# ashawkey/torch-ngp

Hardware: AMD Instinct MI355X
Metric: training samples/s (rays x steps), lego-shaped synthetic, fp16 autocast, full step incl. Adam (higher is better)
Workload: dtype f16

## Files before the change

### include/ngp_hip.h

```cpp
#ifndef NGP_HIP_H
#define NGP_HIP_H

#include <stddef.h>
#include <stdint.h>

#ifdef __cplusplus
extern "C" {
#endif

typedef void* ngp_stream_t;

enum {
    NGP_OK = 0,
    NGP_ERR_INVALID = 1,
    NGP_ERR_LAUNCH = 2,
    NGP_ERR_DEVICE = 3
};

enum { NGP_F32 = 0, NGP_F16 = 1, NGP_F64 = 2 };

#define NGP_MAX_LEVELS 32

const char* ngp_last_error(void);
int ngp_abi_version(void);
// ... 29 lines not shown
int ngp_grid_encode_backward_ordered(const void* grad, const float* inputs, const void* embeddings, const int32_t* offsets,
                                     void* grad_embeddings, uint32_t B, uint32_t D, uint32_t C, uint32_t L, float S, uint32_t H,
                                     const void* dy_dx, void* grad_inputs, uint32_t gridtype, int align_corners, uint32_t interp, int dtype,
                                     float bound, void* workspace, size_t workspace_bytes, ngp_stream_t stream);
int ngp_grid_encode_backward_backward_ordered(const void* grad, const float* inputs, const void* embeddings, const int32_t* offsets,
                                              const void* grad_grad_inputs, void* grad_grad, void* grad_embeddings, void* grad_inputs2,
                                              uint32_t B, uint32_t D, uint32_t C, uint32_t L, float S, uint32_t H, uint32_t gridtype,
                                              int align_corners, uint32_t interp, int dtype, void* workspace, size_t workspace_bytes,
                                              ngp_stream_t stream);
size_t ngp_grid_ordered_workspace_bytes(uint32_t B, uint32_t D, uint32_t C, int dtype);
int ngp_grid_backward_is_reproducible(const int32_t* offsets_host, uint32_t B, uint32_t D, uint32_t C, uint32_t L, float S, uint32_t H,
                                      uint32_t gridtype, int align_corners, int dtype);


int ngp_sh_encode_forward(const void* inputs, void* outputs, uint32_t B, uint32_t D, uint32_t C, void* dy_dx,
                          int dtype, ngp_stream_t stream);
int ngp_sh_encode_backward(const void* grad, const void* inputs, uint32_t B, uint32_t D, uint32_t C,
                           const void* dy_dx, void* grad_inputs, int dtype, ngp_stream_t stream);
int ngp_sh_encode_backward_backward(const void* grad, const void* inputs, const void* dy_dx, const void* u, uint32_t B, uint32_t D,
                                    uint32_t C, void* grad_grad, void* grad_inputs2, int dtype, ngp_stream_t stream);


int ngp_near_far_from_aabb(const float* rays_o, const float* rays_d, const float* aabb, uint32_t N, float min_near,
                           float* nears, float* fars, ngp_stream_t stream);
int ngp_sph_from_ray(const float* rays_o, const float* rays_d, float radius, uint32_t N, float* coords,
                     ngp_stream_t stream);
int ngp_morton3D(const int32_t* coords, uint32_t N, int32_t* indices, ngp_stream_t stream);
int ngp_morton3D_invert(const int32_t* indices, uint32_t N, int32_t* coords, ngp_stream_t stream);
int ngp_packbits(const float* grid, uint32_t N, float density_thresh, uint8_t* bitfield, ngp_stream_t stream);
int ngp_packbits_ex(const float* grid, uint32_t N, float density_thresh, const float* thresh_cap, uint8_t* bitfield,
                    ngp_stream_t stream);

size_t ngp_march_rays_train_workspace_bytes(uint32_t N);
int ngp_march_rays_train(const float* rays_o, const float* rays_d, const uint8_t* grid, float bound, float dt_gamma,
                         uint32_t max_steps, uint32_t N, uint32_t C, uint32_t H, uint32_t M, const float* nears,
                         const float* fars, float* xyzs, float* dirs, float* deltas, int32_t* rays,
                         int32_t* counter, const float* noises, void* workspace, ngp_stream_t stream);

int ngp_composite_rays_train_forward(const float* sigmas, const float* rgbs, const float* deltas,
                                     const int32_t* rays, uint32_t M, uint32_t N, float T_thresh,
                                     float* weights_sum, float* depth, float* image, ngp_stream_t stream);
int ngp_composite_rays_train_backward(const float* grad_weights_sum, const float* grad_image, const float* sigmas,
                                      const float* rgbs, const float* deltas, const int32_t* rays,
                                      const float* weights_sum, const float* image, uint32_t M, uint32_t N,
                                      float T_thresh, float* grad_sigmas, float* grad_rgbs, ngp_stream_t stream);

int ngp_march_rays(uint32_t n_alive, uint32_t n_step, const int32_t* rays_alive, const float* rays_t,
                   const float* rays_o, const float* rays_d, float bound, float dt_gamma, uint32_t max_steps,
                   uint32_t C, uint32_t H, const uint8_t* grid, const float* nears, const float* fars, float* xyzs,
                   float* dirs, float* deltas, const float* noises, ngp_stream_t stream);
int ngp_composite_rays(uint32_t n_alive, uint32_t n_step, float T_thresh, int32_t* rays_alive, float* rays_t,
                       const float* sigmas, const float* rgbs, const float* deltas, float* weights_sum,
                       float* depth, float* image, ngp_stream_t stream);

int ngp_near_far_from_aabb_f64(const double* rays_o, const double* rays_d, const double* aabb, uint32_t N, float min_near,
                               double* nears, double* fars, ngp_stream_t stream);
int ngp_sph_from_ray_f64(const double* rays_o, const double* rays_d, float radius, uint32_t N, double* coords, ngp_stream_t stream);
int ngp_packbits_f64(const double* grid, uint32_t N, float density_thresh, uint8_t* bitfield, ngp_stream_t stream);
int ngp_composite_rays_train_forward_f64(const double* sigmas, const double* rgbs, const double* deltas, const int32_t* rays,
                                         uint32_t M, uint32_t N, float T_thresh, double* weights_sum, double* depth, double* image,
                                         ngp_stream_t stream);
int ngp_composite_rays_train_backward_f64(const double* grad_weights_sum, const double* grad_image, const double* sigmas,
                                          const double* rgbs, const double* deltas, const int32_t* rays, const double* weights_sum,
                                          const double* image, uint32_t M, uint32_t N, float T_thresh, double* grad_sigmas,
                                          double* grad_rgbs, ngp_stream_t stream);
int ngp_composite_rays_f64(uint32_t n_alive, uint32_t n_step, float T_thresh, int32_t* rays_alive, double* rays_t,
                           const double* sigmas, const double* rgbs, const double* deltas, double* weights_sum, double* depth,
                           double* image, ngp_stream_t stream);

size_t ngp_compact_rays_workspace_bytes(uint32_t n_alive);
int ngp_compact_rays(const int32_t* rays_alive, uint32_t n_alive, int32_t* out_alive, int32_t* out_count,
                     void* workspace, ngp_stream_t stream);


int ngp_ffmlp_forward(const void* inputs, const void* weights, uint32_t B, uint32_t input_dim, uint32_t output_dim,
                      uint32_t hidden_dim, uint32_t num_layers, uint32_t activation, uint32_t output_activation,
                      void* forward_buffer, void* outputs, ngp_stream_t stream);
int ngp_ffmlp_inference(const void* inputs, const void* weights, uint32_t B, uint32_t input_dim,
                        uint32_t output_dim, uint32_t hidden_dim, uint32_t num_layers, uint32_t activation,
                        uint32_t output_activation, void* inference_buffer, void* outputs, ngp_stream_t stream);
int ngp_ffmlp_backward(const void* grad, const void* inputs, const void* weights, const void* forward_buffer,
                       uint32_t B, uint32_t input_dim, uint32_t output_dim, uint32_t hidden_dim, uint32_t num_layers,
                       uint32_t activation, uint32_t output_activation, int calc_grad_inputs, void* backward_buffer,
                       void* grad_inputs, void* grad_weights, ngp_stream_t stream);
int ngp_allocate_splitk(size_t size);
int ngp_free_splitk(void);

int ngp_grid_encode_forward_ex(const float* inputs, const void* embeddings, const int32_t* offsets, void* outputs,
                               uint32_t B, uint32_t D, uint32_t C, uint32_t L, float S, uint32_t H, void* dy_dx,
                               uint32_t gridtype, int align_corners, uint32_t interp, int dtype, float bound,
                               ngp_stream_t stream);
int ngp_grid_encode_backward_ex(const void* grad, const float* inputs, const void* embeddings, const int32_t* offsets,
                                void* grad_embeddings, uint32_t B, uint32_t D, uint32_t C, uint32_t L, float S,
                                uint32_t H, const void* dy_dx, void* grad_inputs, uint32_t gridtype, int align_corners,
                                uint32_t interp, int dtype, float bound, ngp_stream_t stream);
int ngp_grid_encode_forward_sched(const float* inputs, const void* embeddings, const int32_t* offsets, void* outputs,
                                  uint32_t B, uint32_t D, uint32_t C, uint32_t L, float S, uint32_t H, void* dy_dx,
                                  uint32_t gridtype, int align_corners, uint32_t interp, int dtype, float bound,
                                  const float* level_cost_host, ngp_stream_t stream);

int ngp_grid_encode_forward_sel(const float* inputs, const void* embeddings, const void* embeddings_alt, const float* parity,
                                const uint32_t* rows_dev, const int32_t* offsets, void* outputs, uint32_t B, uint32_t D, uint32_t C, uint32_t L,
                                float S, uint32_t H, uint32_t gridtype, int align_corners, uint32_t interp, int dtype, float bound,
                                const float* level_cost_host, ngp_stream_t stream);

uint32_t ngp_grid_forward_work_lists(uint32_t L, uint32_t tiles, const float* level_cost_host, uint16_t* level_out, uint32_t* tile0_out,
                                     uint32_t* end_out);

size_t ngp_grid_backward_workspace_bytes(const int32_t* offsets_host, uint32_t B, uint32_t D, uint32_t C, uint32_t L, float S, uint32_t H,
                                         uint32_t gridtype, int align_corners, int dtype);
int ngp_grid_encode_backward_checked(const void* grad, const float* inputs, const void* embeddings, const int32_t* offsets,
                                     void* grad_embeddings, uint32_t B, uint32_t D, uint32_t C, uint32_t L, float S, uint32_t H,
                                     const void* dy_dx, void* grad_inputs, uint32_t gridtype, int align_corners, uint32_t interp,
                                     int dtype, float bound, const int32_t* offsets_host, void* workspace, size_t workspace_bytes,
                                     float* found_inf, ngp_stream_t stream);

typedef struct ngp_table_adam {
    float* param[2]; float* exp_avg[2]; float* exp_avg_sq[2]; void* param_fp16[2];
    const float* state;
    float lr, beta1, beta2, eps;
} ngp_table_adam_t;
uint32_t ngp_grid_table_adam_prefix(const int32_t* offsets_host, uint32_t B, uint32_t D, uint32_t C, uint32_t L, float S, uint32_t H,
                                    uint32_t gridtype, int align_corners, int dtype);
typedef struct ngp_slab_sets {
    const void* slabs_a; uint32_t n_slabs_a, n_params_a; void* grad_weights_a;
    const void* slabs_b; uint32_t n_slabs_b, n_params_b; void* grad_weights_b;
    const float* ray_err; uint32_t n_rays; float* loss;
    uint32_t overwrite_table;
    const ngp_table_adam_t* table_adam;
} ngp_slab_sets_t;
int ngp_grid_encode_backward_checked_slabs(const void* grad, const float* inputs, const void* embeddings, const int32_t* offsets,
                                           void* grad_embeddings, uint32_t B, uint32_t D, uint32_t C, uint32_t L, float S, uint32_t H,
                                           const void* dy_dx, void* grad_inputs, uint32_t gridtype, int align_corners, uint32_t interp,
                                           int dtype, float bound, const int32_t* offsets_host, void* workspace, size_t workspace_bytes,
                                           float* found_inf, const ngp_slab_sets_t* slab_sets, ngp_stream_t stream);
int ngp_grid_encode_backward_ws(const void* grad, const float* inputs, const void* embeddings, const int32_t* offsets,
                                void* grad_embeddings, uint32_t B, uint32_t D, uint32_t C, uint32_t L, float S, uint32_t H,
                                const void* dy_dx, void* grad_inputs, uint32_t gridtype, int align_corners, uint32_t interp,
                                int dtype, float bound, const int32_t* offsets_host, void* workspace, size_t workspace_bytes,
                                ngp_stream_t stream);

size_t ngp_density_grid_update_workspace_bytes(uint32_t n_cells);
int ngp_density_grid_update(const float* sigmas, const int64_t* cells, uint32_t n, float density_scale, float decay, float* density_grid,
                            uint32_t n_cells, float* scratch, float density_thresh, float* mean_out, uint8_t* bitfield, void* workspace,
                            ngp_stream_t stream);

#define NGP_FF_INPUT_PLANAR 1u
#define NGP_FF_DX_PLANAR 2u
#define NGP_FF_LAYERED 4u
#define NGP_FF_SINGLE_WAVE 8u
#define NGP_FF_DEFER_REDUCE 16u
#define NGP_FF_RECOMPUTE 32u
#define NGP_FF_SERIAL_FLUSH 64u
int ngp_ffmlp_forward_ex(const void* inputs, const void* weights, uint32_t B, uint32_t input_dim, uint32_t output_dim,
                         uint32_t hidden_dim, uint32_t num_layers, uint32_t activation, uint32_t output_activation,
                         void* forward_buffer, void* outputs, uint32_t flags, ngp_stream_t stream);
int ngp_ffmlp_inference_ex(const void* inputs, const void* weights, uint32_t B, uint32_t input_dim,
                           uint32_t output_dim, uint32_t hidden_dim, uint32_t num_layers, uint32_t activation,
                           uint32_t output_activation, void* inference_buffer, void* outputs, uint32_t flags,
                           ngp_stream_t stream);
int ngp_ffmlp_backward_ex(const void* grad, const void* inputs, const void* weights, const void* forward_buffer,
                          uint32_t B, uint32_t input_dim, uint32_t output_dim, uint32_t hidden_dim, uint32_t num_layers,
                          uint32_t activation, uint32_t output_activation, int calc_grad_inputs, void* backward_buffer,
                          void* grad_inputs, void* grad_weights, uint32_t flags, ngp_stream_t stream);

size_t ngp_ffmlp_backward_workspace_bytes(uint32_t B, uint32_t input_dim, uint32_t hidden_dim, uint32_t num_layers);
int ngp_ffmlp_backward_ws(const void* grad, const void* inputs, const void* weights, const void* forward_buffer, uint32_t B,
                          uint32_t input_dim, uint32_t output_dim, uint32_t hidden_dim, uint32_t num_layers, uint32_t activation,
                          uint32_t output_activation, int calc_grad_inputs, void* backward_buffer, void* grad_inputs, void* grad_weights,
                          uint32_t flags, void* workspace, size_t workspace_bytes, ngp_stream_t stream);

size_t ngp_ffmlp_backward_backward_workspace_bytes(uint32_t B, uint32_t input_dim, uint32_t hidden_dim, uint32_t num_layers,
                                                   uint32_t activation);
int ngp_ffmlp_backward_backward(const void* grad, const void* inputs, const void* weights, const void* forward_buffer, const void* u,
                                uint32_t B, uint32_t input_dim, uint32_t output_dim, uint32_t hidden_dim, uint32_t num_layers,
                                uint32_t activation, void* grad_grad, void* grad_weights2, void* grad_inputs2, void* workspace,
                                size_t workspace_bytes, ngp_stream_t stream);

int ngp_network_forward(const void* enc, const float* dirs, uint32_t M, uint32_t M_valid, const void* w_sigma, const void* w_color,
                        uint32_t num_layers_sigma, uint32_t num_layers_color, float density_scale, int training,
                        void* forward_buffer_sigma, void* h16, float* sigma, void* color_in, void* forward_buffer_color, float* rgb,
                        uint32_t flags, ngp_stream_t stream);

int ngp_network_forward_rows(const void* enc, const float* dirs, uint32_t M, uint32_t M_valid, const void* w_sigma, const void* w_color,
                             uint32_t num_layers_sigma, uint32_t num_layers_color, float density_scale, int training,
                             void* forward_buffer_sigma, void* h16, float* sigma, void* color_in, void* forward_buffer_color, float* rgb,
                             uint32_t flags, const uint32_t* rows_dev, ngp_stream_t stream);

int ngp_network_backward_color(const void* grad_out16, const void* color_in, const void* w_color, const void* forward_buffer_color, uint32_t M,
                               uint32_t num_layers_color, void* backward_buffer, const float* grad_sigma, const void* h16,
                               float density_scale, void* grad_h16, void* grad_w_color, uint32_t flags, ngp_stream_t stream);
uint32_t ngp_ffmlp_backward_slab_count(uint32_t B, uint32_t input_dim, uint32_t hidden_dim, uint32_t num_layers);
int ngp_ffmlp_reduce_slabs_pair(const void* slabs_a, uint32_t n_slabs_a, uint32_t n_params_a, void* grad_weights_a, const void* slabs_b,
                                uint32_t n_slabs_b, uint32_t n_params_b, void* grad_weights_b, float* found_inf, ngp_stream_t stream);

int ngp_pipeline_mid_forward(const void* h16, const float* dirs, float* sigma, void* color_in, uint32_t M, uint32_t M_valid,
                             float density_scale, ngp_stream_t stream);
int ngp_pipeline_rgb_forward(const void* out16, float* rgb, uint32_t M, ngp_stream_t stream);
int ngp_pipeline_rgb_backward(const float* grad_rgb, const float* rgb, void* grad_out16, uint32_t M, ngp_stream_t stream);
int ngp_pipeline_mid_backward(const float* grad_sigma, const void* h16, const void* grad_color_in, void* grad_h16, uint32_t M,
                              float density_scale, ngp_stream_t stream);

int ngp_pipeline_mse_loss(const float* image, const float* target, uint32_t n, const float* loss_scale, float* loss,
                          float* grad_image, ngp_stream_t stream);

#define NGP_LINEAR_STACK_MAX 8
uint32_t ngp_linear_stack_flat_size(uint32_t depth, uint32_t n_in, uint32_t hidden, uint32_t n_out, int identity);
int ngp_linear_stack_pack(const float* const* weights, uint32_t depth, uint32_t n_in, uint32_t hidden, uint32_t n_out, int identity,
                          void* flat_fp16, ngp_stream_t stream);
int ngp_linear_stack_unpack_grad(const void* grad_flat_fp16, uint32_t depth, uint32_t n_in, uint32_t hidden, uint32_t n_out, int identity,
                                 float* const* grads, ngp_stream_t stream);

int ngp_pad_2d_fp16(const void* src, uint32_t src_rows, uint32_t src_cols, uint32_t src_row_stride, void* dst, uint32_t dst_rows,
                    uint32_t dst_cols, ngp_stream_t stream);

int ngp_rays_from_pixels(const float* poses, uint32_t B, float fx, float fy, float cx, float cy, uint32_t W, const int64_t* inds,
                         uint32_t inds_batch_stride, uint32_t N, float* rays_o, float* rays_d, ngp_stream_t stream);

#define NGP_MARCH_RESET_COUNTER 1u
#define NGP_MARCH_ZERO_TAIL 2u
#define NGP_MARCH_SCAN_LAUNCH 8u
#define NGP_MARCH_NOISE_FROM_SEED 4u
int ngp_march_rays_train_ex(const float* rays_o, const float* rays_d, const uint8_t* grid, float bound, float dt_gamma,
                            uint32_t max_steps, uint32_t N, uint32_t C, uint32_t H, uint32_t M, const float* nears,
                            const float* fars, float* xyzs, float* dirs, float* deltas, int32_t* rays, int32_t* counter,
                            const float* noises, void* workspace, uint32_t flags, ngp_stream_t stream);
int ngp_march_rays_train_aabb(const float* rays_o, const float* rays_d, const uint8_t* grid, float bound, float dt_gamma,
                              uint32_t max_steps, uint32_t N, uint32_t C, uint32_t H, uint32_t M, const float* aabb, float min_near,
                              float* nears, float* fars, float* xyzs, float* dirs, float* deltas, int32_t* rays, int32_t* counter,
                              const float* noises, void* workspace, uint32_t flags, ngp_stream_t stream);

int ngp_march_rays_ex(uint32_t n_alive, uint32_t n_step, const int32_t* rays_alive, const float* rays_t, const float* rays_o,
                      const float* rays_d, float bound, float dt_gamma, uint32_t max_steps, uint32_t C, uint32_t H,
                      const uint8_t* grid, const float* nears, const float* fars, float* xyzs, float* dirs, float* deltas,
                      const float* noises, uint32_t zero_rows, ngp_stream_t stream);

int ngp_march_rays_dev(const int32_t* state, uint32_t alive_bound, uint32_t n_total, uint32_t n_step_cap, const int32_t* rays_alive, const float* rays_t,
                       const float* rays_o, const float* rays_d, float bound, float dt_gamma, uint32_t max_steps, uint32_t C, uint32_t H,
                       const uint8_t* grid, const float* nears, const float* fars, float* xyzs, float* dirs, float* deltas,
                       const float* noises, uint32_t rows, ngp_stream_t stream);
int ngp_march_rays_dev_rows(const int32_t* state, uint32_t alive_bound, uint32_t n_total, uint32_t n_step_cap, const int32_t* rays_alive, const float* rays_t,
                            const float* rays_o, const float* rays_d, float bound, float dt_gamma, uint32_t max_steps, uint32_t C, uint32_t H,
                            const uint8_t* grid, const float* nears, const float* fars, float* xyzs, float* dirs, float* deltas,
                            const float* noises, uint32_t rows, uint32_t* rows_used, ngp_stream_t stream);
int ngp_composite_rays_dev(const int32_t* state, uint32_t alive_bound, uint32_t n_total, uint32_t n_step_cap, float T_thresh, int32_t* rays_alive, float* rays_t,
                           const float* sigmas, const float* rgbs, const float* deltas, float* weights_sum, float* depth, float* image,
                           ngp_stream_t stream);
int ngp_compact_rays_dev(const int32_t* state, uint32_t alive_bound, uint32_t n_total, uint32_t n_step_cap, uint32_t max_steps, const int32_t* rays_alive,
                         int32_t* out_alive, int32_t* out_state, void* workspace, ngp_stream_t stream);

int ngp_composite_rays_features(uint32_t n_alive, uint32_t n_step, float T_thresh, const int32_t* rays_alive, const float* sigmas,
                                const void* feats, const float* deltas, const float* weights_sum, uint32_t C, int feat_dtype,
                                float* out, ngp_stream_t stream);
int ngp_composite_rays_features_dev(const int32_t* state, uint32_t alive_bound, uint32_t n_total, uint32_t n_step_cap, float T_thresh,
                                    const int32_t* rays_alive, const float* sigmas, const void* feats, const float* deltas,
                                    const float* weights_sum, uint32_t C, int feat_dtype, float* out, ngp_stream_t stream);

typedef struct ngp_render_loop {
    int32_t* state;
    int32_t* alive[2];
    float* rays_t; const float* rays_o; const float* rays_d; const float* nears; const float* fars; const uint8_t* grid; const float* noises;
    float* xyzs; float* dirs; float* deltas; void* enc; float* sigmas; float* rgbs;
    const void* embeddings; const int32_t* offsets; const float* level_cost_host; const void* w_sigma; const void* w_color;
    float* weights_sum; float* depth; float* image; void* compact_workspace;
    uint32_t* rows_used;
    uint32_t lanes, rows, n_total, n_step_cap, max_steps, cascade, grid_size;
    uint32_t L, H, gridtype, interp, num_layers_sigma, num_layers_color;
    int32_t align_corners;
    float bound, dt_gamma, T_thresh, S, density_scale;
} ngp_render_loop_t;
int ngp_render_iterations_dev(const ngp_render_loop_t* args, uint32_t n_iter, uint32_t first_cur, ngp_stream_t stream);

size_t ngp_coarse_occupancy_bytes(uint32_t C, uint32_t H);
int ngp_coarse_occupancy(const uint8_t* grid, uint32_t C, uint32_t H, uint8_t* coarse, ngp_stream_t stream);
int ngp_cull_rays(const float* rays_o, const float* rays_d, const float* nears, const float* fars, uint32_t N, float bound, uint32_t C,
                  uint32_t H, const uint8_t* coarse, int32_t* rays_alive, ngp_stream_t stream);

int ngp_composite_rays_train_forward_ex(const float* sigmas, const float* rgbs, const float* deltas, const int32_t* rays,
                                        uint32_t M, uint32_t N, float T_thresh, float* weights_sum, float* depth, float* image,
                                        int bg_mode, float bg_scalar, const float* bg, const float* nears, const float* fars,
                                        float* image_out, float* depth_out, ngp_stream_t stream);
int ngp_composite_rays_train_backward_ex(const float* grad_weights_sum, const float* grad_image, const float* sigmas,
                                         const float* rgbs, const float* deltas, const int32_t* rays,
                                         const float* weights_sum, const float* image, uint32_t M, uint32_t N,
                                         float T_thresh, float* grad_sigmas, float* grad_rgbs, int bg_mode, float bg_scalar,
                                         const float* bg, const uint32_t* rows_used, ngp_stream_t stream);

int ngp_composite_rays_train_geo_forward(const float* sigmas, const float* rgbs, const float* deltas, const int32_t* rays, uint32_t M,
                                         uint32_t N, float T_thresh, float* weights_sum, float* depth, float* image,
                                         float* distortion, ngp_stream_t stream);
int ngp_composite_rays_train_geo_backward(const float* grad_weights_sum, const float* grad_depth, const float* grad_image,
                                          const float* grad_distortion, const float* sigmas, const float* rgbs, const float* deltas,
                                          const int32_t* rays, const float* weights_sum, const float* depth, const float* image,
                                          const float* distortion, uint32_t M, uint32_t N, float T_thresh, float* grad_sigmas,
                                          float* grad_rgbs, ngp_stream_t stream);
int ngp_composite_rays_train_geo_forward_f64(const double* sigmas, const double* rgbs, const double* deltas, const int32_t* rays,
                                             uint32_t M, uint32_t N, float T_thresh, double* weights_sum, double* depth, double* image,
                                             double* distortion, ngp_stream_t stream);
int ngp_composite_rays_train_geo_backward_f64(const double* grad_weights_sum, const double* grad_depth, const double* grad_image,
                                              const double* grad_distortion, const double* sigmas, const double* rgbs,
                                              const double* deltas, const int32_t* rays, const double* weights_sum, const double* depth,
                                              const double* image, const double* distortion, uint32_t M, uint32_t N, float T_thresh,
                                              double* grad_sigmas, double* grad_rgbs, ngp_stream_t stream);

int ngp_composite_rays_train_features_forward(const float* sigmas, const void* feats, const float* deltas, const int32_t* rays, uint32_t M,
                                              uint32_t N, uint32_t C, float T_thresh, int feat_dtype, float* out, ngp_stream_t stream);
// ... 93 lines not shown
```

### torch-ngp_amd/_ngp_capi.py

```python
import ctypes
import os

import torch

_HERE = os.path.dirname(os.path.abspath(__file__))
LIB_PATH = os.environ.get('NGP_HIP_LIBRARY') or os.path.join(_HERE, 'libngp_hip.so')

NGP_F32, NGP_F16, NGP_F64 = 0, 1, 2
NGP_FF_INPUT_PLANAR, NGP_FF_DX_PLANAR, NGP_FF_LAYERED, NGP_FF_SINGLE_WAVE, NGP_FF_DEFER_REDUCE, NGP_FF_RECOMPUTE = 1, 2, 4, 8, 16, 32
NGP_FF_SERIAL_FLUSH = 64
NGP_MARCH_RESET_COUNTER, NGP_MARCH_ZERO_TAIL, NGP_MARCH_NOISE_FROM_SEED, NGP_MARCH_SCAN_LAUNCH = 1, 2, 4, 8
NGP_OPT_PHASE_CHECK, NGP_OPT_PHASE_UPDATE, NGP_OPT_PHASE_COMMIT, NGP_OPT_PHASE_FLIP = 1, 2, 4, 8
ABI_VERSION = 11

if not os.path.exists(LIB_PATH):
    raise ImportError(
        f"{LIB_PATH} is missing: build the HIP extension first (python __graft_entry__.py, or "
        f"make -C {os.path.join(_HERE, 'csrc')}).  There is no CPU fallback for these operators.")

lib = ctypes.CDLL(LIB_PATH)

_vp, _u32, _f32, _i32, _sz = ctypes.c_void_p, ctypes.c_uint32, ctypes.c_float, ctypes.c_int, ctypes.c_size_t

_SIGNATURES = {
    'ngp_grid_encode_forward': [_vp, _vp, _vp, _vp, _u32, _u32, _u32, _u32, _f32, _u32, _vp, _u32, _i32, _u32, _i32, _vp],
    'ngp_grid_encode_backward': [_vp, _vp, _vp, _vp, _vp, _u32, _u32, _u32, _u32, _f32, _u32, _vp, _vp, _u32, _i32, _u32, _i32, _vp],
    'ngp_grad_total_variation': [_vp, _vp, _vp, _vp, _f32, _u32, _u32, _u32, _u32, _f32, _u32, _u32, _i32, _i32, _vp],
    'ngp_grid_corner_indices': [_vp, _vp, _vp, _u32, _u32, _u32, _f32, _u32, _u32, _i32, _vp],
    'ngp_grid_level_table': [_u32, _f32, _u32, _vp, _vp],
    'ngp_grid_encode_backward_backward': [_vp, _vp, _vp, _vp, _vp, _vp, _vp, _vp, _u32, _u32, _u32, _u32, _f32, _u32, _u32, _i32, _u32, _i32, _vp,
                                          _sz, _vp],
    'ngp_grid_encode_backward_ordered': [_vp, _vp, _vp, _vp, _vp, _u32, _u32, _u32, _u32, _f32, _u32, _vp, _vp, _u32, _i32, _u32, _i32, _f32, _vp,
                                         _sz, _vp],
    'ngp_grid_encode_backward_backward_ordered': [_vp, _vp, _vp, _vp, _vp, _vp, _vp, _vp, _u32, _u32, _u32, _u32, _f32, _u32, _u32, _i32, _u32, _i32,
                                                  _vp, _sz, _vp],
    'ngp_grid_backward_is_reproducible': [_vp, _u32, _u32, _u32, _u32, _f32, _u32, _u32, _i32, _i32],
    'ngp_sh_encode_forward': [_vp, _vp, _u32, _u32, _u32, _vp, _i32, _vp],
    'ngp_sh_encode_backward': [_vp, _vp, _u32, _u32, _u32, _vp, _vp, _i32, _vp],
    'ngp_freq_encode_forward': [_vp, _u32, _u32, _u32, _u32, _vp, _vp],
    'ngp_freq_encode_backward': [_vp, _vp, _u32, _u32, _u32, _u32, _vp, _vp],
    'ngp_freq_encode_forward_f64': [_vp, _u32, _u32, _u32, _u32, _vp, _vp],
    'ngp_freq_encode_backward_f64': [_vp, _vp, _u32, _u32, _u32, _u32, _vp, _vp],
    'ngp_freq_encode_backward_backward': [_vp, _vp, _vp, _u32, _u32, _u32, _u32, _vp, _vp, _i32, _vp],
    'ngp_sh_encode_backward_backward': [_vp, _vp, _vp, _vp, _u32, _u32, _u32, _vp, _vp, _i32, _vp],
    'ngp_near_far_from_aabb': [_vp, _vp, _vp, _u32, _f32, _vp, _vp, _vp],
    'ngp_sph_from_ray': [_vp, _vp, _f32, _u32, _vp, _vp],
    'ngp_morton3D': [_vp, _u32, _vp, _vp],
    'ngp_morton3D_invert': [_vp, _u32, _vp, _vp],
    'ngp_packbits': [_vp, _u32, _f32, _vp, _vp],
    'ngp_packbits_ex': [_vp, _u32, _f32, _vp, _vp, _vp],
    'ngp_march_rays_train': [_vp, _vp, _vp, _f32, _f32, _u32, _u32, _u32, _u32, _u32, _vp, _vp, _vp, _vp, _vp, _vp, _vp, _vp, _vp, _vp],
    'ngp_composite_rays_train_forward': [_vp, _vp, _vp, _vp, _u32, _u32, _f32, _vp, _vp, _vp, _vp],
    'ngp_composite_rays_train_backward': [_vp, _vp, _vp, _vp, _vp, _vp, _vp, _vp, _u32, _u32, _f32, _vp, _vp, _vp],
    'ngp_march_rays': [_u32, _u32, _vp, _vp, _vp, _vp, _f32, _f32, _u32, _u32, _u32, _vp, _vp, _vp, _vp, _vp, _vp, _vp, _vp],
    'ngp_march_rays_ex': [_u32, _u32, _vp, _vp, _vp, _vp, _f32, _f32, _u32, _u32, _u32, _vp, _vp, _vp, _vp, _vp, _vp, _vp, _u32, _vp],
    'ngp_composite_rays': [_u32, _u32, _f32, _vp, _vp, _vp, _vp, _vp, _vp, _vp, _vp, _vp],
    'ngp_near_far_from_aabb_f64': [_vp, _vp, _vp, _u32, _f32, _vp, _vp, _vp],
    'ngp_sph_from_ray_f64': [_vp, _vp, _f32, _u32, _vp, _vp],
    'ngp_packbits_f64': [_vp, _u32, _f32, _vp, _vp],
    'ngp_composite_rays_train_forward_f64': [_vp, _vp, _vp, _vp, _u32, _u32, _f32, _vp, _vp, _vp, _vp],
    'ngp_composite_rays_train_backward_f64': [_vp, _vp, _vp, _vp, _vp, _vp, _vp, _vp, _u32, _u32, _f32, _vp, _vp, _vp],
    'ngp_composite_rays_f64': [_u32, _u32, _f32, _vp, _vp, _vp, _vp, _vp, _vp, _vp, _vp, _vp],
    'ngp_compact_rays': [_vp, _u32, _vp, _vp, _vp, _vp],
    'ngp_coarse_occupancy': [_vp, _u32, _u32, _vp, _vp],
    'ngp_cull_rays': [_vp, _vp, _vp, _vp, _u32, _f32, _u32, _u32, _vp, _vp, _vp],
    'ngp_march_rays_dev': [_vp, _u32, _u32, _u32, _vp, _vp, _vp, _vp, _f32, _f32, _u32, _u32, _u32, _vp, _vp, _vp, _vp, _vp, _vp, _vp, _u32, _vp],
    'ngp_composite_rays_dev': [_vp, _u32, _u32, _u32, _f32, _vp, _vp, _vp, _vp, _vp, _vp, _vp, _vp, _vp],
    'ngp_compact_rays_dev': [_vp, _u32, _u32, _u32, _u32, _vp, _vp, _vp, _vp, _vp],
    'ngp_render_iterations_dev': [_vp, _u32, _u32, _vp],
    'ngp_ffmlp_forward': [_vp, _vp, _u32, _u32, _u32, _u32, _u32, _u32, _u32, _vp, _vp, _vp],
    'ngp_ffmlp_inference': [_vp, _vp, _u32, _u32, _u32, _u32, _u32, _u32, _u32, _vp, _vp, _vp],
    'ngp_ffmlp_backward': [_vp, _vp, _vp, _vp, _u32, _u32, _u32, _u32, _u32, _u32, _u32, _i32, _vp, _vp, _vp, _vp],
    'ngp_grid_encode_forward_ex': [_vp, _vp, _vp, _vp, _u32, _u32, _u32, _u32, _f32, _u32, _vp, _u32, _i32, _u32, _i32, _f32, _vp],
    'ngp_grid_encode_forward_sched': [_vp, _vp, _vp, _vp, _u32, _u32, _u32, _u32, _f32, _u32, _vp, _u32, _i32, _u32, _i32, _f32, _vp, _vp],
    'ngp_grid_encode_forward_sel': [_vp, _vp, _vp, _vp, _vp, _vp, _vp, _u32, _u32, _u32, _u32, _f32, _u32, _u32, _i32, _u32, _i32, _f32, _vp, _vp],
    'ngp_grid_encode_backward_ex': [_vp, _vp, _vp, _vp, _vp, _u32, _u32, _u32, _u32, _f32, _u32, _vp, _vp, _u32, _i32, _u32, _i32, _f32, _vp],
    'ngp_grid_encode_backward_ws': [_vp, _vp, _vp, _vp, _vp, _u32, _u32, _u32, _u32, _f32, _u32, _vp, _vp, _u32, _i32, _u32, _i32, _f32, _vp, _vp,
                                    _sz, _vp],
    'ngp_grid_encode_backward_checked': [_vp, _vp, _vp, _vp, _vp, _u32, _u32, _u32, _u32, _f32, _u32, _vp, _vp, _u32, _i32, _u32, _i32, _f32, _vp,
                                         _vp, _sz, _vp, _vp],
    'ngp_grid_encode_backward_checked_slabs': [_vp, _vp, _vp, _vp, _vp, _u32, _u32, _u32, _u32, _f32, _u32, _vp, _vp, _u32, _i32, _u32, _i32, _f32,
                                               _vp, _vp, _sz, _vp, _vp, _vp],
    'ngp_density_grid_update': [_vp, _vp, _u32, _f32, _f32, _vp, _u32, _vp, _f32, _vp, _vp, _vp, _vp],
    'ngp_ffmlp_forward_ex': [_vp, _vp, _u32, _u32, _u32, _u32, _u32, _u32, _u32, _vp, _vp, _u32, _vp],
    'ngp_ffmlp_inference_ex': [_vp, _vp, _u32, _u32, _u32, _u32, _u32, _u32, _u32, _vp, _vp, _u32, _vp],
    'ngp_ffmlp_backward_ex': [_vp, _vp, _vp, _vp, _u32, _u32, _u32, _u32, _u32, _u32, _u32, _i32, _vp, _vp, _vp, _u32, _vp],
    'ngp_ffmlp_backward_ws': [_vp, _vp, _vp, _vp, _u32, _u32, _u32, _u32, _u32, _u32, _u32, _i32, _vp, _vp, _vp, _u32, _vp, _sz, _vp],
    'ngp_ffmlp_backward_backward': [_vp, _vp, _vp, _vp, _vp, _u32, _u32, _u32, _u32, _u32, _u32, _vp, _vp, _vp, _vp, _sz, _vp],
    'ngp_network_forward': [_vp, _vp, _u32, _u32, _vp, _vp, _u32, _u32, _f32, _i32, _vp, _vp, _vp, _vp, _vp, _vp, _u32, _vp],
    'ngp_network_forward_rows': [_vp, _vp, _u32, _u32, _vp, _vp, _u32, _u32, _f32, _i32, _vp, _vp, _vp, _vp, _vp, _vp, _u32, _vp, _vp],
    'ngp_march_rays_dev_rows': [_vp, _u32, _u32, _u32, _vp, _vp, _vp, _vp, _f32, _f32, _u32, _u32, _u32, _vp, _vp, _vp, _vp, _vp, _vp, _vp, _u32, _vp, _vp],
    'ngp_pipeline_mid_forward': [_vp, _vp, _vp, _vp, _u32, _u32, _f32, _vp],
    'ngp_pipeline_rgb_forward': [_vp, _vp, _u32, _vp],
    'ngp_pipeline_rgb_backward': [_vp, _vp, _vp, _u32, _vp],
    'ngp_pipeline_mid_backward': [_vp, _vp, _vp, _vp, _u32, _f32, _vp],
    'ngp_pipeline_mse_loss': [_vp, _vp, _u32, _vp, _vp, _vp, _vp],
    'ngp_rays_from_pixels': [_vp, _u32, _f32, _f32, _f32, _f32, _u32, _vp, _u32, _u32, _vp, _vp, _vp],
    'ngp_march_rays_train_ex': [_vp, _vp, _vp, _f32, _f32, _u32, _u32, _u32, _u32, _u32, _vp, _vp, _vp, _vp, _vp, _vp, _vp, _vp, _vp, _u32, _vp],
    'ngp_march_rays_train_aabb': [_vp, _vp, _vp, _f32, _f32, _u32, _u32, _u32, _u32, _u32, _vp, _f32, _vp, _vp, _vp, _vp, _vp, _vp, _vp, _vp, _vp, _u32,
                                  _vp],
    'ngp_composite_rays_train_forward_ex': [_vp, _vp, _vp, _vp, _u32, _u32, _f32, _vp, _vp, _vp, _i32, _f32, _vp, _vp, _vp, _vp, _vp, _vp],
    'ngp_composite_rays_train_backward_ex': [_vp, _vp, _vp, _vp, _vp, _vp, _vp, _vp, _u32, _u32, _f32, _vp, _vp, _i32, _f32, _vp, _vp, _vp],
    'ngp_composite_rays_train_geo_forward': [_vp, _vp, _vp, _vp, _u32, _u32, _f32, _vp, _vp, _vp, _vp, _vp],
    'ngp_composite_rays_train_geo_backward': [_vp, _vp, _vp, _vp, _vp, _vp, _vp, _vp, _vp, _vp, _vp, _vp, _u32, _u32, _f32, _vp, _vp, _vp],
    'ngp_composite_rays_train_geo_forward_f64': [_vp, _vp, _vp, _vp, _u32, _u32, _f32, _vp, _vp, _vp, _vp, _vp],
    'ngp_composite_rays_train_geo_backward_f64': [_vp, _vp, _vp, _vp, _vp, _vp, _vp, _vp, _vp, _vp, _vp, _vp, _u32, _u32, _f32, _vp, _vp, _vp],
    'ngp_composite_rays_train_features_forward': [_vp, _vp, _vp, _vp, _u32, _u32, _u32, _f32, _i32, _vp, _vp],
    'ngp_composite_rays_train_features_backward': [_vp, _vp, _vp, _vp, _vp, _vp, _u32, _u32, _u32, _f32, _i32, _vp, _vp, _vp],
    'ngp_composite_rays_train_features_forward_f64': [_vp, _vp, _vp, _vp, _u32, _u32, _u32, _f32, _vp, _vp],
    'ngp_composite_rays_train_features_backward_f64': [_vp, _vp, _vp, _vp, _vp, _vp, _u32, _u32, _u32, _f32, _vp, _vp, _vp],
    'ngp_composite_rays_features': [_u32, _u32, _f32, _vp, _vp, _vp, _vp, _vp, _u32, _i32, _vp, _vp],
    'ngp_composite_rays_features_dev': [_vp, _u32, _u32, _u32, _f32, _vp, _vp, _vp, _vp, _vp, _u32, _i32, _vp, _vp],
    'ngp_composite_train_loss_backward': [_vp, _vp, _vp, _vp, _u32, _u32, _f32, _i32, _f32, _vp, _vp, _vp, _vp, _vp, _vp, _vp, _vp, _vp, _vp, _vp,
                                          _vp, _vp, _sz, _vp],
    'ngp_composite_train_geo_loss_backward': [_vp, _vp, _vp, _vp, _u32, _u32, _f32, _i32, _f32, _vp, _vp, _vp, _vp, _f32, _f32, _vp, _vp, _vp, _vp,
                                              _vp, _vp, _vp, _vp, _vp, _vp, _vp, _vp, _vp, _sz, _vp],
    'ngp_network_backward_color': [_vp, _vp, _vp, _vp, _u32, _u32, _vp, _vp, _vp, _f32, _vp, _vp, _u32, _vp],
    'ngp_ffmlp_reduce_slabs_pair': [_vp, _u32, _u32, _vp, _vp, _u32, _u32, _vp, _vp, _vp],
    'ngp_optim_adam_step': [_i32, _vp, _vp, _vp, _vp, _vp, _vp, _vp, _vp, _f32, _f32, _f32, _f32, _f32, _f32, _f32, _vp, _vp],
    'ngp_optim_adam_step_ex': [_i32, _vp, _vp, _vp, _vp, _vp, _vp, _vp, _vp, _f32, _f32, _f32, _f32, _f32, _f32, _f32, _vp, _vp, _f32, _u32, _vp],
    'ngp_optim_adam_small_commit': [_i32, _vp, _vp, _vp, _vp, _vp, _vp, _vp, _vp, _f32, _f32, _f32, _f32, _f32, _f32, _f32, _vp, _i32, _vp, _vp,
                                    ctypes.c_uint64, _vp],
    'ngp_optim_ema_update': [_i32, _vp, _vp, _vp, _f32, _vp],
    'ngp_optim_poison_shards': [_vp, _u32, ctypes.c_uint64, _vp, _vp],
    'ngp_optim_shard_verdict': [_vp, _vp, _vp, _u32, ctypes.c_uint64, _vp],
    'ngp_linear_stack_pack': [_vp, _u32, _u32, _u32, _u32, _i32, _vp, _vp],
    'ngp_linear_stack_unpack_grad': [_vp, _u32, _u32, _u32, _u32, _i32, _vp, _vp],
    'ngp_pad_2d_fp16': [_vp, _u32, _u32, _u32, _vp, _u32, _u32, _vp],
    'ngp_allocate_splitk': [_sz],
    'ngp_free_splitk': [],
    'ngp_cmdlist_create': [_vp],
    'ngp_cmdlist_begin': [_vp],
    'ngp_cmdlist_mark': [_vp, _u32, _i32],
    'ngp_cmdlist_end': [_vp],
    'ngp_cmdlist_count': [_vp, _vp],
    'ngp_cmdlist_entry_name': [_vp, _u32, _vp, _u32],
    'ngp_cmdlist_replay': [_vp, _vp],
    'ngp_cmdlist_wait_mark': [_vp, _u32, _vp],
    'ngp_cmdlist_destroy': [_vp],
    'ngp_ray_sample_ts': [_vp, _vp, _vp, _vp, _u32, _u32, _f32, _vp, _vp],
    'ngp_ray_sample_ts_f64': [_vp, _vp, _vp, _vp, _u32, _u32, _f32, _vp, _vp],
    'ngp_ray_points_forward': [_vp, _vp, _vp, _vp, _u32, _u32, _f32, _vp, _vp, _vp],
    'ngp_ray_points_forward_f64': [_vp, _vp, _vp, _vp, _u32, _u32, _f32, _vp, _vp, _vp],
    'ngp_ray_points_backward': [_vp, _vp, _vp, _vp, _vp, _vp, _vp, _u32, _u32, _f32, _vp, _vp, _vp],
    'ngp_ray_points_backward_f64': [_vp, _vp, _vp, _vp, _vp, _vp, _u32, _u32, _f32, _vp, _vp, _vp],
    'ngp_grid_input_gradient': [_vp, _vp, _vp, _vp, _u32, _u32, _u32, _u32, _f32, _u32, _u32, _i32, _u32, _i32, _f32, _vp, _vp],
    'ngp_rays_from_pixels_backward': [_vp, _vp, _u32, _f32, _f32, _f32, _f32, _u32, _vp, _u32, _u32, _vp, _vp],
}
for _name, _args in _SIGNATURES.items():
    _fn = getattr(lib, _name)
    _fn.argtypes = _args
    _fn.restype = ctypes.c_int
lib.ngp_last_error.restype = ctypes.c_char_p
lib.ngp_target_arch.restype = ctypes.c_char_p
lib.ngp_abi_version.restype = ctypes.c_int
lib.ngp_ffmlp_backward_slab_count.argtypes = [_u32, _u32, _u32, _u32]
lib.ngp_ffmlp_backward_slab_count.restype = _u32
lib.ngp_march_rays_train_workspace_bytes.argtypes = [_u32]
lib.ngp_march_rays_train_workspace_bytes.restype = _sz
lib.ngp_compact_rays_workspace_bytes.argtypes = [_u32]
lib.ngp_ffmlp_backward_workspace_bytes.argtypes = [_u32, _u32, _u32, _u32]
lib.ngp_ffmlp_backward_workspace_bytes.restype = _sz
lib.ngp_ffmlp_backward_backward_workspace_bytes.argtypes = [_u32, _u32, _u32, _u32, _u32]
# ... 156 lines not shown
```

### torch-ngp_amd/csrc/ffmlp.hip

```cpp
#include "common.h"
#include "sh_poly.inc"

namespace ngp {

constexpr int FF_WAVES = 4;
constexpr int FF_THREADS = FF_WAVES * 64;
constexpr int FF_TILE = 32;

enum Act : uint32_t { ACT_RELU = 0, ACT_EXP = 1, ACT_SINE = 2, ACT_SIGMOID = 3, ACT_SQUAREPLUS = 4, ACT_SOFTPLUS = 5, ACT_NONE = 6 };
constexpr float K_ACT = 10.0f;

__device__ __forceinline__ float act_forward(uint32_t a, float x) {
    switch (a) {
        case ACT_RELU: return x > 0.0f ? x : 0.0f;
        case ACT_EXP: return __expf(x);
        case ACT_SINE: return __sinf(x);
        case ACT_SIGMOID: return 1.0f / (1.0f + __expf(-x));
        case ACT_SQUAREPLUS: { const float s = x * K_ACT; return 0.5f * (s + sqrtf(s * s + 4.0f)) / K_ACT; }
        case ACT_SOFTPLUS: return __logf(__expf(x * K_ACT) + 1.0f) / K_ACT;
        default: return x;
    }
}
__device__ __forceinline__ float act_backward_factor(uint32_t a, float y) {
    switch (a) {
// ... 138 lines not shown
            const uint32_t e = e0 + b * blockDim.x;
            const half_t *pl = nullptr, *ph = nullptr;
            if (e < total) forward_fragment_source<WIDTH>(e + shift, w, in_dim, num_layers, pl, ph);
            real[b] = pl != nullptr;
            lo[b] = *reinterpret_cast<const half4_t*>(pl ? pl : w);
            hi[b] = *reinterpret_cast<const half4_t*>(ph ? ph : w);
        }
#pragma unroll
        for (int b = 0; b < IMG_BATCH; b++) {
            const uint32_t e = e0 + b * blockDim.x;
            if (e < total) {
                const half4_t z = {(half_t)0.0f, (half_t)0.0f, (half_t)0.0f, (half_t)0.0f};
                const half4_t l4 = real[b] ? lo[b] : z, h4 = real[b] ? hi[b] : z;
                img[e] = half8_t{l4.x, l4.y, l4.z, l4.w, h4.x, h4.y, h4.z, h4.w};
            }
        }
    }
}

template <int WIDTH>
__device__ __forceinline__ void pack_hidden(const float16_t (&acc)[Shape<WIDTH>::NIB], half8_t (&frag)[Shape<WIDTH>::NKB]) {
#pragma unroll
    for (int kb = 0; kb < Shape<WIDTH>::NKB; kb++) {
#pragma unroll
        for (int j = 0; j < 8; j++) frag[kb][j] = (half_t)acc[kb >> 1][(kb & 1) * 8 + j];
    }
}

__device__ __forceinline__ uint32_t relu_pack2(float a, float b) {
    typedef float f32x2 __attribute__((ext_vector_type(2)));
    typedef short i16x2 __attribute__((ext_vector_type(2)));
    const half2_t hv = __builtin_convertvector(f32x2{a, b}, half2_t);
    return __builtin_bit_cast(uint32_t, __builtin_elementwise_max(__builtin_bit_cast(i16x2, hv), i16x2{0, 0}));
}
template <int WIDTH>
__device__ __forceinline__ void pack_hidden_relu(const float16_t (&acc)[Shape<WIDTH>::NIB], half8_t (&frag)[Shape<WIDTH>::NKB]) {
    typedef uint32_t u32x4 __attribute__((ext_vector_type(4)));
#pragma unroll
    for (int kb = 0; kb < Shape<WIDTH>::NKB; kb++) {
        u32x4 w;
#pragma unroll
        for (int q = 0; q < 4; q++) w[q] = relu_pack2(acc[kb >> 1][(kb & 1) * 8 + 2 * q], acc[kb >> 1][(kb & 1) * 8 + 2 * q + 1]);
        frag[kb] = __builtin_bit_cast(half8_t, w);
    }
}


__device__ __forceinline__ half8_t load_features8(const half_t* __restrict__ inputs, bool planar, size_t rows, size_t s, uint32_t in_dim,
                                                  uint32_t f0) {
    if (!planar) return *reinterpret_cast<const half8_t*>(inputs + s * in_dim + f0);
    half8_t v;
#pragma unroll
    for (int q = 0; q < 4; q++) {
        const half2_t t = *reinterpret_cast<const half2_t*>(inputs + ((size_t)(f0 / 2 + q) * rows + s) * 2);
        v[2 * q] = t.x;
        v[2 * q + 1] = t.y;
    }
    return v;
}

template <typename V>
__device__ __forceinline__ void stream_store(V* dst, V v) {
    __builtin_nontemporal_store(v, dst);
}

template <int WIDTH, bool TRAIN, bool PLAIN >
__device__ __forceinline__ void ffmlp_forward_body(const half_t* __restrict__ inputs, const half_t* __restrict__ weights,
                                                   half_t* __restrict__ forward_buffer, half_t* __restrict__ outputs, uint32_t n_tiles,
                                                   uint32_t in_dim, uint32_t num_layers, uint32_t act, uint32_t out_act, bool in_planar) {
    constexpr int NIB = Shape<WIDTH>::NIB, NKB = Shape<WIDTH>::NKB;
    extern __shared__ __attribute__((aligned(16))) unsigned char smem[];
    half8_t* img = reinterpret_cast<half8_t*>(smem);
    build_forward_image<WIDTH>(img, weights, in_dim, num_layers);
    const size_t rows = (size_t)n_tiles * FF_TILE;
    __syncthreads();

    const int lane = threadIdx.x & 63, wid = threadIdx.x >> 6;
    const int n = lane & 31, h = lane >> 5;
    const uint32_t in_kb = in_dim / 16;
    const half8_t* img_l0 = img + lane;
    const half8_t* img_hid = img_l0 + (size_t)NIB * in_kb * 64;
    const half8_t* img_out = img_hid + (size_t)(num_layers - 1) * NIB * NKB * 64;
    const size_t layer_stride = (size_t)n_tiles * NKB * 64;

    for (uint32_t tile = blockIdx.x * FF_WAVES + wid; tile < n_tiles; tile += gridDim.x * FF_WAVES) {
        const size_t srow = (size_t)tile * FF_TILE + n;
        float16_t acc[NIB];
#pragma unroll
        for (int ib = 0; ib < NIB; ib++) acc[ib] = zero16();
        for (uint32_t kb = 0; kb < in_kb; kb++) {
            const half8_t x = load_features8(inputs, in_planar, rows, srow, in_dim, 16 * kb + 8 * h);
#pragma unroll
            for (int ib = 0; ib < NIB; ib++) acc[ib] = mfma(img_l0[(ib * in_kb + kb) * 64], x, acc[ib]);
        }
        half8_t hid[NKB];
        for (uint32_t l = 0;; l++) {
            if (PLAIN || act == ACT_RELU) {
                pack_hidden_relu<WIDTH>(acc, hid);
            } else {
                if (act != ACT_NONE) {
#pragma unroll
                    for (int ib = 0; ib < NIB; ib++)
#pragma unroll
                        for (int r = 0; r < 16; r++) acc[ib][r] = act_forward(act, acc[ib][r]);
                }
                pack_hidden<WIDTH>(acc, hid);
            }
            if (TRAIN) {
                half8_t* dst = reinterpret_cast<half8_t*>(forward_buffer) + l * layer_stride + (size_t)tile * NKB * 64 + lane;
#pragma unroll
                for (int kb = 0; kb < NKB; kb++) stream_store(dst + kb * 64, hid[kb]);
            }
            if (l + 1 == num_layers) break;
            const half8_t* wl = img_hid + (size_t)l * NIB * NKB * 64;
#pragma unroll
            for (int ib = 0; ib < NIB; ib++) {
                acc[ib] = zero16();
#pragma unroll
                for (int kb = 0; kb < NKB; kb++) acc[ib] = mfma(wl[(ib * NKB + kb) * 64], hid[kb], acc[ib]);
            }
        }
        float16_t o = zero16();
#pragma unroll
        for (int kb = 0; kb < NKB; kb++) o = mfma(img_out[kb * 64], hid[kb], o);
        half4_t lo, hi;
#pragma unroll
        for (int c = 0; c < 4; c++) {
            lo[c] = (half_t)(PLAIN ? o[c] : act_forward(out_act, o[c]));
            hi[c] = (half_t)(PLAIN ? o[4 + c] : act_forward(out_act, o[4 + c]));
        }
        half_t* orow = outputs + ((size_t)tile * FF_TILE + n) * 16 + 4 * h;
        *reinterpret_cast<half4_t*>(orow) = lo;
        *reinterpret_cast<half4_t*>(orow + 8) = hi;
    }
}

template <int WIDTH, bool TRAIN, bool PLAIN>
__global__ __launch_bounds__(FF_THREADS) __attribute__((amdgpu_waves_per_eu(4, 4))) void k_ffmlp_forward(
    const half_t* __restrict__ inputs, const half_t* __restrict__ weights, half_t* __restrict__ forward_buffer, half_t* __restrict__ outputs,
    uint32_t n_tiles, uint32_t in_dim, uint32_t num_layers, uint32_t act, uint32_t out_act, bool in_planar) {
    ffmlp_forward_body<WIDTH, TRAIN, PLAIN>(inputs, weights, forward_buffer, outputs, n_tiles, in_dim, num_layers, act, out_act, in_planar);
}
template <int WIDTH, bool TRAIN, bool PLAIN>
__global__ __launch_bounds__(FF_THREADS) __attribute__((amdgpu_waves_per_eu(2, 2))) void k_ffmlp_forward_wide(
    const half_t* __restrict__ inputs, const half_t* __restrict__ weights, half_t* __restrict__ forward_buffer, half_t* __restrict__ outputs,
    uint32_t n_tiles, uint32_t in_dim, uint32_t num_layers, uint32_t act, uint32_t out_act, bool in_planar) {
    ffmlp_forward_body<WIDTH, TRAIN, PLAIN>(inputs, weights, forward_buffer, outputs, n_tiles, in_dim, num_layers, act, out_act, in_planar);
}


template <bool TRAIN, int NT>
__device__ __forceinline__ void relu_network_tail(float16_t (&acc)[NT][2], float16_t (&o)[NT], const half8_t* __restrict__ hid_img,
                                                  const half8_t* __restrict__ out_img, uint32_t nl, half_t* __restrict__ fb, size_t layer_stride,
                                                  const uint32_t (&tile)[NT], const bool (&live)[NT], int lane) {
    constexpr int WIDTH = 64, NIB = 2, NKB = 4;
    half8_t hid[NT][NKB];
    for (uint32_t l = 0;; l++) {
#pragma unroll
        for (int t = 0; t < NT; t++) {
            pack_hidden_relu<WIDTH>(acc[t], hid[t]);
            if (TRAIN && fb && live[t]) {
                half8_t* dst = reinterpret_cast<half8_t*>(fb) + l * layer_stride + (size_t)tile[t] * NKB * 64 + lane;
#pragma unroll
                for (int kb = 0; kb < NKB; kb++) stream_store(dst + kb * 64, hid[t][kb]);
            }
        }
        if (l + 1 == nl) break;
        const half8_t* wl = hid_img + (size_t)l * NIB * NKB * 64;
#pragma unroll
        for (int ib = 0; ib < NIB; ib++) {
#pragma unroll
            for (int t = 0; t < NT; t++) acc[t][ib] = zero16();
#pragma unroll
            for (int kb = 0; kb < NKB; kb++) {
                const half8_t a = wl[(ib * NKB + kb) * 64];
#pragma unroll
                for (int t = 0; t < NT; t++) acc[t][ib] = mfma(a, hid[t][kb], acc[t][ib]);
            }
        }
    }
#pragma unroll
    for (int t = 0; t < NT; t++) o[t] = zero16();
#pragma unroll
    for (int kb = 0; kb < NKB; kb++) {
        const half8_t a = out_img[kb * 64];
#pragma unroll
        for (int t = 0; t < NT; t++) o[t] = mfma(a, hid[t][kb], o[t]);
    }
}

template <bool TRAIN, int WAVES , int NT >
__global__ __launch_bounds__(WAVES * 64) __attribute__((amdgpu_waves_per_eu(NT == 1 ? 4 : 2, NT == 1 ? 4 : 3))) void k_network_forward(
    const half_t* __restrict__ enc, bool enc_planar, const float* __restrict__ dirs, uint32_t M_valid, const half_t* __restrict__ w_sigma,
    const half_t* __restrict__ w_color, half_t* __restrict__ fb_s, half_t* __restrict__ h16, float* __restrict__ sigma,
    half_t* __restrict__ color_in, half_t* __restrict__ fb_c, float* __restrict__ rgb, uint32_t n_tiles_cap, uint32_t nl_s, uint32_t nl_c,
    float density_scale, const uint32_t* __restrict__ rows_dev) {
    constexpr int WIDTH = 64, NIB = 2, NKB = 4;
    constexpr uint32_t in_kb = 2;
    const uint32_t n_tiles = rows_dev ? min(n_tiles_cap, (rows_dev[0] + (uint32_t)FF_TILE - 1u) / (uint32_t)FF_TILE) : n_tiles_cap;
    extern __shared__ __attribute__((aligned(16))) unsigned char smem[];
    half8_t* img_s = reinterpret_cast<half8_t*>(smem);
    const uint32_t frags_s = NIB * in_kb + (nl_s - 1) * NIB * NKB + NKB;
    half8_t* img_c = img_s + (size_t)frags_s * 64;
    const size_t rows = (size_t)n_tiles_cap * FF_TILE;
    const int lane = threadIdx.x & 63, wid = threadIdx.x >> 6;
    const int n = lane & 31, h = lane >> 5;
    const uint32_t n_groups = (n_tiles + NT - 1) / NT;
    half8_t x_next[NT][in_kb];
    float dir_next[NT][3];
#pragma unroll
    for (int t = 0; t < NT; t++) dir_next[t][0] = dir_next[t][1] = dir_next[t][2] = 0.0f;
    auto request = [&](uint32_t group) {
        if (group < n_groups) {
#pragma unroll
            for (int t = 0; t < NT; t++) {
                const uint32_t tl = group * NT + t < n_tiles ? group * NT + t : n_tiles - 1;
                const size_t srow = (size_t)tl * FF_TILE + n;
#pragma unroll
                for (uint32_t kb = 0; kb < in_kb; kb++) x_next[t][kb] = load_features8(enc, enc_planar, rows, srow, 32, 16 * kb + 8 * h);
                dir_next[t][0] = dir_next[t][1] = dir_next[t][2] = 0.0f;
                if (srow < M_valid) { dir_next[t][0] = dirs[srow * 3]; dir_next[t][1] = dirs[srow * 3 + 1]; dir_next[t][2] = dirs[srow * 3 + 2]; }
            }
        }
    };
    request(blockIdx.x * WAVES + wid);
    build_forward_image<WIDTH>(img_s, w_sigma, 32, nl_s);
    build_forward_image<WIDTH>(img_c, w_color, 32, nl_c);
    __syncthreads();

    const size_t layer_stride = (size_t)n_tiles_cap * NKB * 64;
    const half8_t* s_l0 = img_s + lane;
    const half8_t* s_hid = s_l0 + (size_t)NIB * in_kb * 64;
    const half8_t* s_out = s_hid + (size_t)(nl_s - 1) * NIB * NKB * 64;
    const half8_t* c_l0 = img_c + lane;
    const half8_t* c_hid = c_l0 + (size_t)NIB * in_kb * 64;
    const half8_t* c_out = c_hid + (size_t)(nl_c - 1) * NIB * NKB * 64;

    for (uint32_t group = blockIdx.x * WAVES + wid; group < n_groups; group += gridDim.x * WAVES) {
        uint32_t tile[NT];
        bool live[NT];
        size_t srow[NT];
        half8_t x_cur[NT][in_kb];
        float dir_x[NT], dir_y[NT], dir_z[NT];
#pragma unroll
        for (int t = 0; t < NT; t++) {
            live[t] = NT == 1 || group * NT + t < n_tiles;
            tile[t] = live[t] ? group * NT + t : n_tiles - 1;
            srow[t] = (size_t)tile[t] * FF_TILE + n;
#pragma unroll
            for (uint32_t kb = 0; kb < in_kb; kb++) x_cur[t][kb] = x_next[t][kb];
            dir_x[t] = dir_next[t][0]; dir_y[t] = dir_next[t][1]; dir_z[t] = dir_next[t][2];
        }
        request(group + gridDim.x * WAVES);
        float16_t acc[NT][NIB], o[NT];
#pragma unroll
        for (int t = 0; t < NT; t++)
#pragma unroll
            for (int ib = 0; ib < NIB; ib++) acc[t][ib] = zero16();
#pragma unroll
        for (uint32_t kb = 0; kb < in_kb; kb++)
#pragma unroll
            for (int ib = 0; ib < NIB; ib++) {
                const half8_t a = s_l0[(ib * in_kb + kb) * 64];
#pragma unroll
                for (int t = 0; t < NT; t++) acc[t][ib] = mfma(a, x_cur[t][kb], acc[t][ib]);
            }
        relu_network_tail<TRAIN, NT>(acc, o, s_hid, s_out, nl_s, fb_s, layer_stride, tile, live, lane);
        half8_t cin[NT][2];
#pragma unroll
        for (int t = 0; t < NT; t++) {
            half4_t lo, hi;
#pragma unroll
            for (int c = 0; c < 4; c++) { lo[c] = (half_t)o[t][c]; hi[c] = (half_t)o[t][4 + c]; }
            if (TRAIN && live[t]) {
                half_t* hrow = h16 + srow[t] * 16 + 4 * h;
                *reinterpret_cast<half4_t*>(hrow) = lo;
                *reinterpret_cast<half4_t*>(hrow + 8) = hi;
            }
            if (h == 0 && live[t]) sigma[srow[t]] = density_scale * expf((float)lo[0]);
            const float x = dir_x[t], y = dir_y[t], z = dir_z[t];
            float sh_0, sh_1, sh_2, sh_3, sh_4, sh_5, sh_6, sh_7, sh_8, sh_9, sh_10, sh_11, sh_12, sh_13, sh_14, sh_15;
#define SH_OUT(i, v) { sh_##i = (v); asm volatile("" : "+v"(sh_##i)); }
            SH_BAND_0_VALUES;
            SH_BAND_1_VALUES;
            SH_BAND_2_VALUES;
            SH_BAND_3_VALUES;
#undef SH_OUT
            typedef float f32x2 __attribute__((ext_vector_type(2)));
#define SH_PAIR(q, a0, a1, b0, b1) { const half2_t pr = __builtin_convertvector(f32x2{h ? b0 : a0, h ? b1 : a1}, half2_t); cin[t][0][2 * (q)] = pr.x; cin[t][0][2 * (q) + 1] = pr.y; }
            SH_PAIR(0, sh_0, sh_1, sh_8, sh_9);
            SH_PAIR(1, sh_2, sh_3, sh_10, sh_11);
            SH_PAIR(2, sh_4, sh_5, sh_12, sh_13);
            SH_PAIR(3, sh_6, sh_7, sh_14, sh_15);
#undef SH_PAIR
            const uint32_t m0 = __builtin_bit_cast(uint32_t, half2_t{lo[0], lo[1]}), m1 = __builtin_bit_cast(uint32_t, half2_t{lo[2], lo[3]});
            const uint32_t m2 = __builtin_bit_cast(uint32_t, half2_t{hi[0], hi[1]}), m3 = __builtin_bit_cast(uint32_t, half2_t{hi[2], hi[3]});
            const half2_t p0 = __builtin_bit_cast(half2_t, (uint32_t)__shfl_xor((int)m0, 32, 64)), p1 = __builtin_bit_cast(half2_t, (uint32_t)__shfl_xor((int)m1, 32, 64));
            const half2_t p2 = __builtin_bit_cast(half2_t, (uint32_t)__shfl_xor((int)m2, 32, 64)), p3 = __builtin_bit_cast(half2_t, (uint32_t)__shfl_xor((int)m3, 32, 64));
            if (h == 0) {
                cin[t][1][0] = lo[1]; cin[t][1][1] = lo[2]; cin[t][1][2] = lo[3];
                cin[t][1][3] = p0.x; cin[t][1][4] = p0.y; cin[t][1][5] = p1.x; cin[t][1][6] = p1.y;
                cin[t][1][7] = hi[0];
            } else {
                cin[t][1][0] = p2.y; cin[t][1][1] = p3.x; cin[t][1][2] = p3.y;
                cin[t][1][3] = hi[0]; cin[t][1][4] = hi[1]; cin[t][1][5] = hi[2]; cin[t][1][6] = hi[3];
                cin[t][1][7] = (half_t)0.0f;
            }
            if (TRAIN && live[t]) {
                half_t* crow = color_in + srow[t] * 32 + 8 * h;
                stream_store(reinterpret_cast<half8_t*>(crow), cin[t][0]);
                stream_store(reinterpret_cast<half8_t*>(crow + 16), cin[t][1]);
            }
        }
#pragma unroll
        for (int t = 0; t < NT; t++)
#pragma unroll
            for (int ib = 0; ib < NIB; ib++) acc[t][ib] = zero16();
#pragma unroll
        for (uint32_t kb = 0; kb < in_kb; kb++)
#pragma unroll
            for (int ib = 0; ib < NIB; ib++) {
                const half8_t a = c_l0[(ib * in_kb + kb) * 64];
#pragma unroll
                for (int t = 0; t < NT; t++) acc[t][ib] = mfma(a, cin[t][kb], acc[t][ib]);
            }
        relu_network_tail<TRAIN, NT>(acc, o, c_hid, c_out, nl_c, fb_c, layer_stride, tile, live, lane);
#pragma unroll
        for (int t = 0; t < NT; t++) {
            if (h == 0 && live[t]) {
                float* prgb = rgb + srow[t] * 3;
#pragma unroll
                for (int c = 0; c < 3; c++) {
                    const float v = (float)(half_t)o[t][c];
                    prgb[c] = (float)to_half_rne(1.0f / (1.0f + expf(-v)));
                }
            }
        }
    }
}

template <int WIDTH>
__host__ __device__ __forceinline__ uint32_t bwd_frag_count(uint32_t in_dim, uint32_t num_layers, bool with_dx) {
    constexpr int NIB = Shape<WIDTH>::NIB, NKB = Shape<WIDTH>::NKB;
    return NIB + (num_layers - 1) * NIB * NKB + (with_dx ? ((in_dim + 31) / 32) * NKB : 0);
}

template <int WIDTH>
__device__ __forceinline__ void backward_fragment_source(uint32_t e, const half_t* __restrict__ w, uint32_t in_dim, uint32_t num_layers,
                                                         const half_t*& src, uint32_t& stride, bool& slot_order) {
    constexpr int NIB = Shape<WIDTH>::NIB, NKB = Shape<WIDTH>::NKB;
    const half_t* w_hid = w + (size_t)WIDTH * in_dim;
    const half_t* w_out = w_hid + (size_t)(num_layers - 1) * WIDTH * WIDTH;
    const uint32_t frag = e >> 6, lane = e & 63;
    const int i = lane & 31, h = lane >> 5;
    uint32_t f = frag;
    if (f < NIB) {
        src = 32 * f + i < (uint32_t)WIDTH ? w_out + (size_t)(8 * h) * WIDTH + (32 * f + i) : nullptr;
        stride = WIDTH;
        slot_order = false;
    } else if ((f -= NIB) < (num_layers - 1) * NIB * NKB) {
        const uint32_t li = f / (NIB * NKB), rem = f % (NIB * NKB);
        const uint32_t ib = rem / NKB, kb = rem % NKB;
        const half_t* wl = w_hid + (size_t)(num_layers - 2 - li) * WIDTH * WIDTH;
        src = 32 * ib + i < (uint32_t)WIDTH ? wl + (size_t)slot_feature(kb, h, 0) * WIDTH + (32 * ib + i) : nullptr;
        stride = WIDTH;
        slot_order = true;
    } else {
        f -= (num_layers - 1) * NIB * NKB;
        const uint32_t ib = f / NKB, kb = f % NKB;
        const uint32_t col = 32 * ib + i;
        src = col < in_dim ? w + (size_t)slot_feature(kb, h, 0) * in_dim + col : nullptr;
        stride = in_dim;
        slot_order = true;
    }
}

template <int WIDTH>
__device__ void build_backward_image(half8_t* img, const half_t* __restrict__ w, uint32_t in_dim, uint32_t num_layers, bool with_dx,
                                     uint32_t first_frag = 0, uint32_t n_frags = 0xFFFFFFFFu) {
    constexpr int BATCH = 3;
    const uint32_t total = (n_frags == 0xFFFFFFFFu ? bwd_frag_count<WIDTH>(in_dim, num_layers, with_dx) : n_frags) * 64;
    const uint32_t shift = first_frag * 64;
    for (uint32_t e0 = threadIdx.x; e0 < total; e0 += BATCH * blockDim.x) {
        half_t v[BATCH][8];
        bool real[BATCH];
#pragma unroll
        for (int b = 0; b < BATCH; b++) {
            const uint32_t e = e0 + b * blockDim.x;
            const half_t* src = nullptr;
            uint32_t stride = 0;
            bool slot_order = false;
            if (e < total) backward_fragment_source<WIDTH>(e + shift, w, in_dim, num_layers, src, stride, slot_order);
            real[b] = src != nullptr;
            const half_t* p = src ? src : w;
            const uint32_t st = src ? stride : 0u;
#pragma unroll
            for (int j = 0; j < 8; j++) {
                const uint32_t row = slot_order ? (uint32_t)((j & 3) + 8 * (j >> 2)) : (uint32_t)j;
                v[b][j] = p[(size_t)row * st];
            }
        }
#pragma unroll
        for (int b = 0; b < BATCH; b++) {
            const uint32_t e = e0 + b * blockDim.x;
            if (e < total) {
                half8_t o;
#pragma unroll
                for (int j = 0; j < 8; j++) o[j] = real[b] ? v[b][j] : (half_t)0.0f;
                img[e] = o;
            }
        }
    }
}

struct Selectors {
    half8_t hid[2];
    half8_t nat[2];
    half8_t out;
};

__device__ __forceinline__ Selectors make_selectors(int n, int h) {
    Selectors s;
#pragma unroll
    for (int e = 0; e < 2; e++)
#pragma unroll
        for (int j = 0; j < 8; j++) {
            const bool hid = ((n >> 4) == e) && (((n >> 2) & 1) == h) && (j == ((n >> 3) & 1) * 4 + (n & 3));
            const bool nat = ((n >> 4) == e) && (((n >> 3) & 1) == h) && (j == (n & 7));
            s.hid[e][j] = hid ? (half_t)1.0f : (half_t)0.0f;
            s.nat[e][j] = nat ? (half_t)1.0f : (half_t)0.0f;
        }
#pragma unroll
    for (int j = 0; j < 8; j++) s.out[j] = ((n < 16) && ((n >> 3) == h) && (j == (n & 7))) ? (half_t)1.0f : (half_t)0.0f;
    return s;
}

__device__ __forceinline__ void pack_transposed(const float16_t& t, half8_t (&frag)[2]) {
#pragma unroll
    for (int g = 0; g < 2; g++)
#pragma unroll
        for (int j = 0; j < 8; j++) frag[g][j] = (half_t)t[8 * g + j];
}

template <int WIDTH>
__device__ __forceinline__ void transpose_hidden(const half8_t (&v)[Shape<WIDTH>::NKB], const Selectors& sel,
                                                 half8_t (&out)[Shape<WIDTH>::NIB][2]) {
#pragma unroll
    for (int ib = 0; ib < Shape<WIDTH>::NIB; ib++) {
        float16_t t = mfma(v[2 * ib], sel.hid[0], zero16());
        if constexpr (Shape<WIDTH>::NKB > 1) t = mfma(v[2 * ib + 1], sel.hid[1], t);
        pack_transposed(t, out[ib]);
    }
}

__device__ __noinline__ float act_backward_factor_slow(uint32_t a, float y) { return act_backward_factor(a, y); }

template <int WIDTH, bool RELU>
__device__ __forceinline__ void activation_transfer(uint32_t act, const float16_t (&acc)[Shape<WIDTH>::NIB],
                                                    const half8_t (&post)[Shape<WIDTH>::NKB], half8_t (&dz)[Shape<WIDTH>::NKB]) {
    if (RELU) {
        typedef short short2_t __attribute__((ext_vector_type(2)));
#pragma unroll
        for (int kb = 0; kb < Shape<WIDTH>::NKB; kb++) {
            uint32_t out[4];
#pragma unroll
            for (int q = 0; q < 4; q++) {
                const half2_t h = {(half_t)acc[kb >> 1][(kb & 1) * 8 + 2 * q], (half_t)acc[kb >> 1][(kb & 1) * 8 + 2 * q + 1]};
                const half2_t y = {post[kb][2 * q], post[kb][2 * q + 1]};
                const short2_t live = ((short2_t){0, 0} - __builtin_bit_cast(short2_t, y)) >> (short2_t){15, 15};
                out[q] = __builtin_bit_cast(uint32_t, h) & __builtin_bit_cast(uint32_t, live);
            }
            uint32_t packed[4] = {out[0], out[1], out[2], out[3]};
            __builtin_memcpy(&dz[kb], packed, sizeof(packed));
        }
    } else {
#pragma unroll
        for (int kb = 0; kb < Shape<WIDTH>::NKB; kb++)
#pragma unroll
            for (int j = 0; j < 8; j++)
// ... 216 lines not shown
#pragma unroll
    for (int li = 0; li < NHM; li++) {
        const uint32_t base = lay.hidden(lay.num_layers - 1 - li);
#pragma unroll
        for (int ib = 0; ib < NIB; ib++)
#pragma unroll
            for (int jb = 0; jb < NIB; jb++) sink.put(gw_hid[li][ib][jb], base, WIDTH, ib, jb, WIDTH, WIDTH);
    }
#pragma unroll
    for (int jb = 0; jb < NIB; jb++) sink.put(gw_out[jb], lay.out(), WIDTH, 0, jb, 16, WIDTH);
}

template <int WIDTH, int IN_JB , int NHM , bool RELU >
__global__ __launch_bounds__(FF_THREADS) void k_ffmlp_backward(const half_t* __restrict__ grad, const half_t* __restrict__ inputs,
                                                               const half_t* __restrict__ weights, const half_t* __restrict__ forward_buffer,
                                                               uint32_t n_tiles, uint32_t in_dim, uint32_t num_layers, uint32_t act,
                                                               bool with_dx, half_t* __restrict__ grad_inputs, float* __restrict__ slabs,
                                                               half_t* __restrict__ grad_weights_direct, bool in_planar, bool dx_planar, uint32_t pf_depth,
                                                               uint32_t lds_bytes, bool serial_flush) {
    constexpr int NIB = Shape<WIDTH>::NIB, NKB = Shape<WIDTH>::NKB;
    extern __shared__ __attribute__((aligned(16))) unsigned char smem[];
    half8_t* img = reinterpret_cast<half8_t*>(smem);
    const uint32_t nfrag = bwd_frag_count<WIDTH>(in_dim, num_layers, with_dx);
    build_backward_image<WIDTH>(img, weights, in_dim, num_layers, with_dx);
    const int lane = threadIdx.x & 63, wid = threadIdx.x >> 6;
    const int n = lane & 31, h = lane >> 5;
    (void)nfrag;
    const Selectors sel = make_selectors(n, h);
    __syncthreads();

    const uint32_t in_kb = in_dim / 16;
    const half8_t* img_out = img + lane;
    const half8_t* img_hid = img_out + (size_t)NIB * 64;
    const half8_t* img_in = img_hid + (size_t)(num_layers - 1) * NIB * NKB * 64;
    const size_t layer_stride = (size_t)n_tiles * NKB * 64;
    const half8_t* fb = reinterpret_cast<const half8_t*>(forward_buffer);
    const size_t rows = (size_t)n_tiles * FF_TILE;

    float16_t gw_out[NIB];
    float16_t gw_in[NIB][IN_JB];
#pragma unroll
    for (int jb = 0; jb < NIB; jb++) gw_out[jb] = zero16();
#pragma unroll
    for (int ib = 0; ib < NIB; ib++)
#pragma unroll
        for (int jb = 0; jb < IN_JB; jb++) gw_in[ib][jb] = zero16();
    float16_t gw_hid[NHM][NIB][NIB];
#pragma unroll
    for (int l = 0; l < NHM; l++)
#pragma unroll
        for (int ib = 0; ib < NIB; ib++)
#pragma unroll
            for (int jb = 0; jb < NIB; jb++) gw_hid[l][ib][jb] = zero16();

    const uint32_t tile_frags = 1 + num_layers * NKB + in_dim / 16;
    unsigned char* pf_base = smem + (size_t)nfrag * 1024 + (size_t)wid * pf_depth * tile_frags * 1024;
    const uint32_t tile_step = gridDim.x * FF_WAVES;
    uint32_t cur = 0;
    {
        const uint32_t first = blockIdx.x * FF_WAVES + wid;
        if (first < n_tiles) prefetch_tile<WIDTH>(pf_base, first, grad, fb, inputs, num_layers, layer_stride, rows, in_dim, in_planar, lane, n, h);
    }
    for (uint32_t tile = blockIdx.x * FF_WAVES + wid; tile < n_tiles; tile += tile_step) {
        asm volatile("s_waitcnt vmcnt(0)" ::: "memory");
        const unsigned char* tb = pf_base + (size_t)cur * tile_frags * 1024;
        if (pf_depth > 1) {
            cur ^= 1u;
            if (tile + tile_step < n_tiles)
                prefetch_tile<WIDTH>(pf_base + (size_t)cur * tile_frags * 1024, tile + tile_step, grad, fb, inputs, num_layers, layer_stride,
                                     rows, in_dim, in_planar, lane, n, h);
        }
        const half8_t* tfrag = reinterpret_cast<const half8_t*>(tb) + lane;
        const half8_t dy = tfrag[0];
        half8_t a_prev[NKB];
#pragma unroll
        for (int kb = 0; kb < NKB; kb++) a_prev[kb] = tfrag[(1 + (num_layers - 1) * NKB + kb) * 64];
        half8_t aT[NIB][2], zT[NIB][2];
        transpose_hidden<WIDTH>(a_prev, sel, aT);
        {
            half8_t yT[2];
            pack_transposed(mfma(dy, sel.out, zero16()), yT);
#pragma unroll
            for (int g = 0; g < 2; g++)
#pragma unroll
                for (int jb = 0; jb < NIB; jb++) gw_out[jb] = mfma(yT[g], aT[jb][g], gw_out[jb]);
        }
        float16_t acc[NIB];
        dgrad_out<WIDTH>(img_out, dy, acc);

        half8_t dz[NKB];
#pragma unroll
        for (int li = 0; li < NHM; li++) {
            activation_transfer<WIDTH, RELU>(act, acc, a_prev, dz);
            const uint32_t lay = num_layers - 1 - li;
#pragma unroll
            for (int kb = 0; kb < NKB; kb++) a_prev[kb] = tfrag[(1 + (lay - 1) * NKB + kb) * 64];
            transpose_hidden<WIDTH>(dz, sel, zT);
            transpose_hidden<WIDTH>(a_prev, sel, aT);
            wgrad_blocks(zT, aT, gw_hid[li]);
            dgrad_hidden<WIDTH>(img_hid + (size_t)li * NIB * NKB * 64, dz, acc);
        }
        activation_transfer<WIDTH, RELU>(act, acc, a_prev, dz);
        transpose_hidden<WIDTH>(dz, sel, zT);
        {
#pragma unroll
            for (int jb = 0; jb < IN_JB; jb++) {
                float16_t t = zero16();
#pragma unroll
                for (int e = 0; e < 2; e++) {
                    const uint32_t kb = 2 * jb + e;
                    if (kb < in_kb) t = mfma(tile_x(tb + (size_t)(1 + num_layers * NKB) * 1024, kb, in_planar, lane), sel.nat[e], t);
                }
                half8_t xT[2];
                pack_transposed(t, xT);
#pragma unroll
                for (int g = 0; g < 2; g++)
#pragma unroll
                    for (int ib = 0; ib < NIB; ib++) gw_in[ib][jb] = mfma(zT[ib][g], xT[g], gw_in[ib][jb]);
            }
        }
        if (with_dx) store_dx<WIDTH, IN_JB>(img_in, dz, grad_inputs, tile, n, h, in_dim, rows, dx_planar);
        if (pf_depth == 1 && tile + tile_step < n_tiles) {
            asm volatile("s_waitcnt lgkmcnt(0)" ::: "memory");
            prefetch_tile<WIDTH>(pf_base, tile + tile_step, grad, fb, inputs, num_layers, layer_stride, rows, in_dim, in_planar, lane, n, h);
        }
    }

    float* red = reinterpret_cast<float*>(smem);
    const SlabLayout lay{WIDTH, in_dim, num_layers};
    const uint32_t n_params = lay.n_params();
    auto each = [&](const auto& sink) { slab_put_all<WIDTH, IN_JB, NHM>(sink, lay, gw_in, gw_hid, gw_out); };
    if (slab_staged_single<WIDTH, IN_JB, NHM> && !serial_flush) {
        static_assert(!slab_staged_single<WIDTH, IN_JB, NHM> || slab_fits_whole<WIDTH, IN_JB, NHM>, "the single-wave staged sum is one pass");
        slab_sum_pass<FF_THREADS>(red, lds_bytes, SlabPart{0, n_params}, wid, slabs + (size_t)blockIdx.x * n_params, grad_weights_direct, n, h, each);
        return;
    }
    slab_serial_begin<FF_THREADS>(red, n_params);
    const SlabSerial serial{red, n, h};
    for (int turn = 0; turn < FF_WAVES; turn++) {
        if (wid == turn) each(serial);
        __syncthreads();
    }
    slab_serial_store<FF_THREADS>(red, n_params, slabs, grad_weights_direct);
}

constexpr int FP_PAIRS = 4;
constexpr int FP_THREADS = 2 * FP_PAIRS * 64;

struct MidEpilogue {
    const float* grad_sigma;
    const half_t* h16;
    half_t* grad_h16;
    float density_scale;
};

template <int WIDTH, int NHM, typename Sink>
__device__ __forceinline__ void recompute_hidden(const half8_t* __restrict__ fimg_lane, uint32_t in_kb, const unsigned char* xb, bool in_planar,
                                                 int lane, Sink&& sink) {
    constexpr int NIB = Shape<WIDTH>::NIB, NKB = Shape<WIDTH>::NKB;
    float16_t acc[NIB];
#pragma unroll
    for (int ib = 0; ib < NIB; ib++) acc[ib] = zero16();
    for (uint32_t kb = 0; kb < in_kb; kb++) {
        const half8_t x = tile_x(xb, kb, in_planar, lane);
#pragma unroll
        for (int ib = 0; ib < NIB; ib++) acc[ib] = mfma(fimg_lane[(ib * in_kb + kb) * 64], x, acc[ib]);
    }
    const half8_t* fhid = fimg_lane + (size_t)NIB * in_kb * 64;
    half8_t hid[NKB];
#pragma unroll
    for (int l = 0; l <= NHM; l++) {
        pack_hidden_relu<WIDTH>(acc, hid);
        sink(l, hid);
        if (l == NHM) break;
        const half8_t* wl = fhid + (size_t)l * NIB * NKB * 64;
#pragma unroll
        for (int ib = 0; ib < NIB; ib++) {
            acc[ib] = zero16();
#pragma unroll
            for (int kb = 0; kb < NKB; kb++) acc[ib] = mfma(wl[(ib * NKB + kb) * 64], hid[kb], acc[ib]);
        }
    }
}

template <int N>
__device__ __forceinline__ void wait_vmcnt() {
    asm volatile("s_waitcnt vmcnt(%0)" ::"n"(N) : "memory");
}

template <int WIDTH, int IN_JB, int NHM , bool RELU, bool RECOMP = false>
__global__ __launch_bounds__(FP_THREADS) __attribute__((amdgpu_waves_per_eu(2, 2)))
void k_ffmlp_backward_paired(const half_t* __restrict__ grad, const half_t* __restrict__ inputs, const half_t* __restrict__ weights,
                             const half_t* __restrict__ forward_buffer, uint32_t n_tiles, uint32_t in_dim, uint32_t num_layers, uint32_t act,
                             bool with_dx, half_t* __restrict__ grad_inputs, float* __restrict__ slabs,
                             half_t* __restrict__ grad_weights_direct, bool in_planar, bool dx_planar, uint32_t pf_depth, MidEpilogue mid,
                             uint32_t lds_bytes, bool serial_flush) {
    static_assert(NHM == 1 || NHM == 2, "the paired backward covers 2- and 3-layer networks");
    constexpr int NIB = Shape<WIDTH>::NIB, NKB = Shape<WIDTH>::NKB;
    extern __shared__ __attribute__((aligned(16))) unsigned char smem[];
    half8_t* img = reinterpret_cast<half8_t*>(smem);
    const uint32_t nfrag = bwd_frag_count<WIDTH>(in_dim, num_layers, with_dx);
    const uint32_t in_kb = in_dim / 16;
    const uint32_t ffrag = RECOMP ? NIB * in_kb + (num_layers - 1) * NIB * NKB : 0u;
    const int lane = threadIdx.x & 63, wid = threadIdx.x >> 6;
    const int n = lane & 31, h = lane >> 5;
    const int pair = wid & (FP_PAIRS - 1), role = wid / FP_PAIRS;
    const size_t layer_stride = (size_t)n_tiles * NKB * 64;
    const half8_t* fb = reinterpret_cast<const half8_t*>(forward_buffer);
    const size_t rows = (size_t)n_tiles * FF_TILE;
    const uint32_t act_layers = RECOMP ? 0u : num_layers;
    const uint32_t tile_frags = 1 + act_layers * NKB + in_kb;
    unsigned char* pf_base = smem + (size_t)(nfrag + ffrag) * 1024 + (size_t)pair * pf_depth * tile_frags * 1024;
    half8_t* scratch = reinterpret_cast<half8_t*>(smem + (size_t)(nfrag + ffrag) * 1024 + (size_t)FP_PAIRS * pf_depth * tile_frags * 1024 +
                                                  (size_t)pair * NHM * NKB * 1024) + lane;
    const uint32_t base_step = gridDim.x * FP_PAIRS;
    uint32_t cur = 0;
    const uint32_t tile_loads = tile_dma_count<WIDTH>(act_layers, in_dim, in_planar);
    auto prefetch = [&](uint32_t buffer, uint32_t tile) {
        const uint32_t issued = prefetch_tile<WIDTH>(pf_base + (size_t)buffer * tile_frags * 1024, tile, grad, fb, inputs, act_layers, layer_stride,
                                                     rows, in_dim, in_planar, lane, n, h);
        NGP_BOUNDS(issued == tile_loads);
        (void)issued;
    };
    if (role == 0) {
        for (uint32_t d = 0; d + 1 < (pf_depth > 1 ? pf_depth : 2u); d++)
            if (blockIdx.x * FP_PAIRS + d * base_step + pair < n_tiles) prefetch(d, blockIdx.x * FP_PAIRS + d * base_step + pair);
    }
    build_backward_image<WIDTH>(img, weights, in_dim, num_layers, with_dx);
    if (RECOMP) build_forward_image<WIDTH>(img + (size_t)nfrag * 64, weights, in_dim, num_layers, 0, ffrag);
    const Selectors sel = make_selectors(n, h);
    __syncthreads();

    const half8_t* img_out = img + lane;
    const half8_t* img_hid = img_out + (size_t)NIB * 64;
    const half8_t* img_in = img_hid + (size_t)(num_layers - 1) * NIB * NKB * 64;
    const half8_t* fimg = img + (size_t)nfrag * 64 + lane;
    static_assert(tile_dma_count<64>(0, 32, false) == 3u && tile_dma_count<64>(0, 32, true) == 9u && tile_dma_count<64>(2, 32, false) == 11u &&
                  tile_dma_count<64>(2, 32, true) == 17u, "the enumerated vmcnt immediates below are the DMA counts of the three-deep shapes");
    const bool deep = pf_depth == 3 && (tile_loads == 3u || tile_loads == 9u || tile_loads == 11u || tile_loads == 17u);
    auto next_tile_buffer = [&](uint32_t base) -> const unsigned char* {
        if (role == 0) {
            if (deep && base + base_step + pair < n_tiles) {
                switch (tile_loads) {
                    case 3u: wait_vmcnt<3>(); break;
                    case 9u: wait_vmcnt<9>(); break;
                    case 11u: wait_vmcnt<11>(); break;
                    default: wait_vmcnt<17>(); break;
                }
            } else {
                wait_vmcnt<0>();
            }
        }
        __syncthreads();
        const unsigned char* tb = pf_base + (size_t)cur * tile_frags * 1024;
        if (pf_depth > 1) {
            const uint32_t ahead = pf_depth - 1;
            const uint32_t fill = cur == 0 ? pf_depth - 1 : cur - 1;
            cur = cur + 1 == pf_depth ? 0u : cur + 1;
            if (role == 0 && base + ahead * base_step + pair < n_tiles) prefetch(fill, base + ahead * base_step + pair);
        }
        return tb;
    };
    auto end_of_round = [&](uint32_t base) {
        if (pf_depth == 1) {
            __syncthreads();
            if (role == 0 && base + base_step + pair < n_tiles) prefetch(0, base + base_step + pair);
        }
    };
    float* red = reinterpret_cast<float*>(smem);
    const SlabLayout lay{WIDTH, in_dim, num_layers};
    const uint32_t n_params = lay.n_params();
    const uint32_t base_out = lay.out();
    const uint32_t base_top = lay.hidden(num_layers - 1);
    const uint32_t base_low = lay.hidden(1);
    const SlabSerial serial{red, n, h};
    constexpr bool whole = slab_fits_whole<WIDTH, IN_JB, NHM>;
    const SlabPart part_a = whole ? SlabPart{0u, n_params} : SlabPart{base_low, n_params - base_low}, part_b = SlabPart{0u, base_low};
    auto pass = [&](SlabPart p, auto&& stage_fn) {
        slab_sum_pass<FP_THREADS>(red, lds_bytes, p, pair, slabs + (size_t)blockIdx.x * n_params, grad_weights_direct, n, h, stage_fn);
    };

    if (role == 0) {
        float16_t gw_out[NIB], gw_top[NIB][NIB];
#pragma unroll
        for (int jb = 0; jb < NIB; jb++) gw_out[jb] = zero16();
#pragma unroll
        for (int ib = 0; ib < NIB; ib++)
#pragma unroll
            for (int jb = 0; jb < NIB; jb++) gw_top[ib][jb] = zero16();
        for (uint32_t base = blockIdx.x * FP_PAIRS; base < n_tiles; base += base_step) {
            const unsigned char* tb = next_tile_buffer(base);
            if (base + pair < n_tiles) {
                const half8_t* tfrag = reinterpret_cast<const half8_t*>(tb) + lane;
                const half8_t dy = tfrag[0];
                half8_t a_top[NKB], a_below[NKB];
                if constexpr (RECOMP) {
                    recompute_hidden<WIDTH, NHM>(fimg, in_kb, tb + 1024, in_planar, lane, [&](int l, const half8_t (&hid)[NKB]) {
                        if (l == NHM) {
#pragma unroll
                            for (int kb = 0; kb < NKB; kb++) a_top[kb] = hid[kb];
                        } else if (l == NHM - 1) {
#pragma unroll
                            for (int kb = 0; kb < NKB; kb++) a_below[kb] = hid[kb];
                        }
                    });
                } else {
#pragma unroll
                    for (int kb = 0; kb < NKB; kb++) a_top[kb] = tfrag[(1 + NHM * NKB + kb) * 64];
#pragma unroll
                    for (int kb = 0; kb < NKB; kb++) a_below[kb] = tfrag[(1 + (NHM - 1) * NKB + kb) * 64];
                }
                half8_t aT[NIB][2], zT[NIB][2];
                transpose_hidden<WIDTH>(a_top, sel, aT);
                {
                    half8_t yT[2];
                    pack_transposed(mfma(dy, sel.out, zero16()), yT);
#pragma unroll
                    for (int g = 0; g < 2; g++)
#pragma unroll
                        for (int jb = 0; jb < NIB; jb++) gw_out[jb] = mfma(yT[g], aT[jb][g], gw_out[jb]);
                }
                float16_t acc[NIB];
                dgrad_out<WIDTH>(img_out, dy, acc);
                half8_t dz[NKB];
                activation_transfer<WIDTH, RELU>(act, acc, a_top, dz);
                transpose_hidden<WIDTH>(dz, sel, zT);
                transpose_hidden<WIDTH>(a_below, sel, aT);
                wgrad_blocks(zT, aT, gw_top);
            }
            end_of_round(base);
        }
        auto each = [&](const auto& sink) {
#pragma unroll
            for (int ib = 0; ib < NIB; ib++)
#pragma unroll
                for (int jb = 0; jb < NIB; jb++) sink.put(gw_top[ib][jb], base_top, WIDTH, ib, jb, WIDTH, WIDTH);
#pragma unroll
            for (int jb = 0; jb < NIB; jb++) sink.put(gw_out[jb], base_out, WIDTH, 0, jb, 16, WIDTH);
        };
        if (slab_staged_paired<WIDTH, IN_JB, NHM> && !serial_flush) {
            pass(part_a, each);
            if constexpr (!whole) pass(part_b, [](const SlabCopy&) {});
            return;
        }
        slab_serial_begin<FP_THREADS>(red, n_params);
        for (int turn = 0; turn < FP_PAIRS; turn++) {
            if (pair == turn) each(serial);
            __syncthreads();
        }
    } else {
        float16_t gw_in[NIB][IN_JB], gw_low[NHM == 2 ? NIB : 1][NHM == 2 ? NIB : 1];
#pragma unroll
        for (int ib = 0; ib < NIB; ib++)
#pragma unroll
            for (int jb = 0; jb < IN_JB; jb++) gw_in[ib][jb] = zero16();
        if constexpr (NHM == 2) {
#pragma unroll
            for (int ib = 0; ib < NIB; ib++)
#pragma unroll
                for (int jb = 0; jb < NIB; jb++) gw_low[ib][jb] = zero16();
        }
        for (uint32_t base = blockIdx.x * FP_PAIRS; base < n_tiles; base += base_step) {
            const unsigned char* tb = next_tile_buffer(base);
            const uint32_t tile = base + pair;
            if (tile < n_tiles) {
                const half8_t* tfrag = reinterpret_cast<const half8_t*>(tb) + lane;
                const half8_t dy = tfrag[0];
                half8_t a_prev[NKB];
                const half8_t* afrag = RECOMP ? scratch : tfrag + 64;
                if constexpr (RECOMP) {
                    recompute_hidden<WIDTH, NHM>(fimg, in_kb, tb + 1024, in_planar, lane, [&](int l, const half8_t (&hid)[NKB]) {
                        if (l == NHM) {
#pragma unroll
                            for (int kb = 0; kb < NKB; kb++) a_prev[kb] = hid[kb];
                        } else {
#pragma unroll
                            for (int kb = 0; kb < NKB; kb++) scratch[(l * NKB + kb) * 64] = hid[kb];
                        }
                    });
                    asm volatile("" ::: "memory");
                } else {
#pragma unroll
                    for (int kb = 0; kb < NKB; kb++) a_prev[kb] = afrag[(NHM * NKB + kb) * 64];
                }
                float16_t acc[NIB];
                dgrad_out<WIDTH>(img_out, dy, acc);
                half8_t dz[NKB];
                half8_t aT[NIB][2], zT[NIB][2];
                activation_transfer<WIDTH, RELU>(act, acc, a_prev, dz);
#pragma unroll
                for (int kb = 0; kb < NKB; kb++) a_prev[kb] = afrag[((NHM - 1) * NKB + kb) * 64];
                dgrad_hidden<WIDTH>(img_hid, dz, acc);
                if constexpr (NHM == 2) {
                    activation_transfer<WIDTH, RELU>(act, acc, a_prev, dz);
#pragma unroll
                    for (int kb = 0; kb < NKB; kb++) a_prev[kb] = afrag[kb * 64];
                    transpose_hidden<WIDTH>(dz, sel, zT);
                    transpose_hidden<WIDTH>(a_prev, sel, aT);
                    wgrad_blocks(zT, aT, gw_low);
                    const half8_t* wl = img_hid + (size_t)NIB * NKB * 64;
#pragma unroll
                    for (int ib = 0; ib < NIB; ib++) {
                        acc[ib] = zero16();
#pragma unroll
                        for (int kb = 0; kb < NKB; kb++) acc[ib] = mfma(wl[(ib * NKB + kb) * 64], dz[kb], acc[ib]);
                    }
                }
                activation_transfer<WIDTH, RELU>(act, acc, a_prev, dz);
                transpose_hidden<WIDTH>(dz, sel, zT);
#pragma unroll
                for (int jb = 0; jb < IN_JB; jb++) {
                    float16_t t = zero16();
#pragma unroll
                    for (int e = 0; e < 2; e++) {
                        const uint32_t kb = 2 * jb + e;
                        if (kb < in_kb) t = mfma(tile_x(tb + (size_t)(1 + act_layers * NKB) * 1024, kb, in_planar, lane), sel.nat[e], t);
                    }
                    half8_t xT[2];
                    pack_transposed(t, xT);
#pragma unroll
                    for (int g = 0; g < 2; g++)
#pragma unroll
                        for (int ib = 0; ib < NIB; ib++) gw_in[ib][jb] = mfma(zT[ib][g], xT[g], gw_in[ib][jb]);
                }
                if (with_dx && mid.grad_sigma) {
                    if constexpr (IN_JB == 1) {
                        float16_t dx = zero16();
#pragma unroll
                        for (int kb = 0; kb < NKB; kb++) dx = mfma(img_in[kb * 64], dz[kb], dx);
                        const size_t srow = (size_t)tile * FF_TILE + n;
                        half_t v2[4], v3[4];
#pragma unroll
                        for (int j = 0; j < 4; j++) { v2[j] = (half_t)dx[8 + j]; v3[j] = (half_t)dx[12 + j]; }
                        const float sib2 = __shfl_xor((float)v2[3], 32, 64), sib3 = __shfl_xor((float)v3[3], 32, 64);
                        half4_t a, b;
                        if (h == 0) {
                            const float x0 = (float)mid.h16[srow * 16];
                            const float gs = (mid.density_scale * mid.grad_sigma[srow]) * (x0 != x0 ? x0 : expf(fminf(15.0f, fmaxf(-15.0f, x0))));
                            a = half4_t{to_half_rne(gs), v2[0], v2[1], v2[2]};
                            b = half4_t{(half_t)sib2, v3[0], v3[1], v3[2]};
                        } else {
                            a = half4_t{(half_t)sib2, v2[0], v2[1], v2[2]};
                            b = half4_t{(half_t)sib3, v3[0], v3[1], v3[2]};
                        }
                        half_t* grow = mid.grad_h16 + srow * 16 + 4 * h;
                        *reinterpret_cast<half4_t*>(grow) = a;
                        *reinterpret_cast<half4_t*>(grow + 8) = b;
                    }
                } else if (with_dx) {
                    store_dx<WIDTH, IN_JB>(img_in, dz, grad_inputs, tile, n, h, in_dim, rows, dx_planar);
                }
            }
            end_of_round(base);
        }
        auto each_in = [&](const auto& sink) {
#pragma unroll
            for (int ib = 0; ib < NIB; ib++)
#pragma unroll
                for (int jb = 0; jb < IN_JB; jb++) sink.put(gw_in[ib][jb], lay.in(), in_dim, ib, jb, WIDTH, in_dim);
        };
        auto each_low = [&](const auto& sink) {
            if constexpr (NHM == 2) {
#pragma unroll
                for (int ib = 0; ib < NIB; ib++)
#pragma unroll
                    for (int jb = 0; jb < NIB; jb++) sink.put(gw_low[ib][jb], base_low, WIDTH, ib, jb, WIDTH, WIDTH);
            }
        };
        if (slab_staged_paired<WIDTH, IN_JB, NHM> && !serial_flush) {
            pass(part_a, [&](const SlabCopy& c) {
                if constexpr (whole) each_in(c);
                each_low(c);
            });
            if constexpr (!whole) pass(part_b, each_in);
            return;
        }
        slab_serial_begin<FP_THREADS>(red, n_params);
        for (int turn = 0; turn < FP_PAIRS; turn++) {
            if (pair == turn) {
                each_in(serial);
                each_low(serial);
            }
            __syncthreads();
        }
    }
    slab_serial_store<FP_THREADS>(red, n_params, slabs, grad_weights_direct);
}


template <int WIDTH>
__device__ __forceinline__ void fwd_matmul_range(uint32_t m, uint32_t in_dim, uint32_t num_layers, uint32_t& first, uint32_t& count) {
    constexpr uint32_t NIB = Shape<WIDTH>::NIB, NKB = Shape<WIDTH>::NKB;
    const uint32_t in_kb = in_dim / 16;
    if (m == 0) { first = 0; count = NIB * in_kb; }
    else if (m < num_layers) { first = NIB * in_kb + (m - 1) * NIB * NKB; count = NIB * NKB; }
    else { first = NIB * in_kb + (num_layers - 1) * NIB * NKB; count = NKB; }
}

template <int WIDTH, bool TRAIN>
__global__ __launch_bounds__(FF_THREADS) void k_ffmlp_forward_layered(const half_t* __restrict__ inputs, const half_t* __restrict__ weights,
                                                                      half_t* __restrict__ buffer, half_t* __restrict__ outputs, uint32_t n_tiles,
                                                                      uint32_t in_dim, uint32_t num_layers, uint32_t act, uint32_t out_act,
                                                                      bool in_planar) {
    constexpr int NIB = Shape<WIDTH>::NIB, NKB = Shape<WIDTH>::NKB;
    extern __shared__ __attribute__((aligned(16))) unsigned char smem[];
    half8_t* img = reinterpret_cast<half8_t*>(smem);
    const int lane = threadIdx.x & 63, wid = threadIdx.x >> 6;
    const int n = lane & 31, h = lane >> 5;
    const uint32_t in_kb = in_dim / 16;
    const size_t rows = (size_t)n_tiles * FF_TILE;
    const size_t layer_stride = (size_t)n_tiles * NKB * 64;
    half8_t* buf = reinterpret_cast<half8_t*>(buffer);
    const half8_t* a = img + lane;
    for (uint32_t m = 0; m <= num_layers; m++) {
        uint32_t first, count;
        fwd_matmul_range<WIDTH>(m, in_dim, num_layers, first, count);
        __syncthreads();
        build_forward_image<WIDTH>(img, weights, in_dim, num_layers, first, count);
        __syncthreads();
        for (uint32_t tile = blockIdx.x * FF_WAVES + wid; tile < n_tiles; tile += gridDim.x * FF_WAVES) {
                const half8_t* src = buf + (TRAIN ? (size_t)(m ? m - 1 : 0) * layer_stride : 0) + (size_t)tile * NKB * 64 + lane;
            if (m == num_layers) {
                float16_t o = zero16();
#pragma unroll
                for (int kb = 0; kb < NKB; kb++) o = mfma(a[kb * 64], src[kb * 64], o);
                half4_t lo, hi;
#pragma unroll
                for (int c = 0; c < 4; c++) {
                    lo[c] = (half_t)act_forward(out_act, o[c]);
                    hi[c] = (half_t)act_forward(out_act, o[4 + c]);
                }
                half_t* orow = outputs + ((size_t)tile * FF_TILE + n) * 16 + 4 * h;
                *reinterpret_cast<half4_t*>(orow) = lo;
                *reinterpret_cast<half4_t*>(orow + 8) = hi;
                continue;
            }
            float16_t acc[NIB];
#pragma unroll
            for (int ib = 0; ib < NIB; ib++) acc[ib] = zero16();
            if (m == 0) {
                const size_t srow = (size_t)tile * FF_TILE + n;
                for (uint32_t kb = 0; kb < in_kb; kb++) {
                    const half8_t x = load_features8(inputs, in_planar, rows, srow, in_dim, 16 * kb + 8 * h);
#pragma unroll
                    for (int ib = 0; ib < NIB; ib++) acc[ib] = mfma(a[(ib * in_kb + kb) * 64], x, acc[ib]);
                }
            } else {
#pragma unroll
                for (int kb = 0; kb < NKB; kb++) {
                    const half8_t hk = src[kb * 64];
#pragma unroll
                    for (int ib = 0; ib < NIB; ib++) acc[ib] = mfma(a[(ib * NKB + kb) * 64], hk, acc[ib]);
                }
            }
            half8_t* dst = buf + (TRAIN ? (size_t)m * layer_stride : 0) + (size_t)tile * NKB * 64 + lane;
#pragma unroll
            for (int kb = 0; kb < NKB; kb++) {
                half8_t f;
#pragma unroll
                for (int j = 0; j < 8; j++) f[j] = (half_t)act_forward(act, acc[kb >> 1][(kb & 1) * 8 + j]);
                dst[kb * 64] = f;
            }
        }
        __threadfence();
    }
}

template <int WIDTH, bool RELU>
__global__ __launch_bounds__(FF_THREADS) void k_ffmlp_dgrad_layered(const half_t* __restrict__ grad, const half_t* __restrict__ weights,
                                                                    const half_t* __restrict__ forward_buffer, half_t* __restrict__ backward_buffer,
                                                                    uint32_t n_tiles, uint32_t in_dim, uint32_t num_layers, uint32_t act, bool with_dx,
                                                                    half_t* __restrict__ grad_inputs, bool dx_planar) {
    constexpr int NIB = Shape<WIDTH>::NIB, NKB = Shape<WIDTH>::NKB;
    extern __shared__ __attribute__((aligned(16))) unsigned char smem[];
    half8_t* img = reinterpret_cast<half8_t*>(smem);
    const int lane = threadIdx.x & 63, wid = threadIdx.x >> 6;
    const int n = lane & 31, h = lane >> 5;
    const size_t rows = (size_t)n_tiles * FF_TILE;
    const size_t layer_stride = (size_t)n_tiles * NKB * 64;
    const half8_t* fb = reinterpret_cast<const half8_t*>(forward_buffer);
    half8_t* bb = reinterpret_cast<half8_t*>(backward_buffer);
    const half8_t* a = img + lane;
    const uint32_t in_jb = (in_dim + 31) / 32;
    const uint32_t passes = num_layers + (with_dx ? 1u : 0u);
    for (uint32_t p = 0; p < passes; p++) {
        uint32_t first, count;
        if (p == 0) { first = 0; count = NIB; }
        else if (p < num_layers) { first = NIB + (p - 1) * NIB * NKB; count = NIB * NKB; }
        else { first = NIB + (num_layers - 1) * NIB * NKB; count = in_jb * NKB; }
        __syncthreads();
// ... 189 lines not shown
    NGP_REQUIRE(num_layers >= 2, NGP_ERR_INVALID, "%s: num_layers should be larger than 2 (3 matmuls), but got %u", fn, num_layers);
    NGP_REQUIRE(B % 128 == 0, NGP_ERR_INVALID, "%s: batch size must be 128 * m, but got %u", fn, B);
    return NGP_OK;
}

static int raise_lds(const void* kern, size_t lds, const char* what) {
    if (lds > 64 * 1024) {
        hipError_t e = hipFuncSetAttribute(kern, hipFuncAttributeMaxDynamicSharedMemorySize, (int)lds);
        NGP_REQUIRE(e == hipSuccess, NGP_ERR_LAUNCH, "%s: cannot raise the dynamic LDS limit: %s", what, hipGetErrorString(e));
    }
    return NGP_OK;
}

static int reduce_slabs(const void* slabs, uint32_t n_slabs, uint32_t n_params, void* grad_weights, hipStream_t st, const char* what) {
    SlabSets sets = {};
    const uint32_t blocks = slab_set(sets, 0, slabs, n_slabs, n_params, grad_weights, false);
    NGP_LAUNCH(k_ffmlp_reduce_slabs_pair, dim3(blocks), dim3(RS_PARAMS * RS_GROUPS), 0, st, sets, (float*)nullptr);
    return check_launch(what);
}

template <int WIDTH>
static size_t forward_image_bytes(uint32_t in_dim, uint32_t num_layers) {
    return (size_t)fwd_frag_count<WIDTH>(in_dim, num_layers) * 1024;
}

template <int WIDTH, bool TRAIN>
static int launch_forward_layered(const void* inputs, const void* weights, uint32_t B, uint32_t in_dim, uint32_t num_layers, uint32_t act,
                                  uint32_t out_act, void* buffer, void* outputs, uint32_t flags, hipStream_t st) {
    constexpr int NIB = Shape<WIDTH>::NIB, NKB = Shape<WIDTH>::NKB;
    const uint32_t n_tiles = B / FF_TILE;
    uint32_t frags = NIB * (in_dim / 16);
    if (frags < (uint32_t)(NIB * NKB)) frags = NIB * NKB;
    const size_t lds = (size_t)frags * 1024;
    NGP_REQUIRE(lds <= 152 * 1024, NGP_ERR_INVALID, "ffmlp: one %u x %u layer (%zu B) exceeds the LDS of a CU", (unsigned)WIDTH, in_dim, lds);
    NGP_REQUIRE(buffer, NGP_ERR_INVALID, "ffmlp: this network shape needs the %s the reference passes", TRAIN ? "forward_buffer" : "inference_buffer [B, hidden]");
    auto kern = k_ffmlp_forward_layered<WIDTH, TRAIN>;
    int rc = raise_lds(reinterpret_cast<const void*>(kern), lds, "ffmlp");
    if (rc) return rc;
    const uint32_t per_cu = (uint32_t)((160 * 1024) / (lds + 1024));
    uint32_t blocks = (uint32_t)device_info().cus * (per_cu < 1 ? 1 : (per_cu > 2 ? 2 : per_cu));
    const uint32_t need = cdiv(n_tiles, FF_WAVES);
    if (blocks > need) blocks = need;
    NGP_LAUNCH(kern, dim3(blocks), dim3(FF_THREADS), lds, st, (const half_t*)inputs, (const half_t*)weights, (half_t*)buffer,
                       (half_t*)outputs, n_tiles, in_dim, num_layers, act, out_act, (flags & NGP_FF_INPUT_PLANAR) != 0);
    return check_launch(TRAIN ? "ffmlp_forward(layered)" : "ffmlp_inference(layered)");
}

template <int WIDTH, bool TRAIN>
static int launch_forward(const void* inputs, const void* weights, uint32_t B, uint32_t in_dim, uint32_t num_layers, uint32_t act,
                          uint32_t out_act, void* fwd, void* outputs, uint32_t flags, hipStream_t st) {
    const uint32_t n_tiles = B / FF_TILE;
    const size_t lds = forward_image_bytes<WIDTH>(in_dim, num_layers);
    if (WIDTH > 128 || lds > 152 * 1024 || (flags & NGP_FF_LAYERED))
        return launch_forward_layered<WIDTH, TRAIN>(inputs, weights, B, in_dim, num_layers, act, out_act, fwd, outputs, flags, st);
    if constexpr (WIDTH > 128) {
        return NGP_ERR_INVALID;
    } else {
    const bool plain = act == ACT_RELU && out_act == ACT_NONE;
    using forward_kernel_t = void (*)(const half_t*, const half_t*, half_t*, half_t*, uint32_t, uint32_t, uint32_t, uint32_t, uint32_t, bool);
    forward_kernel_t kern;
    if constexpr (WIDTH > 64) kern = plain ? k_ffmlp_forward_wide<WIDTH, TRAIN, true> : k_ffmlp_forward_wide<WIDTH, TRAIN, false>;
    else kern = plain ? k_ffmlp_forward<WIDTH, TRAIN, true> : k_ffmlp_forward<WIDTH, TRAIN, false>;
    int rc = raise_lds(reinterpret_cast<const void*>(kern), lds, "ffmlp");
    if (rc) return rc;
    const uint32_t per_cu = (uint32_t)((160 * 1024) / (lds + 1024));
    uint32_t blocks = (uint32_t)device_info().cus * (per_cu < 1 ? 1 : (per_cu > 4 ? 4 : per_cu));
    const uint32_t need = cdiv(n_tiles, FF_WAVES);
    if (blocks > need) blocks = need;
    const hipError_t e = NGP_LAUNCH_STATUS(kern, dim3(blocks), dim3(FF_THREADS), lds, st, (const half_t*)inputs, (const half_t*)weights, (half_t*)fwd,
                                           (half_t*)outputs, n_tiles, in_dim, num_layers, act, out_act, (flags & NGP_FF_INPUT_PLANAR) != 0);
    NGP_REQUIRE(e == hipSuccess, NGP_ERR_LAUNCH, "ffmlp: kernel launch failed: %s", hipGetErrorString(e));
    return check_launch(TRAIN ? "ffmlp_forward" : "ffmlp_inference");
    }
}

constexpr uint32_t WG_MAX_CHUNKS = 64;

template <int WIDTH>
static int launch_backward_layered(const void* grad, const void* inputs, const void* weights, const void* fwd, uint32_t B, uint32_t in_dim,
                                   uint32_t num_layers, uint32_t act, bool with_dx, void* backward_buffer, void* grad_inputs,
                                   void* grad_weights, uint32_t flags, void* workspace, size_t workspace_bytes, hipStream_t st) {
    constexpr int NIB = Shape<WIDTH>::NIB, NKB = Shape<WIDTH>::NKB;
    const bool in_planar = (flags & NGP_FF_INPUT_PLANAR) != 0, dx_planar = (flags & NGP_FF_DX_PLANAR) != 0;
    const uint32_t n_tiles = B / FF_TILE;
    const uint32_t in_jb = (in_dim + 31) / 32;
    uint32_t frags = NIB * NKB;
    if (with_dx && frags < in_jb * NKB) frags = in_jb * NKB;
    const size_t lds = (size_t)frags * 1024;
    NGP_REQUIRE(lds <= 152 * 1024, NGP_ERR_INVALID, "ffmlp_backward: one %u x %u layer (%zu B) exceeds the LDS of a CU", (unsigned)WIDTH, in_dim, lds);
    const void* dk = act == ACT_RELU ? reinterpret_cast<const void*>(k_ffmlp_dgrad_layered<WIDTH, true>)
                                     : reinterpret_cast<const void*>(k_ffmlp_dgrad_layered<WIDTH, false>);
    int rc = raise_lds(dk, lds, "ffmlp_backward");
    if (rc) return rc;
    const uint32_t per_cu = (uint32_t)((160 * 1024) / (lds + 1024));
    uint32_t blocks = (uint32_t)device_info().cus * (per_cu < 1 ? 1 : (per_cu > 2 ? 2 : per_cu));
    const uint32_t need = cdiv(n_tiles, FF_WAVES);
    if (blocks > need) blocks = need;
    if (act == ACT_RELU)
        NGP_LAUNCH((k_ffmlp_dgrad_layered<WIDTH, true>), dim3(blocks), dim3(FF_THREADS), lds, st, (const half_t*)grad, (const half_t*)weights,
                           (const half_t*)fwd, (half_t*)backward_buffer, n_tiles, in_dim, num_layers, act, with_dx, (half_t*)grad_inputs, dx_planar);
    else
        NGP_LAUNCH((k_ffmlp_dgrad_layered<WIDTH, false>), dim3(blocks), dim3(FF_THREADS), lds, st, (const half_t*)grad, (const half_t*)weights,
                           (const half_t*)fwd, (half_t*)backward_buffer, n_tiles, in_dim, num_layers, act, with_dx, (half_t*)grad_inputs, dx_planar);
    rc = check_launch("ffmlp_backward(dgrad)");
    if (rc) return rc;
    const uint32_t n_params = ff_param_count(in_dim, WIDTH, num_layers);
    const uint32_t jobs = wgrad_jobs_of(NIB, in_jb) + (num_layers - 1) * wgrad_jobs_of(NIB, NIB) + wgrad_jobs_of(1, NIB);
    uint32_t chunks = 1;
    if (workspace) {
        chunks = (uint32_t)(workspace_bytes / ((size_t)n_params * 4));
        const uint32_t want = cdiv((uint32_t)device_info().cus * 4u, jobs);
        if (chunks > want) chunks = want;
        if (chunks > WG_MAX_CHUNKS) chunks = WG_MAX_CHUNKS;
        const uint32_t by_tiles = cdiv(n_tiles, 2 * FF_WAVES);
        if (chunks > by_tiles) chunks = by_tiles;
        if (chunks < 1) chunks = 1;
    }
    const uint32_t tiles_per_chunk = cdiv(n_tiles, chunks);
    chunks = cdiv(n_tiles, tiles_per_chunk);
    const bool direct = chunks == 1;
    NGP_LAUNCH(k_ffmlp_wgrad<WIDTH>, dim3(chunks, jobs), dim3(FF_THREADS), 0, st, (const half_t*)grad, (const half_t*)inputs, (const half_t*)fwd,
                       (const half_t*)backward_buffer, n_tiles, in_dim, num_layers, in_planar, tiles_per_chunk, direct ? (float*)nullptr : (float*)workspace,
                       direct ? (half_t*)grad_weights : (half_t*)nullptr);
    rc = check_launch("ffmlp_backward(wgrad)");
    if (rc || direct) return rc;
    return reduce_slabs(workspace, chunks, n_params, grad_weights, st, "ffmlp_backward(reduce)");
}

static bool ff_register_resident(uint32_t in_dim, uint32_t hidden, uint32_t num_layers) {
    return (hidden == 32 || hidden == 64) && num_layers <= 4 && in_dim <= 64;
}
static bool ff_leaves_slabs(uint32_t in_dim, uint32_t hidden, uint32_t num_layers) {
    return ff_register_resident(in_dim, hidden, num_layers) && num_layers >= 2 && num_layers <= 3;
}

template <int WIDTH>
static uint32_t backward_slab_count(uint32_t B, uint32_t in_dim, uint32_t num_layers) {
    const uint32_t n_params = SlabLayout{WIDTH, in_dim, num_layers}.n_params();
    const size_t buf_bytes = (size_t)num_layers * B * WIDTH * sizeof(half_t);
    uint32_t blocks = (uint32_t)device_info().cus;
    const uint32_t need = cdiv(B / FF_TILE, FF_WAVES);
    if (blocks > need) blocks = need;
    const size_t fit = buf_bytes / ((size_t)n_params * 4);
    if (blocks > fit) blocks = (uint32_t)fit;
    return blocks;
}

struct BackwardLds {
    size_t image, tile;
    uint32_t pf_depth;
    size_t stage, total;
};
template <int WIDTH, int IN_JB, int NHM>
static BackwardLds backward_lds_plan(uint32_t in_dim, uint32_t num_layers, bool with_dx, uint32_t flags, bool recompute) {
    constexpr int NKB = Shape<WIDTH>::NKB;
    static_assert(FF_WAVES == FP_PAIRS, "one tile stream per wave or per pair: the same number of tile buffers");
    const SlabLayout lay{WIDTH, in_dim, num_layers};
    BackwardLds p;
    const uint32_t nfrag = bwd_frag_count<WIDTH>(in_dim, num_layers, with_dx);
    size_t scratch = 0;
    if (recompute) {
        p.image = (size_t)(nfrag + fwd_frag_count<WIDTH>(in_dim, num_layers) - NKB) * 1024;
        p.tile = (size_t)(1 + in_dim / 16) * 1024;
        p.pf_depth = 3;
        scratch = (size_t)FP_PAIRS * NHM * NKB * 1024;
    } else {
        p.image = (size_t)nfrag * 1024;
        p.tile = (size_t)(1 + num_layers * NKB + in_dim / 16) * 1024;
        p.pf_depth = p.image + 2 * FF_WAVES * p.tile > 160 * 1024 ? 1 : 2;
    }
    const bool paired = (NHM == 1 || NHM == 2) && !(flags & NGP_FF_SINGLE_WAVE);
    const bool staged = !(flags & NGP_FF_SERIAL_FLUSH) && (paired ? slab_staged_paired<WIDTH, IN_JB, NHM> : slab_staged_single<WIDTH, IN_JB, NHM>);
    p.stage = staged ? slab_stage_bytes(slab_fits_whole<WIDTH, IN_JB, NHM>, lay) : 0;
    p.total = p.image + (size_t)p.pf_depth * FF_WAVES * p.tile + scratch;
    if (p.total < (size_t)lay.n_params() * 4) p.total = (size_t)lay.n_params() * 4;
    if (p.total < p.stage) p.total = p.stage;
    return p;
}

template <typename Launch>
static int launch_and_reduce(const void* kern, size_t lds, uint32_t blocks, bool defer, void* backward_buffer, void* grad_weights, uint32_t n_params,
                             hipStream_t st, Launch&& launch) {
    int rc = raise_lds(kern, lds, "ffmlp_backward");
    if (rc) return rc;
    const bool direct = blocks <= 1;
    launch(dim3(direct ? 1 : blocks), direct ? (float*)nullptr : (float*)backward_buffer, direct ? (half_t*)grad_weights : (half_t*)nullptr);
    rc = check_launch("ffmlp_backward");
    if (rc || direct || defer) return rc;
    return reduce_slabs(backward_buffer, blocks, n_params, grad_weights, st, "ffmlp_backward(reduce)");
}

template <int WIDTH, int IN_JB, int NHM, bool RELU>
static int launch_backward_t(const void* grad, const void* inputs, const void* weights, const void* fwd, uint32_t B, uint32_t in_dim,
                           uint32_t num_layers, uint32_t act, bool with_dx, void* backward_buffer, void* grad_inputs,
                           void* grad_weights, uint32_t flags, hipStream_t st, const MidEpilogue* mid_in) {
    const bool in_planar = (flags & NGP_FF_INPUT_PLANAR) != 0, dx_planar = (flags & NGP_FF_DX_PLANAR) != 0;
    const bool defer = (flags & NGP_FF_DEFER_REDUCE) != 0, serial = (flags & NGP_FF_SERIAL_FLUSH) != 0;
    const MidEpilogue mid = mid_in ? *mid_in : MidEpilogue{nullptr, nullptr, nullptr, 0.0f};
    const uint32_t n_tiles = B / FF_TILE;
    const uint32_t n_params = SlabLayout{WIDTH, in_dim, num_layers}.n_params();
    const BackwardLds lds = backward_lds_plan<WIDTH, IN_JB, NHM>(in_dim, num_layers, with_dx, flags, false);
    NGP_REQUIRE(lds.total <= 160 * 1024, NGP_ERR_INVALID, "ffmlp_backward: LDS need (%zu B) exceeds 160 KiB", lds.total);
    const uint32_t blocks = backward_slab_count<WIDTH>(B, in_dim, num_layers);
    const half_t *g = (const half_t*)grad, *x = (const half_t*)inputs, *w = (const half_t*)weights;
    if (flags & NGP_FF_RECOMPUTE) {
        if constexpr (WIDTH == 64 && IN_JB == 1 && RELU && (NHM == 1 || NHM == 2)) {
            NGP_REQUIRE(in_dim == 32 && !(flags & NGP_FF_SINGLE_WAVE), NGP_ERR_INVALID, "ffmlp_backward: NGP_FF_RECOMPUTE needs input_dim 32 and the paired kernel");
            const BackwardLds lds_r = backward_lds_plan<WIDTH, IN_JB, NHM>(in_dim, num_layers, with_dx, flags, true);
            NGP_REQUIRE(lds_r.total <= 160 * 1024, NGP_ERR_INVALID, "ffmlp_backward: LDS need (%zu B) exceeds 160 KiB", lds_r.total);
            auto pk = k_ffmlp_backward_paired<WIDTH, IN_JB, NHM, RELU, true>;
            return launch_and_reduce(reinterpret_cast<const void*>(pk), lds_r.total, blocks, defer, backward_buffer, grad_weights, n_params, st,
                                     [&](dim3 grid, float* slabs, half_t* direct) {
                NGP_LAUNCH(pk, grid, dim3(FP_THREADS), lds_r.total, st, g, x, w, (const half_t*)nullptr, n_tiles, in_dim, num_layers, act, with_dx,
                                   (half_t*)grad_inputs, slabs, direct, in_planar, dx_planar, lds_r.pf_depth, mid, (uint32_t)lds_r.total, serial);
            });
        } else {
            NGP_REQUIRE(false, NGP_ERR_INVALID, "ffmlp_backward: NGP_FF_RECOMPUTE serves 64-wide ReLU networks with 32 inputs and 2 or 3 layers");
        }
    }
    if constexpr (NHM == 1 || NHM == 2) {
        if (!(flags & NGP_FF_SINGLE_WAVE)) {
            auto pk = k_ffmlp_backward_paired<WIDTH, IN_JB, NHM, RELU>;
            return launch_and_reduce(reinterpret_cast<const void*>(pk), lds.total, blocks, defer, backward_buffer, grad_weights, n_params, st,
                                     [&](dim3 grid, float* slabs, half_t* direct) {
                NGP_LAUNCH(pk, grid, dim3(FP_THREADS), lds.total, st, g, x, w, (const half_t*)fwd, n_tiles, in_dim, num_layers, act, with_dx,
                                   (half_t*)grad_inputs, slabs, direct, in_planar, dx_planar, lds.pf_depth, mid, (uint32_t)lds.total, serial);
            });
        }
    }
    NGP_REQUIRE(!mid.grad_sigma && !defer, NGP_ERR_INVALID, "ffmlp_backward: this extension needs the paired kernel (2 or 3 layers)");
    auto kern = k_ffmlp_backward<WIDTH, IN_JB, NHM, RELU>;
    return launch_and_reduce(reinterpret_cast<const void*>(kern), lds.total, blocks, false, backward_buffer, grad_weights, n_params, st,
                             [&](dim3 grid, float* slabs, half_t* direct) {
        NGP_LAUNCH(kern, grid, dim3(FF_THREADS), lds.total, st, g, x, w, (const half_t*)fwd, n_tiles, in_dim, num_layers, act, with_dx,
                           (half_t*)grad_inputs, slabs, direct, in_planar, dx_planar, lds.pf_depth, (uint32_t)lds.total, serial);
    });
}

template <int WIDTH, int IN_JB, int NHM>
static int launch_backward(const void* grad, const void* inputs, const void* weights, const void* fwd, uint32_t B, uint32_t in_dim,
                           uint32_t num_layers, uint32_t act, bool with_dx, void* backward_buffer, void* grad_inputs,
                           void* grad_weights, uint32_t flags, hipStream_t st, const MidEpilogue* mid = nullptr) {
    if (act == ACT_RELU)
        return launch_backward_t<WIDTH, IN_JB, NHM, true>(grad, inputs, weights, fwd, B, in_dim, num_layers, act, with_dx, backward_buffer,
                                                          grad_inputs, grad_weights, flags, st, mid);
    return launch_backward_t<WIDTH, IN_JB, NHM, false>(grad, inputs, weights, fwd, B, in_dim, num_layers, act, with_dx, backward_buffer,
                                                       grad_inputs, grad_weights, flags, st, mid);
}

}

using namespace ngp;

#define FF_WIDTHS(CALL)                  \
    switch (hidden_dim) {                \
        case 16: return CALL(16);        \
        case 32: return CALL(32);        \
        case 64: return CALL(64);        \
        case 128: return CALL(128);      \
        default: return CALL(256);       \
    }

extern "C" int ngp_ffmlp_forward_ex(const void* inputs, const void* weights, uint32_t B, uint32_t input_dim, uint32_t output_dim,
                                    uint32_t hidden_dim, uint32_t num_layers, uint32_t activation, uint32_t output_activation,
                                    void* forward_buffer, void* outputs, uint32_t flags, ngp_stream_t stream) {
    int rc = check_ff_args("ffmlp_forward", B, input_dim, output_dim, hidden_dim, num_layers);
    if (rc) return rc;
    if (B == 0) return NGP_OK;
    NGP_REQUIRE(inputs && weights && forward_buffer && outputs, NGP_ERR_INVALID, "ffmlp_forward: NULL tensor");
    hipStream_t st = as_stream(stream);
#define FF_FWD(W) launch_forward<W, true>(inputs, weights, B, input_dim, num_layers, activation, output_activation, forward_buffer, outputs, flags, st)
    FF_WIDTHS(FF_FWD)
#undef FF_FWD
}

extern "C" int ngp_ffmlp_inference_ex(const void* inputs, const void* weights, uint32_t B, uint32_t input_dim, uint32_t output_dim,
                                      uint32_t hidden_dim, uint32_t num_layers, uint32_t activation, uint32_t output_activation,
                                      void* inference_buffer, void* outputs, uint32_t flags, ngp_stream_t stream) {
    int rc = check_ff_args("ffmlp_inference", B, input_dim, output_dim, hidden_dim, num_layers);
    if (rc) return rc;
    if (B == 0) return NGP_OK;
    NGP_REQUIRE(inputs && weights && outputs, NGP_ERR_INVALID, "ffmlp_inference: NULL tensor");
    hipStream_t st = as_stream(stream);
#define FF_INF(W) launch_forward<W, false>(inputs, weights, B, input_dim, num_layers, activation, output_activation, inference_buffer, outputs, flags, st)
    FF_WIDTHS(FF_INF)
#undef FF_INF
}

extern "C" size_t ngp_ffmlp_backward_workspace_bytes(uint32_t B, uint32_t input_dim, uint32_t hidden_dim, uint32_t num_layers) {
    if (ff_register_resident(input_dim, hidden_dim, num_layers) || B == 0) return 0;
    return (size_t)WG_MAX_CHUNKS * SlabLayout{hidden_dim, input_dim, num_layers}.n_params() * sizeof(float);
}

extern "C" int ngp_ffmlp_backward_ws(const void* grad, const void* inputs, const void* weights, const void* forward_buffer, uint32_t B,
                                     uint32_t input_dim, uint32_t output_dim, uint32_t hidden_dim, uint32_t num_layers, uint32_t activation,
                                     uint32_t output_activation, int calc_grad_inputs, void* backward_buffer, void* grad_inputs,
                                     void* grad_weights, uint32_t flags, void* workspace, size_t workspace_bytes, ngp_stream_t stream) {
    (void)output_activation;
    int rc = check_ff_args("ffmlp_backward", B, input_dim, output_dim, hidden_dim, num_layers);
    if (rc) return rc;
    if (B == 0) {
        if (grad_weights && !(flags & NGP_FF_DEFER_REDUCE)) {
            const size_t n_w = (size_t)hidden_dim * ((size_t)input_dim + (size_t)hidden_dim * (num_layers - 1) + (size_t)output_dim);
            hipError_t e = ::ngp::memset_async(grad_weights, 0, n_w * sizeof(half_t), as_stream(stream));
            NGP_REQUIRE(e == hipSuccess, NGP_ERR_LAUNCH, "ffmlp_backward: hipMemsetAsync failed: %s", hipGetErrorString(e));
        }
        return NGP_OK;
    }
    NGP_REQUIRE(grad && inputs && weights && (forward_buffer || (flags & NGP_FF_RECOMPUTE)) && backward_buffer && grad_weights, NGP_ERR_INVALID,
                "ffmlp_backward: NULL tensor");
    NGP_REQUIRE(!calc_grad_inputs || grad_inputs, NGP_ERR_INVALID, "ffmlp_backward: grad_inputs is NULL but calc_grad_inputs is set");
    hipStream_t st = as_stream(stream);
    const bool dx = calc_grad_inputs != 0;
    const bool fast = ff_register_resident(input_dim, hidden_dim, num_layers) && !(flags & NGP_FF_LAYERED);
    NGP_REQUIRE(fast || !(flags & NGP_FF_RECOMPUTE), NGP_ERR_INVALID, "ffmlp_backward: NGP_FF_RECOMPUTE serves 64-wide ReLU networks with 32 inputs and 2 or 3 layers");
    NGP_REQUIRE(fast || !(flags & NGP_FF_DEFER_REDUCE), NGP_ERR_INVALID, "ffmlp_backward: NGP_FF_DEFER_REDUCE needs a 2- or 3-layer network of width 32 / 64");
    if (!fast) {
#define FF_LAY(W) launch_backward_layered<W>(grad, inputs, weights, forward_buffer, B, input_dim, num_layers, activation, dx, backward_buffer, grad_inputs, grad_weights, flags, workspace, workspace_bytes, st)
        FF_WIDTHS(FF_LAY)
#undef FF_LAY
    }
    const uint32_t in_jb = (input_dim + 31) / 32;
#define FF_BWD(W, J, N) \
    return launch_backward<W, J, N>(grad, inputs, weights, forward_buffer, B, input_dim, num_layers, activation, dx, backward_buffer, grad_inputs, grad_weights, flags, st)
#define FF_BWD_N(W, J)                      \
    switch (num_layers - 1) {               \
        case 1: FF_BWD(W, J, 1);            \
        case 2: FF_BWD(W, J, 2);            \
        default: FF_BWD(W, J, 3);           \
    }
    if (hidden_dim == 64) {
        if (in_jb == 1) { FF_BWD_N(64, 1) }
        FF_BWD_N(64, 2)
    }
    if (in_jb == 1) { FF_BWD_N(32, 1) }
    FF_BWD_N(32, 2)
#undef FF_BWD_N
#undef FF_BWD
}

extern "C" int ngp_ffmlp_backward_ex(const void* grad, const void* inputs, const void* weights, const void* forward_buffer, uint32_t B,
                                     uint32_t input_dim, uint32_t output_dim, uint32_t hidden_dim, uint32_t num_layers, uint32_t activation,
                                     uint32_t output_activation, int calc_grad_inputs, void* backward_buffer, void* grad_inputs,
                                     void* grad_weights, uint32_t flags, ngp_stream_t stream) {
    return ngp_ffmlp_backward_ws(grad, inputs, weights, forward_buffer, B, input_dim, output_dim, hidden_dim, num_layers, activation,
                                 output_activation, calc_grad_inputs, backward_buffer, grad_inputs, grad_weights, flags, nullptr, 0, stream);
}


extern "C" uint32_t ngp_ffmlp_backward_slab_count(uint32_t B, uint32_t input_dim, uint32_t hidden_dim, uint32_t num_layers) {
    if (!ff_leaves_slabs(input_dim, hidden_dim, num_layers) || B == 0) return 0;
    const uint32_t blocks = hidden_dim == 64 ? backward_slab_count<64>(B, input_dim, num_layers) : backward_slab_count<32>(B, input_dim, num_layers);
    return blocks <= 1 ? 0u : blocks;
}

extern "C" int ngp_ffmlp_reduce_slabs_pair(const void* slabs_a, uint32_t n_slabs_a, uint32_t n_params_a, void* grad_weights_a,
                                           const void* slabs_b, uint32_t n_slabs_b, uint32_t n_params_b, void* grad_weights_b,
                                           float* found_inf, ngp_stream_t stream) {
    SlabSets sets = {};
    const uint32_t blocks_a = slab_set(sets, 0, slabs_a, n_slabs_a, n_params_a, grad_weights_a, found_inf != nullptr);
    const uint32_t blocks_b = slab_set(sets, 1, slabs_b, n_slabs_b, n_params_b, grad_weights_b, found_inf != nullptr);
    if (blocks_a + blocks_b == 0) return NGP_OK;
    NGP_REQUIRE((!blocks_a || ((slabs_a || !n_slabs_a) && grad_weights_a)) && (!blocks_b || ((slabs_b || !n_slabs_b) && grad_weights_b)),
                NGP_ERR_INVALID, "ffmlp_reduce_slabs_pair: NULL tensor");
    NGP_LAUNCH(k_ffmlp_reduce_slabs_pair, dim3(blocks_a + blocks_b), dim3(RS_PARAMS * RS_GROUPS), 0, as_stream(stream), sets, found_inf);
    return check_launch("ffmlp_reduce_slabs_pair");
}

extern "C" int ngp_network_backward_color(const void* grad_out16, const void* color_in, const void* w_color, const void* forward_buffer_color,
                                          uint32_t M, uint32_t num_layers_color, void* backward_buffer, const float* grad_sigma,
                                          const void* h16, float density_scale, void* grad_h16, void* grad_w_color, uint32_t flags,
                                          ngp_stream_t stream) {
    NGP_REQUIRE(num_layers_color == 2 || num_layers_color == 3, NGP_ERR_INVALID,
                "network_backward_color: 2 or 3 layers (got %u); use ngp_ffmlp_backward_ex + ngp_pipeline_mid_backward", num_layers_color);
    NGP_REQUIRE(!(flags & ~(NGP_FF_DEFER_REDUCE | NGP_FF_RECOMPUTE | NGP_FF_SERIAL_FLUSH)), NGP_ERR_INVALID,
                "network_backward_color: only NGP_FF_DEFER_REDUCE, NGP_FF_RECOMPUTE and NGP_FF_SERIAL_FLUSH are accepted");
    int rc = check_ff_args("network_backward_color", M, 32, 16, 64, num_layers_color);
    if (rc) return rc;
    if (M == 0) return NGP_OK;
    NGP_REQUIRE(grad_out16 && color_in && w_color && (forward_buffer_color || (flags & NGP_FF_RECOMPUTE)) && backward_buffer && grad_sigma && h16 &&
                    grad_h16 && grad_w_color,
                NGP_ERR_INVALID, "network_backward_color: NULL tensor");
    const MidEpilogue mid{grad_sigma, (const half_t*)h16, (half_t*)grad_h16, density_scale};
    if (num_layers_color == 2)
        return launch_backward<64, 1, 1>(grad_out16, color_in, w_color, forward_buffer_color, M, 32, 2, ACT_RELU, true, backward_buffer, nullptr,
                                         grad_w_color, flags, as_stream(stream), &mid);
    return launch_backward<64, 1, 2>(grad_out16, color_in, w_color, forward_buffer_color, M, 32, 3, ACT_RELU, true, backward_buffer, nullptr,
                                     grad_w_color, flags, as_stream(stream), &mid);
}

extern "C" int ngp_network_forward(const void* enc, const float* dirs, uint32_t M, uint32_t M_valid, const void* w_sigma, const void* w_color,
                                   uint32_t num_layers_sigma, uint32_t num_layers_color, float density_scale, int training,
                                   void* forward_buffer_sigma, void* h16, float* sigma, void* color_in, void* forward_buffer_color,
                                   float* rgb, uint32_t flags, ngp_stream_t stream) {
    return ngp_network_forward_rows(enc, dirs, M, M_valid, w_sigma, w_color, num_layers_sigma, num_layers_color, density_scale, training,
                                    forward_buffer_sigma, h16, sigma, color_in, forward_buffer_color, rgb, flags, nullptr, stream);
}

extern "C" int ngp_network_forward_rows(const void* enc, const float* dirs, uint32_t M, uint32_t M_valid, const void* w_sigma, const void* w_color,
                                        uint32_t num_layers_sigma, uint32_t num_layers_color, float density_scale, int training,
                                        void* forward_buffer_sigma, void* h16, float* sigma, void* color_in, void* forward_buffer_color,
                                        float* rgb, uint32_t flags, const uint32_t* rows_dev, ngp_stream_t stream) {
    NGP_REQUIRE(M % 128 == 0, NGP_ERR_INVALID, "network_forward: sample count must be 128 * m, but got %u", M);
    NGP_REQUIRE(num_layers_sigma >= 2 && num_layers_color >= 2, NGP_ERR_INVALID, "network_forward: num_layers should be larger than 2");
    if (M == 0) return NGP_OK;
    NGP_REQUIRE(enc && dirs && w_sigma && w_color && sigma && rgb, NGP_ERR_INVALID, "network_forward: NULL tensor");
    NGP_REQUIRE(!training || (h16 && color_in && (forward_buffer_sigma != nullptr) == (forward_buffer_color != nullptr)), NGP_ERR_INVALID,
                "network_forward: the training variant needs h16 and color_in, and both forward buffers or (NGP_FF_RECOMPUTE backward) neither");
    const size_t lds = forward_image_bytes<64>(32, num_layers_sigma) + forward_image_bytes<64>(32, num_layers_color);
    NGP_REQUIRE(lds <= 152 * 1024, NGP_ERR_INVALID, "network_forward: weights (%zu B) exceed the LDS of a CU", lds);
#ifndef NGP_NETFWD_TRAIN_WAVES
#define NGP_NETFWD_TRAIN_WAVES 4
#endif
#ifndef NGP_NETFWD_INFER_WAVES
#define NGP_NETFWD_INFER_WAVES 4
#endif
#ifndef NGP_NETFWD_TRAIN_TILES
#define NGP_NETFWD_TRAIN_TILES 1
#endif
#ifndef NGP_NETFWD_INFER_TILES
#define NGP_NETFWD_INFER_TILES 1
#endif
    constexpr int TW = NGP_NETFWD_TRAIN_WAVES, IW = NGP_NETFWD_INFER_WAVES, TT = NGP_NETFWD_TRAIN_TILES, IT = NGP_NETFWD_INFER_TILES;
    const void* kern = training ? reinterpret_cast<const void*>(k_network_forward<true, TW, TT>) : reinterpret_cast<const void*>(k_network_forward<false, IW, IT>);
    int rc = raise_lds(kern, lds, "network_forward");
    if (rc) return rc;
    const uint32_t n_tiles = M / FF_TILE;
    const uint32_t waves = training ? TW : IW, nt = training ? TT : IT;
    const uint32_t by_lds = (uint32_t)((160 * 1024) / (lds + 1024)), by_waves = (nt == 1 ? 16u : 12u) / waves;
#ifndef NGP_NETFWD_PER_CU
#define NGP_NETFWD_PER_CU 4u
#endif
    uint32_t per_cu = by_lds < by_waves ? by_lds : by_waves;
    per_cu = per_cu < 1 ? 1 : (per_cu > NGP_NETFWD_PER_CU ? NGP_NETFWD_PER_CU : per_cu);
    uint32_t blocks = (uint32_t)device_info().cus * per_cu;
    const uint32_t need = cdiv(cdiv(n_tiles, nt), waves);
    if (blocks > need) blocks = need;
    hipStream_t st = as_stream(stream);
    const bool planar = (flags & NGP_FF_INPUT_PLANAR) != 0;
    if (training)
        NGP_LAUNCH((k_network_forward<true, TW, TT>), dim3(blocks), dim3(TW * 64), lds, st, (const half_t*)enc, planar, dirs, M_valid, (const half_t*)w_sigma,
                           (const half_t*)w_color, (half_t*)forward_buffer_sigma, (half_t*)h16, sigma, (half_t*)color_in, (half_t*)forward_buffer_color, rgb,
                           n_tiles, num_layers_sigma, num_layers_color, density_scale, rows_dev);
    else
        NGP_LAUNCH((k_network_forward<false, IW, IT>), dim3(blocks), dim3(IW * 64), lds, st, (const half_t*)enc, planar, dirs, M_valid, (const half_t*)w_sigma,
                           (const half_t*)w_color, (half_t*)nullptr, (half_t*)nullptr, sigma, (half_t*)nullptr, (half_t*)nullptr, rgb, n_tiles,
                           num_layers_sigma, num_layers_color, density_scale, rows_dev);
    return check_launch("network_forward");
}

extern "C" int ngp_ffmlp_forward(const void* inputs, const void* weights, uint32_t B, uint32_t input_dim, uint32_t output_dim,
                                 uint32_t hidden_dim, uint32_t num_layers, uint32_t activation, uint32_t output_activation,
                                 void* forward_buffer, void* outputs, ngp_stream_t stream) {
    return ngp_ffmlp_forward_ex(inputs, weights, B, input_dim, output_dim, hidden_dim, num_layers, activation, output_activation,
                                forward_buffer, outputs, 0u, stream);
}
extern "C" int ngp_ffmlp_inference(const void* inputs, const void* weights, uint32_t B, uint32_t input_dim, uint32_t output_dim,
                                   uint32_t hidden_dim, uint32_t num_layers, uint32_t activation, uint32_t output_activation,
                                   void* inference_buffer, void* outputs, ngp_stream_t stream) {
    return ngp_ffmlp_inference_ex(inputs, weights, B, input_dim, output_dim, hidden_dim, num_layers, activation, output_activation,
                                  inference_buffer, outputs, 0u, stream);
}
extern "C" int ngp_ffmlp_backward(const void* grad, const void* inputs, const void* weights, const void* forward_buffer, uint32_t B,
                                  uint32_t input_dim, uint32_t output_dim, uint32_t hidden_dim, uint32_t num_layers, uint32_t activation,
                                  uint32_t output_activation, int calc_grad_inputs, void* backward_buffer, void* grad_inputs,
                                  void* grad_weights, ngp_stream_t stream) {
    return ngp_ffmlp_backward_ex(grad, inputs, weights, forward_buffer, B, input_dim, output_dim, hidden_dim, num_layers, activation,
                                 output_activation, calc_grad_inputs, backward_buffer, grad_inputs, grad_weights, 0u, stream);
}

static size_t g_splitk_request = 0;
extern "C" int ngp_allocate_splitk(size_t size) {
    g_splitk_request = size;
    return NGP_OK;
}
extern "C" int ngp_free_splitk(void) {
    g_splitk_request = 0;
    return NGP_OK;
}

#include "ffmlp_second.inc"
```

### torch-ngp_amd/fused.py

```python
import ctypes
import os
from collections import namedtuple

import numpy as np
import torch
from torch.autograd import Function

import _ngp_capi as capi
from optim import announce_overwrite, clean_deposits, resync_stale_shadows

_PLANAR_IN = capi.NGP_FF_INPUT_PLANAR
_PLANAR_DX = capi.NGP_FF_DX_PLANAR

NetCfg = namedtuple('NetCfg', 'bound L S H gridtype align interp nl_sigma nl_color training')
RenderCfg = namedtuple('RenderCfg', 'cascade grid_size min_near capacity perturb dt_gamma max_steps T_thresh density_scale bg_scalar')
Marched = namedtuple('Marched', 'xyzs dirs deltas rays nears fars ws')
Saved = namedtuple('Saved', 'xyzs offsets enc ws16 wc16 fb_s fb_c h16 color_in rgb sigma deltas rays weights_sum image_raw bg march_ws')
Bufs = namedtuple('Bufs', 'emb16 ws16 wc16 g_emb g_ws g_wc')


class GeoLoss(namedtuple('GeoLoss', 'lambda_distortion lambda_depth target_depth depth_weight', defaults=(0.0, 0.0, None, None))):
    __slots__ = ()

    def __new__(cls, lambda_distortion=0.0, lambda_depth=0.0, target_depth=None, depth_weight=None):
        lams = []
        for name, v in (('lambda_distortion', lambda_distortion), ('lambda_depth', lambda_depth)):
            if isinstance(v, bool) or not isinstance(v, (int, float)):
                raise TypeError(f'GeoLoss: {name} must be a host float, got {type(v).__name__}')
            v = float(v)
            if not (0.0 <= v < float('inf')):
                raise ValueError(f'GeoLoss: {name} must be finite and >= 0, got {v}')
            lams.append(v)
        if lams[1] > 0 and target_depth is None:
            raise ValueError('GeoLoss: lambda_depth > 0 needs target_depth')
        for name, t in (('target_depth', target_depth), ('depth_weight', depth_weight)):
            if t is not None and not (torch.is_tensor(t) and t.dtype == torch.float32 and t.dim() == 1 and t.is_contiguous()):
                raise ValueError(f'GeoLoss: {name} must be a contiguous [N] float32 tensor')
        return super().__new__(cls, lams[0], lams[1], target_depth, depth_weight)


def _grid_forward(x, emb16, offsets, enc, M, L, S, H, gridtype, align, interp, bound, costs, st):
    sel = getattr(emb16, '_ngp_sel', None)
    if sel is not None:
        capi.check(capi.lib.ngp_grid_encode_forward_sel(x.data_ptr(), emb16.data_ptr(), sel[0].data_ptr(), sel[1].data_ptr(), None, offsets.data_ptr(),
                                                         enc.data_ptr(), M, 3, 2, L, S, H, gridtype, align, interp, capi.NGP_F16, float(bound), costs, st))
    else:
        capi.check(capi.lib.ngp_grid_encode_forward_sched(x.data_ptr(), emb16.data_ptr(), offsets.data_ptr(), enc.data_ptr(), M, 3, 2, L, S, H,
                                                           None, gridtype, align, interp, capi.NGP_F16, float(bound), costs, st))


class _fused_ngp(Function):
    @staticmethod
    def forward(ctx, x, d, embeddings, w_sigma, w_color, offsets, cfg, bufs, density_scale=1.0):
        M = x.shape[0]
        dev = x.device
        st = capi.stream()
        x = x.contiguous()
        d = d.contiguous()
        half = dict(device=dev, dtype=torch.half)

        enc = torch.empty(cfg.L, M, 2, **half)
        costs = capi.ray_level_costs(cfg.L, cfg.S, cfg.H, 3.0 ** 0.5 / (1024.0 * max(float(cfg.bound), 1e-6))) if USE_BALANCED_FORWARD else None
        _grid_forward(x, bufs.emb16, offsets, enc, M, cfg.L, cfg.S, cfg.H, cfg.gridtype, cfg.align, cfg.interp, cfg.bound, costs, st)
        h16 = torch.empty(M, 16, **half)
        color_in = torch.empty(M, 32, **half)
        out16 = torch.empty(M, 16, **half)
        sigma = torch.empty(M, device=dev, dtype=torch.float32)
        rgb = torch.empty(M, 3, device=dev, dtype=torch.float32)
        d_valid = d.shape[0]
        if cfg.training:
            fb_s = torch.empty(cfg.nl_sigma, M, 64, **half)
            fb_c = torch.empty(cfg.nl_color, M, 64, **half)
        else:
            fb_s = fb_c = None
        assert not cfg.training or density_scale == 1.0, 'the backward of _fused_ngp knows no density scale (the fused training render folds it itself)'
        _network_forward(enc, d, d_valid, bufs.ws16, bufs.wc16, cfg.nl_sigma, cfg.nl_color, float(density_scale), cfg.training, fb_s, h16, sigma,
                         color_in, fb_c, out16, rgb, M, st)
        if cfg.training:
            ctx.save_for_backward(x, offsets, enc, bufs.ws16, bufs.wc16, fb_s, fb_c, h16, color_in, rgb)
            ctx.cfg = cfg
            ctx.n_emb = embeddings.shape[0]
            ctx.bufs = bufs
        return sigma, rgb

    @staticmethod
    def backward(ctx, grad_sigma, grad_rgb):
        x, offsets, enc, ws16, wc16, fb_s, fb_c, h16, color_in, rgb = ctx.saved_tensors
        cfg = ctx.cfg
        nl_sigma, nl_color = cfg.nl_sigma, cfg.nl_color
        M = x.shape[0]
        dev = x.device
        st = capi.stream()
        half = dict(device=dev, dtype=torch.half)
        grad_sigma = torch.zeros(M, device=dev) if grad_sigma is None else grad_sigma.contiguous().float()
        grad_rgb = torch.zeros(M, 3, device=dev) if grad_rgb is None else grad_rgb.contiguous().float()

        g_out16 = torch.empty(M, 16, **half)
        capi.check(capi.lib.ngp_pipeline_rgb_backward(grad_rgb.data_ptr(), rgb.data_ptr(), g_out16.data_ptr(), M, st))
        g_color_in = torch.empty(M, 32, **half)
        g_emb, g_ws, g_wc, deposited = _grad_targets(ctx.bufs, ctx.n_emb, dev)
        scratch_c = torch.empty(nl_color, M, 64, **half)
        capi.check(capi.lib.ngp_ffmlp_backward_ex(g_out16.data_ptr(), color_in.data_ptr(), wc16.data_ptr(), fb_c.data_ptr(), M, 32, 16, 64,
                                                   nl_color, 0, 6, 1, scratch_c.data_ptr(), g_color_in.data_ptr(), g_wc.data_ptr(), 0, st))
        g_h16 = g_out16
        capi.check(capi.lib.ngp_pipeline_mid_backward(grad_sigma.data_ptr(), h16.data_ptr(), g_color_in.data_ptr(), g_h16.data_ptr(), M, 1.0, st))
        g_enc = torch.empty(cfg.L, M, 2, **half)
        scratch_s = scratch_c[:nl_sigma]
        capi.check(capi.lib.ngp_ffmlp_backward_ex(g_h16.data_ptr(), enc.data_ptr(), ws16.data_ptr(), fb_s.data_ptr(), M, 32, 16, 64, nl_sigma,
                                                   0, 6, 1, scratch_s.data_ptr(), g_enc.data_ptr(), g_ws.data_ptr(), _PLANAR_IN | _PLANAR_DX, st))
        _grid_backward(g_enc, x, offsets, g_emb, M, cfg.L, cfg.S, cfg.H, cfg.gridtype, cfg.align, cfg.interp, cfg.bound, st)
        if deposited:
            return None, None, None, None, None, None, None, None, None
        return None, None, g_emb, g_ws, g_wc, None, None, None, None


USE_FUSED_NETWORK = True


def _network_forward(enc, dirs, d_valid, ws16, wc16, nl_sigma, nl_color, density_scale, training, fb_s, h16, sigma, color_in, fb_c, out16, rgb, M, st):
    if USE_FUSED_NETWORK:
        capi.check(capi.lib.ngp_network_forward(enc.data_ptr(), dirs.data_ptr(), M, d_valid, ws16.data_ptr(), wc16.data_ptr(), nl_sigma, nl_color,
                                                 float(density_scale), 1 if training else 0, capi.ptr(fb_s), capi.ptr(h16) if training else None,
                                                 sigma.data_ptr(), capi.ptr(color_in) if training else None, capi.ptr(fb_c), rgb.data_ptr(), _PLANAR_IN, st))
        return
    if training:
        capi.check(capi.lib.ngp_ffmlp_forward_ex(enc.data_ptr(), ws16.data_ptr(), M, 32, 16, 64, nl_sigma, 0, 6, fb_s.data_ptr(), h16.data_ptr(),
                                                  _PLANAR_IN, st))
    else:
        capi.check(capi.lib.ngp_ffmlp_inference_ex(enc.data_ptr(), ws16.data_ptr(), M, 32, 16, 64, nl_sigma, 0, 6, None, h16.data_ptr(), _PLANAR_IN, st))
    capi.check(capi.lib.ngp_pipeline_mid_forward(h16.data_ptr(), dirs.data_ptr(), sigma.data_ptr(), color_in.data_ptr(), M, d_valid, float(density_scale), st))
    if training:
        capi.check(capi.lib.ngp_ffmlp_forward_ex(color_in.data_ptr(), wc16.data_ptr(), M, 32, 16, 64, nl_color, 0, 6, fb_c.data_ptr(), out16.data_ptr(), 0, st))
    else:
        capi.check(capi.lib.ngp_ffmlp_inference_ex(color_in.data_ptr(), wc16.data_ptr(), M, 32, 16, 64, nl_color, 0, 6, None, out16.data_ptr(), 0, st))
    capi.check(capi.lib.ngp_pipeline_rgb_forward(out16.data_ptr(), rgb.data_ptr(), M, st))


def _grid_backward(g_enc, x, offsets, g_emb, M, L, S, H, gridtype, align, interp, bound, st, found_inf=None, slabs=None, overwrite=False,
                   table_adam=None):
    arr, ws, nbytes = capi.grid_backward_workspace(offsets, M, 3, 2, L, S, H, gridtype, align, capi.NGP_F16)
    if overwrite:
        slabs = slabs if slabs is not None else capi.SlabSets()
        slabs.overwrite_table = 1
    if table_adam is not None:
        if not overwrite:
            raise RuntimeError('fused: table_adam needs overwrite_table')
        slabs.table_adam = ctypes.cast(ctypes.pointer(table_adam), ctypes.c_void_p)
    if found_inf is not None and arr is None:
        raise RuntimeError('fused: the in-kernel non-finite sweep needs the host copy of the encoder offsets (call iteration_checks_gradients '
                           'outside stream capture first)')
    capi.check(capi.lib.ngp_grid_encode_backward_checked_slabs(g_enc.data_ptr(), x.data_ptr(), None, offsets.data_ptr(), capi.ptr(g_emb), M, 3, 2, L, S,
                                                                 H, None, None, gridtype, align, interp, capi.NGP_F16, float(bound),
                                                                 None if arr is None else ctypes.cast(arr, ctypes.c_void_p), capi.ptr(ws), nbytes,
                                                                 capi.ptr(found_inf), None if slabs is None else ctypes.cast(ctypes.pointer(slabs), ctypes.c_void_p),
                                                                 st))


def _half_weights(params, cast=True):
    sh = [getattr(p, '_ngp_fp16_pin', None) for p in params]
    if any(t is None for t in sh):
        resync_stale_shadows(params)
        sh = [t if t is not None else getattr(p, '_ngp_fp16', None) for t, p in zip(sh, params)]
    if cast:
        sh = [t if t is not None else p.detach().to(torch.half) for t, p in zip(sh, params)]
    return sh


def _operands(params, deposit, overwrite_table=False):
    sh = [getattr(p, '_ngp_fp16', None) for p in params]
    gr = [getattr(p, '_ngp_grad16', None) for p in params]
    if not deposit or any(t is None for t in sh + gr):
        return Bufs(*_half_weights(params), None, None, None)
    resync_stale_shadows(params)
    clean_deposits(params[1:] if overwrite_table else params)
    return Bufs(*sh, *gr)


def _grad_targets(bufs, n_emb, dev):
    if bufs.g_emb is not None:
        return bufs.g_emb, bufs.g_ws.view(-1), bufs.g_wc.view(-1), True
    return torch.zeros(n_emb, 2, device=dev, dtype=torch.half), torch.empty_like(bufs.ws16), torch.empty_like(bufs.wc16), False


def fused_ngp(x, d, encoder, sigma_net, color_net, bound, training, density_scale=1.0):
    cfg = network_cfg(encoder, sigma_net, color_net, bound, training)
    params = (encoder.embeddings, sigma_net.weights, color_net.weights)
    return _fused_ngp.apply(x, d, *params, encoder.offsets, cfg, _operands(params, deposit=training), density_scale)


def _render_train_march(rays_o, rays_d, bitfield, aabb, counter, cfg, rcfg, noise_seed=None, into=None):
    N = rays_o.shape[0]
    M = rcfg.capacity
    dev = rays_o.device
    st = capi.stream()
    f32 = dict(device=dev, dtype=torch.float32)
    if into is not None:
        (xyzs, dirs, deltas, rays, nears, fars, ws) = into
    else:
        nears = torch.empty(N, **f32)
        fars = torch.empty(N, **f32)
        xyzs = torch.empty(M, 3, **f32)
        dirs = torch.empty(M, 3, **f32)
        deltas = torch.empty(M, 2, **f32)
        rays = torch.empty(N, 3, device=dev, dtype=torch.int32)
        ws = torch.empty(capi.lib.ngp_march_rays_train_workspace_bytes(N), dtype=torch.uint8, device=dev)
    march_flags = capi.NGP_MARCH_RESET_COUNTER | capi.NGP_MARCH_ZERO_TAIL | (0 if USE_FUSED_SCAN else capi.NGP_MARCH_SCAN_LAUNCH)
    if rcfg.perturb and noise_seed is not None:
        noises, march_flags = noise_seed, march_flags | capi.NGP_MARCH_NOISE_FROM_SEED
    else:
        noises = torch.rand(N, **f32) if rcfg.perturb else torch.zeros(N, **f32)
    capi.check(capi.lib.ngp_march_rays_train_aabb(rays_o.data_ptr(), rays_d.data_ptr(), bitfield.data_ptr(), float(cfg.bound), float(rcfg.dt_gamma),
                                                   rcfg.max_steps, N, rcfg.cascade, rcfg.grid_size, M, aabb.data_ptr(), float(rcfg.min_near),
                                                   nears.data_ptr(), fars.data_ptr(), xyzs.data_ptr(), dirs.data_ptr(), deltas.data_ptr(),
                                                   rays.data_ptr(), counter.data_ptr(), noises.data_ptr(), ws.data_ptr(), march_flags, st))
    return Marched(xyzs, dirs, deltas, rays, nears, fars, ws)


def _render_train_network(marched, bufs, bg, offsets, cfg, rcfg, composite=True):
    xyzs, rays = marched.xyzs, marched.rays
    nl_sigma, nl_color = cfg.nl_sigma, cfg.nl_color
    N, M = rays.shape[0], rcfg.capacity
    dev = xyzs.device
    st = capi.stream()
    f32 = dict(device=dev, dtype=torch.float32)
    half = dict(device=dev, dtype=torch.half)
    enc = torch.empty(cfg.L, M, 2, **half)
    costs = capi.ray_level_costs(cfg.L, cfg.S, cfg.H, 3.0 ** 0.5 / (rcfg.max_steps * max(float(cfg.bound), 1e-6))) if USE_BALANCED_FORWARD else None
    _grid_forward(xyzs, bufs.emb16, offsets, enc, M, cfg.L, cfg.S, cfg.H, cfg.gridtype, cfg.align, cfg.interp, cfg.bound, costs, st)
    h16 = torch.empty(M, 16, **half)
    color_in = torch.empty(M, 32, **half)
    out16 = torch.empty(M, 16, **half)
    sigma = torch.empty(M, **f32)
    rgb = torch.empty(M, 3, **f32)
    if _recompute(nl_sigma, nl_color):
        fb_s = fb_c = None
    else:
        fb_s = torch.empty(nl_sigma, M, 64, **half)
        fb_c = torch.empty(nl_color, M, 64, **half)
    _network_forward(enc, marched.dirs, M, bufs.ws16, bufs.wc16, nl_sigma, nl_color, float(rcfg.density_scale), True, fb_s, h16, sigma, color_in, fb_c,
                     out16, rgb, M, st)
    saved = Saved(xyzs, offsets, enc, bufs.ws16, bufs.wc16, fb_s, fb_c, h16, color_in, rgb, sigma, marched.deltas, rays, weights_sum=None,
                  image_raw=None, bg=bg, march_ws=marched.ws)
    if not composite:
        return saved
    weights_sum = torch.empty(N, **f32)
    depth_raw = torch.empty(N, **f32)
    image_raw = torch.empty(N, 3, **f32)
    image = torch.empty(N, 3, **f32)
    depth = torch.empty(N, **f32)
    bg_mode = 2 if bg is not None else 1
    capi.check(capi.lib.ngp_composite_rays_train_forward_ex(sigma.data_ptr(), rgb.data_ptr(), marched.deltas.data_ptr(), rays.data_ptr(), M, N,
                                                             float(rcfg.T_thresh), weights_sum.data_ptr(), depth_raw.data_ptr(), image_raw.data_ptr(),
                                                             bg_mode, float(rcfg.bg_scalar), capi.ptr(bg), marched.nears.data_ptr(),
                                                             marched.fars.data_ptr(), image.data_ptr(), depth.data_ptr(), st))
    return image, depth, weights_sum, saved._replace(weights_sum=weights_sum, image_raw=image_raw)


def _render_train_backward(saved, cfg, rcfg, grad_image, grad_ws, g_emb, g_ws, g_wc, found_inf=None, overwrite=False, input_grads=False):
    s = saved
    M, N = s.xyzs.shape[0], s.rays.shape[0]
    dev = s.xyzs.device
    st = capi.stream()
    g_sigma = torch.empty(M, device=dev)
    g_rgb = torch.empty(M, 3, device=dev)
    bg_mode = 2 if s.bg is not None else 1
    capi.check(capi.lib.ngp_composite_rays_train_backward_ex(capi.ptr(grad_ws), grad_image.data_ptr(), s.sigma.data_ptr(), s.rgb.data_ptr(),
                                                              s.deltas.data_ptr(), s.rays.data_ptr(), s.weights_sum.data_ptr(),
                                                              s.image_raw.data_ptr(), M, N, float(rcfg.T_thresh), g_sigma.data_ptr(),
                                                              g_rgb.data_ptr(), bg_mode, float(rcfg.bg_scalar), capi.ptr(s.bg),
                                                              s.march_ws.data_ptr(), st))
    g_out16 = torch.empty(M, 16, device=dev, dtype=torch.half)
    capi.check(capi.lib.ngp_pipeline_rgb_backward(g_rgb.data_ptr(), s.rgb.data_ptr(), g_out16.data_ptr(), M, st))
    return _network_backward(saved, cfg, rcfg, g_sigma, g_out16, g_emb, g_ws, g_wc, found_inf, None, overwrite, input_grads=input_grads)


def _network_backward(saved, cfg, rcfg, g_sigma, g_out16, g_emb, g_ws, g_wc, found_inf=None, loss_job=None, overwrite=False, table_adam=None,
                      input_grads=False):
    if input_grads and saved.fb_c is None:
        raise RuntimeError('fused: gradients with respect to the rays need the stored activations of the MLPs; this render was run with '
                           'NGP_FUSED_RECOMPUTE=1 (NGP_FF_RECOMPUTE: no forward buffers) -- switch it off to refine poses')
    s = saved
    nl_sigma, nl_color, density_scale = cfg.nl_sigma, cfg.nl_color, rcfg.density_scale
    grid = (cfg.L, cfg.S, cfg.H, cfg.gridtype, cfg.align, cfg.interp, cfg.bound)
    M = s.xyzs.shape[0]
    st = capi.stream()
    half = dict(device=s.xyzs.device, dtype=torch.half)
    g_enc = torch.empty(cfg.L, M, 2, **half)
    g_color_in = None
    if USE_FUSED_MID and nl_color in (2, 3) and nl_sigma in (2, 3) and not input_grads:
        scratch_c = torch.empty(nl_color, M, 64, **half)
        scratch_s = torch.empty(nl_sigma, M, 64, **half)
        g_h16 = torch.empty(M, 16, **half)
        rc = capi.NGP_FF_RECOMPUTE if s.fb_c is None else 0
        capi.check(capi.lib.ngp_network_backward_color(g_out16.data_ptr(), s.color_in.data_ptr(), s.wc16.data_ptr(), capi.ptr(s.fb_c), M, nl_color,
                                                        scratch_c.data_ptr(), g_sigma.data_ptr(), s.h16.data_ptr(), float(density_scale),
                                                        g_h16.data_ptr(), g_wc.data_ptr(), capi.NGP_FF_DEFER_REDUCE | rc, st))
        capi.check(capi.lib.ngp_ffmlp_backward_ex(g_h16.data_ptr(), s.enc.data_ptr(), s.ws16.data_ptr(), capi.ptr(s.fb_s), M, 32, 16, 64, nl_sigma,
                                                   0, 6, 1, scratch_s.data_ptr(), g_enc.data_ptr(), g_ws.data_ptr(),
                                                   _PLANAR_IN | _PLANAR_DX | capi.NGP_FF_DEFER_REDUCE | rc, st))
        n_c, n_s = capi.lib.ngp_ffmlp_backward_slab_count(M, 32, 64, nl_color), capi.lib.ngp_ffmlp_backward_slab_count(M, 32, 64, nl_sigma)
        if USE_SLABS_IN_ACCUMULATE:
            err, loss = loss_job if loss_job is not None else (None, None)
            slabs = capi.SlabSets(scratch_c.data_ptr(), n_c, g_wc.numel(), g_wc.data_ptr(), scratch_s.data_ptr(), n_s, g_ws.numel(), g_ws.data_ptr(),
                                  capi.ptr(err), 0 if err is None else err.numel(), capi.ptr(loss))
            _grid_backward(g_enc, s.xyzs, s.offsets, g_emb, M, *grid, st, found_inf, slabs, overwrite, table_adam)
            return
        if loss_job is not None:
            raise RuntimeError('fused: a deferred loss sum needs the carried reductions (_carries_reductions)')
        capi.check(capi.lib.ngp_ffmlp_reduce_slabs_pair(scratch_c.data_ptr(), n_c, g_wc.numel(), g_wc.data_ptr(), scratch_s.data_ptr(), n_s, g_ws.numel(),
                                                         g_ws.data_ptr(), capi.ptr(found_inf), st))
    else:
        if found_inf is not None:
            raise RuntimeError('fused: found_inf needs the fused colour-head / slab-reduction path (see iteration_checks_gradients)')
        if loss_job is not None:
            raise RuntimeError('fused: a deferred loss sum needs the carried reductions (_carries_reductions)')
        g_color_in = torch.empty(M, 32, **half)
        scratch = torch.empty(max(nl_color, nl_sigma), M, 64, **half)
        capi.check(capi.lib.ngp_ffmlp_backward_ex(g_out16.data_ptr(), s.color_in.data_ptr(), s.wc16.data_ptr(), s.fb_c.data_ptr(), M, 32, 16, 64,
                                                   nl_color, 0, 6, 1, scratch.data_ptr(), g_color_in.data_ptr(), g_wc.data_ptr(), 0, st))
        g_h16 = g_out16
        capi.check(capi.lib.ngp_pipeline_mid_backward(g_sigma.data_ptr(), s.h16.data_ptr(), g_color_in.data_ptr(), g_h16.data_ptr(), M,
                                                       float(density_scale), st))
        capi.check(capi.lib.ngp_ffmlp_backward_ex(g_h16.data_ptr(), s.enc.data_ptr(), s.ws16.data_ptr(), s.fb_s.data_ptr(), M, 32, 16, 64, nl_sigma,
                                                   0, 6, 1, scratch[:nl_sigma].data_ptr(), g_enc.data_ptr(), g_ws.data_ptr(),
                                                   _PLANAR_IN | _PLANAR_DX, st))
    _grid_backward(g_enc, s.xyzs, s.offsets, g_emb, M, *grid, st, found_inf, None, overwrite, table_adam)
    return g_enc, g_color_in


def _ray_gradients(saved, cfg, g_enc, g_color_in, emb16, rays_o, rays_d):
    s = saved
    M, N = s.xyzs.shape[0], s.rays.shape[0]
    dev = s.xyzs.device
    st = capi.stream()
    sel = getattr(emb16, '_ngp_sel', None)
    if sel is not None:
        raise RuntimeError('fused: gradients with respect to the rays are not provided for a double-buffered table (optim.NGPAdam table fusion)')
    g_xyzs = torch.empty(M, 3, device=dev)
    capi.check(capi.lib.ngp_grid_input_gradient(g_enc.data_ptr(), s.xyzs.data_ptr(), emb16.data_ptr(), s.offsets.data_ptr(), M, 3, 2, cfg.L, cfg.S,
                                                cfg.H, cfg.gridtype, cfg.align, cfg.interp, capi.NGP_F16, float(cfg.bound), g_xyzs.data_ptr(), st))
    ts = torch.empty(M, device=dev)
    capi.check(capi.lib.ngp_ray_sample_ts(s.xyzs.data_ptr(), rays_o.data_ptr(), rays_d.data_ptr(), s.rays.data_ptr(), M, N, float(cfg.bound),
                                          ts.data_ptr(), st))
    grad_o = torch.empty(N, 3, device=dev)
    grad_d = torch.empty(N, 3, device=dev)
    capi.check(capi.lib.ngp_ray_points_backward(g_xyzs.data_ptr(), None, g_color_in.data_ptr(), s.xyzs.data_ptr(), ts.data_ptr(), rays_d.data_ptr(),
                                                s.rays.data_ptr(), M, N, float(cfg.bound), grad_o.data_ptr(), grad_d.data_ptr(), st))
    return grad_o, grad_d


class _fused_render_train(Function):
    @staticmethod
    def forward(ctx, rays_o, rays_d, embeddings, w_sigma, w_color, bg, offsets, bitfield, aabb, counter, cfg, rcfg, bufs):
        marched = _render_train_march(rays_o, rays_d, bitfield, aabb, counter, cfg, rcfg)
        image, depth, weights_sum, saved = _render_train_network(marched, bufs, bg, offsets, cfg, rcfg)
        ctx.ray_grads = bool(ctx.needs_input_grad[0] or ctx.needs_input_grad[1])
        if ctx.ray_grads and saved.fb_c is None:
            raise RuntimeError('fused: gradients with respect to the rays need the stored activations of the MLPs; NGP_FUSED_RECOMPUTE=1 '
                               '(NGP_FF_RECOMPUTE: no forward buffers) does not keep them -- switch it off to refine poses')
        ctx.save_for_backward(*saved, *((rays_o.contiguous(), rays_d.contiguous()) if ctx.ray_grads else ()))
        ctx.cfg, ctx.rcfg, ctx.n_emb, ctx.bufs = cfg, rcfg, embeddings.shape[0], bufs
        ctx.mark_non_differentiable(depth)
        return image, depth, weights_sum

    @staticmethod
    def backward(ctx, grad_image, grad_depth, grad_ws):
        n_saved = len(Saved._fields)
        saved = Saved(*ctx.saved_tensors[:n_saved])
        dev = saved.xyzs.device
        N = saved.rays.shape[0]
        grad_image = torch.zeros(N, 3, device=dev) if grad_image is None else grad_image.contiguous().float()
        grad_ws = None if grad_ws is None else grad_ws.contiguous().float()
        g_emb, g_ws, g_wc, deposited = _grad_targets(ctx.bufs, ctx.n_emb, dev)
        grad_o = grad_d = None
        if ctx.ray_grads:
            rays_o, rays_d = ctx.saved_tensors[n_saved:]
            g_enc, g_color_in = _render_train_backward(saved, ctx.cfg, ctx.rcfg, grad_image, grad_ws, g_emb, g_ws, g_wc, input_grads=True)
            grad_o, grad_d = _ray_gradients(saved, ctx.cfg, g_enc, g_color_in, ctx.bufs.emb16, rays_o, rays_d)
        else:
            _render_train_backward(saved, ctx.cfg, ctx.rcfg, grad_image, grad_ws, g_emb, g_ws, g_wc)
        if deposited:
            return (grad_o, grad_d) + (None,) * 11
        return grad_o, grad_d, g_emb, g_ws, g_wc, None, None, None, None, None, None, None, None


def network_cfg(encoder, sigma_net, color_net, bound, training):
    return NetCfg(float(bound), int(encoder.num_levels), float(np.log2(encoder.per_level_scale)), int(encoder.base_resolution),
                  int(encoder.gridtype_id), int(bool(encoder.align_corners)), int(encoder.interp_id), int(sigma_net.num_layers),
                  int(color_net.num_layers), bool(training))


def fused_render_train(model, rays_o, rays_d, box, counter, capacity, bg_color, perturb, dt_gamma, max_steps, T_thresh):
    cfg = network_cfg(model.encoder, model.sigma_net, model.color_net, model.bound, True)
    bg_t, rcfg = _render_cfg(model, capacity, bg_color, perturb, dt_gamma, max_steps, T_thresh)
    params = (model.encoder.embeddings, model.sigma_net.weights, model.color_net.weights)
    return _fused_render_train.apply(rays_o, rays_d, *params, bg_t, model.encoder.offsets, model.density_bitfield, box, counter, cfg, rcfg,
                                     _operands(params, deposit=True))


def _render_cfg(model, capacity, bg_color, perturb, dt_gamma, max_steps, T_thresh):
    bg_t, bg_s = (bg_color.contiguous().float().view(-1, 3), 0.0) if torch.is_tensor(bg_color) else (None, float(bg_color))
    rcfg = RenderCfg(int(model.cascade), int(model.grid_size), float(model.min_near), int(capacity), bool(perturb), float(dt_gamma),
                     int(max_steps), float(T_thresh), float(model.density_scale), bg_s)
    return bg_t, rcfg


@torch.no_grad()
def fused_train_iteration(model, rays_o, rays_d, target, box, counter, capacity, loss_scale, bg_color=1, perturb=False, dt_gamma=0,
                          max_steps=1024, T_thresh=1e-4, noise_seed=None, found_inf=None, overwrite_table=False, table_adam=None, geo_loss=None):
    march, rest = fused_train_iteration_split(model, rays_o, rays_d, target, box, counter, capacity, loss_scale, bg_color, perturb, dt_gamma,
                                              max_steps, T_thresh, noise_seed, found_inf, overwrite_table, table_adam, geo_loss)
    march()
    return rest()


def _table_adam_prefix(model, cfg, M):
    arr = capi.host_offsets(model.encoder.offsets)
    prefix = int(capi.lib.ngp_grid_table_adam_prefix(ctypes.cast(arr, ctypes.c_void_p), int(M), 3, 2, cfg.L, cfg.S, cfg.H, cfg.gridtype, cfg.align,
                                                     capi.NGP_F16))
    if prefix == 0xffffffff:
        raise RuntimeError('fused: table_adam: this batch / table shape cannot carry the sweep (ngp_grid_table_adam_prefix)')
    return prefix


def _table_adam_of(optimizer, model):
    if optimizer is None:
        return None
    if getattr(optimizer, 'fused_table', None) is not model.encoder.embeddings:
        raise RuntimeError('fused: table_adam: call optimizer.enable_table_fusion(model.encoder.embeddings) first')
    return optimizer.table_adam()


USE_BALANCED_FORWARD = True
USE_FUSED_CHECK = True
USE_FUSED_SCAN = True
USE_FUSED_MID = True
USE_FUSED_COMPOSITE = True
USE_OVERWRITE_TABLE = os.environ.get('NGP_FUSED_OVERWRITE_TABLE', '1') != '0'
USE_SLABS_IN_ACCUMULATE = os.environ.get('NGP_FUSED_SLABS_IN_ACCUMULATE', '1') != '0'
USE_RECOMPUTE = os.environ.get('NGP_FUSED_RECOMPUTE', '0') == '1'


def _carries_reductions(nl_sigma, nl_color):
    return bool(USE_SLABS_IN_ACCUMULATE and USE_FUSED_MID and nl_color in (2, 3) and nl_sigma in (2, 3))


def _recompute(nl_sigma, nl_color):
    return bool(USE_RECOMPUTE and USE_FUSED_NETWORK and USE_FUSED_MID and nl_color in (2, 3) and nl_sigma in (2, 3))


def iteration_checks_gradients(model):
    nl = (int(model.sigma_net.num_layers), int(model.color_net.num_layers))
    return bool(USE_FUSED_CHECK and USE_FUSED_MID and all(n in (2, 3) for n in nl) and capi.host_offsets(model.encoder.offsets) is not None)


def _train_iteration_rest(marched, bufs, bg_t, offsets, target, loss_scale, cfg, rcfg, found_inf=None, overwrite=False, table_adam=None,
                          geo_loss=None):
    if table_adam is not None and not (USE_FUSED_COMPOSITE and found_inf is not None and overwrite):
        raise RuntimeError('fused: table_adam needs the fused compositor, the in-kernel non-finite sweep (found_inf) and overwrite_table')
    if geo_loss is not None and not USE_FUSED_COMPOSITE:
        raise RuntimeError('fused: geo_loss needs the fused compositor (USE_FUSED_COMPOSITE)')
    g_emb, g_ws, g_wc = bufs.g_emb, bufs.g_ws.view(-1), bufs.g_wc.view(-1)
    if not USE_FUSED_COMPOSITE:
        image, depth, weights_sum, saved = _render_train_network(marched, bufs, bg_t, offsets, cfg, rcfg)
        loss = torch.empty(1, device=image.device, dtype=torch.float32)
        grad_image = torch.empty_like(image)
        capi.check(capi.lib.ngp_pipeline_mse_loss(image.data_ptr(), target.data_ptr(), image.numel(), capi.ptr(loss_scale), loss.data_ptr(),
                                                   grad_image.data_ptr(), capi.stream()))
        _render_train_backward(saved, cfg, rcfg, grad_image, None, g_emb, g_ws, g_wc, found_inf, overwrite)
        return loss, image, depth, weights_sum
    s = _render_train_network(marched, bufs, bg_t, offsets, cfg, rcfg, composite=False)
    N, M, dev = s.rays.shape[0], s.xyzs.shape[0], s.xyzs.device
    f32 = dict(device=dev, dtype=torch.float32)
    weights_sum, image, depth = torch.empty(N, **f32), torch.empty(N, 3, **f32), torch.empty(N, **f32)
    loss, ray_err = torch.empty(1, **f32), torch.empty(N, **f32)
    g_sigma = torch.empty(M, **f32)
    g_out16 = torch.empty(M, 16, device=dev, dtype=torch.half)
    defer = _carries_reductions(cfg.nl_sigma, cfg.nl_color)
    if geo_loss is not None:
        for name in ('target_depth', 'depth_weight'):
            t = getattr(geo_loss, name)
            if t is not None and (t.shape[0] != N or t.device != dev):
                raise RuntimeError(f'fused: geo_loss.{name} must be [{N}] float32 on {dev}')
        depth_raw, distortion = torch.empty(N, **f32), torch.empty(N, **f32)
        capi.check(capi.lib.ngp_composite_train_geo_loss_backward(s.sigma.data_ptr(), s.rgb.data_ptr(), s.deltas.data_ptr(), s.rays.data_ptr(), M, N,
                                                                   float(rcfg.T_thresh), 2 if s.bg is not None else 1, float(rcfg.bg_scalar),
                                                                   capi.ptr(s.bg), marched.nears.data_ptr(), marched.fars.data_ptr(),
                                                                   target.data_ptr(), geo_loss.lambda_distortion, geo_loss.lambda_depth,
                                                                   capi.ptr(geo_loss.target_depth), capi.ptr(geo_loss.depth_weight),
                                                                   capi.ptr(loss_scale), weights_sum.data_ptr(), image.data_ptr(), depth.data_ptr(),
                                                                   depth_raw.data_ptr(), distortion.data_ptr(),
                                                                   None if defer else loss.data_ptr(), ray_err.data_ptr(), g_sigma.data_ptr(),
                                                                   g_out16.data_ptr(), s.march_ws.data_ptr(),
                                                                   s.march_ws.numel() * s.march_ws.element_size(), capi.stream()))
        _network_backward(s, cfg, rcfg, g_sigma, g_out16, g_emb, g_ws, g_wc, found_inf, loss_job=(ray_err, loss) if defer else None,
                          overwrite=overwrite, table_adam=table_adam)
        return loss, image, depth, weights_sum, depth_raw, distortion
    capi.check(capi.lib.ngp_composite_train_loss_backward(s.sigma.data_ptr(), s.rgb.data_ptr(), s.deltas.data_ptr(), s.rays.data_ptr(), M, N,
                                                           float(rcfg.T_thresh), 2 if s.bg is not None else 1, float(rcfg.bg_scalar), capi.ptr(s.bg),
                                                           marched.nears.data_ptr(), marched.fars.data_ptr(), target.data_ptr(),
                                                           capi.ptr(loss_scale), weights_sum.data_ptr(), image.data_ptr(), depth.data_ptr(),
                                                           None if defer else loss.data_ptr(), ray_err.data_ptr(), g_sigma.data_ptr(),
                                                           g_out16.data_ptr(), s.march_ws.data_ptr(),
                                                           s.march_ws.numel() * s.march_ws.element_size(), capi.stream()))
    _network_backward(s, cfg, rcfg, g_sigma, g_out16, g_emb, g_ws, g_wc, found_inf, loss_job=(ray_err, loss) if defer else None,
                      overwrite=overwrite, table_adam=table_adam)
    return loss, image, depth, weights_sum


@torch.no_grad()
def fused_train_iteration_split(model, rays_o, rays_d, target, box, counter, capacity, loss_scale, bg_color=1, perturb=False, dt_gamma=0,
                                max_steps=1024, T_thresh=1e-4, noise_seed=None, found_inf=None, overwrite_table=False, table_adam=None,
                                geo_loss=None):
    cfg = network_cfg(model.encoder, model.sigma_net, model.color_net, model.bound, True)
    bg_t, rcfg = _render_cfg(model, capacity, bg_color, perturb, dt_gamma, max_steps, T_thresh)
    bufs = _operands((model.encoder.embeddings, model.sigma_net.weights, model.color_net.weights), True, overwrite_table)
    if bufs.g_emb is None:
        raise RuntimeError('fused_train_iteration: the parameters are not managed by optim.NGPAdam(deposit=True)')
    rays_o = rays_o.contiguous().view(-1, 3)
    rays_d = rays_d.contiguous().view(-1, 3)
    target = target.contiguous().view(-1, 3)
    if target.shape[0] != rays_o.shape[0] or target.dtype != torch.float32:
        raise RuntimeError('fused_train_iteration: target must be [N,3] float32')
    if geo_loss is not None and not isinstance(geo_loss, GeoLoss):
        raise TypeError('fused_train_iteration: geo_loss must be a fused.GeoLoss')
    box_ = {}

    def march():
        box_['m'] = _render_train_march(rays_o, rays_d, model.density_bitfield, box, counter, cfg, rcfg, noise_seed, into=box_.get('m'))

    def rest():
        ta = _table_adam_of(table_adam, model)
        out = _train_iteration_rest(box_['m'], bufs, bg_t, model.encoder.offsets, target, loss_scale, cfg, rcfg, found_inf, overwrite_table, ta,
                                    geo_loss)
        if overwrite_table:
            announce_overwrite(model.encoder.embeddings, None if ta is None else _table_adam_prefix(model, cfg, capacity))
        return out
    return march, rest


density_point_spacing = None


@torch.no_grad()
def fused_density(x, encoder, sigma_net, bound):
    M = x.shape[0]
    dev = x.device
    st = capi.stream()
    emb16, w16 = _half_weights((encoder.embeddings, sigma_net.weights))
    L = int(encoder.num_levels)
    enc = torch.empty(L, M, 2, device=dev, dtype=torch.half)
    S, H = float(np.log2(encoder.per_level_scale)), int(encoder.base_resolution)
    costs = None if density_point_spacing is None else capi.ray_level_costs(L, S, H, float(density_point_spacing))
    _grid_forward(x.contiguous(), emb16, encoder.offsets, enc, M, L, S, H, int(encoder.gridtype_id), int(bool(encoder.align_corners)),
                  int(encoder.interp_id), bound, costs, st)
    h16 = torch.empty(M, 16, device=dev, dtype=torch.half)
    capi.check(capi.lib.ngp_ffmlp_inference_ex(enc.data_ptr(), w16.data_ptr(), M, 32, 16, 64, int(sigma_net.num_layers), 0, 6, None, h16.data_ptr(),
                                                _PLANAR_IN, st))
    return torch.exp(h16[:, 0].float()), h16[:, 1:]


def inference_weights(model, x):
    enc, sn, cn = getattr(model, 'encoder', None), getattr(model, 'sigma_net', None), getattr(model, 'color_net', None)
    if enc is None or sn is None or cn is None or torch.is_grad_enabled():
        return None
    probe = torch.empty(128, 3, device=x.device, dtype=torch.float32)
    if not getattr(model, '_fused_ok', lambda *_: False)(probe, probe):
        return None
    emb16, ws16, wc16 = _half_weights((enc.embeddings, sn.weights, cn.weights), cast=False)
    if emb16 is None or ws16 is None or wc16 is None or getattr(emb16, '_ngp_sel', None) is not None:
        return None
    return emb16, ws16, wc16, network_cfg(enc, sn, cn, model.bound, False)


class pinned_half_weights:

    def __init__(self, model):
        enc, sn, cn = getattr(model, 'encoder', None), getattr(model, 'sigma_net', None), getattr(model, 'color_net', None)
        self.params = [getattr(enc, 'embeddings', None), getattr(sn, 'weights', None), getattr(cn, 'weights', None)]

    def __enter__(self):
        if all(p is not None and p.is_cuda for p in self.params) and not torch.is_grad_enabled():
            for p in self.params:
                fn = getattr(p, '_ngp_materialize', None)
                if fn is not None:
                    fn()
                buf = getattr(p, '_ngp_fp16_pinbuf', None)
                if buf is None or buf.shape != p.shape or buf.device != p.device:
                    buf = torch.empty_like(p, dtype=torch.half)
                    p._ngp_fp16_pinbuf = buf
                buf.copy_(p.detach())
                p._ngp_fp16_pin = buf
        return self

    def __exit__(self, *exc):
        for p in self.params:
            if p is not None and hasattr(p, '_ngp_fp16_pin'):
                del p._ngp_fp16_pin
        return False
```

Baseline: 653.3 million.

## Recompute first hidden layer in MLP backward instead of storing it

Adds flags that let the fused forward skip storing hidden layer 0 of the sigma and/or colour MLPs. The paired backward kernel then recomputes that layer from the input tile with the first-layer weights, which are kept in LDS. A second, opt-in flag stores only column 0 of the sigma output h16 instead of all 16 columns. The default env setting enables first-layer recompute for the colour network only. This trades forward-buffer write and read traffic for extra MFMA work and LDS space in the backward.

```diff
diff --git a/include/ngp_hip.h b/include/ngp_hip.h
--- a/include/ngp_hip.h
+++ b/include/ngp_hip.h
@@ -205,6 +205,10 @@
 #define NGP_FF_DEFER_REDUCE 16u
 #define NGP_FF_RECOMPUTE 32u
 #define NGP_FF_SERIAL_FLUSH 64u
+#define NGP_FF_RECOMPUTE_FIRST 128u
+#define NGP_FF_H0_ONLY 256u
+#define NGP_FF_RECOMPUTE_FIRST_SIGMA 512u
+#define NGP_FF_RECOMPUTE_FIRST_COLOR 1024u
 int ngp_ffmlp_forward_ex(const void* inputs, const void* weights, uint32_t B, uint32_t input_dim, uint32_t output_dim,
                          uint32_t hidden_dim, uint32_t num_layers, uint32_t activation, uint32_t output_activation,
                          void* forward_buffer, void* outputs, uint32_t flags, ngp_stream_t stream);
diff --git a/torch-ngp_amd/_ngp_capi.py b/torch-ngp_amd/_ngp_capi.py
--- a/torch-ngp_amd/_ngp_capi.py
+++ b/torch-ngp_amd/_ngp_capi.py
@@ -9,6 +9,7 @@
 NGP_F32, NGP_F16, NGP_F64 = 0, 1, 2
 NGP_FF_INPUT_PLANAR, NGP_FF_DX_PLANAR, NGP_FF_LAYERED, NGP_FF_SINGLE_WAVE, NGP_FF_DEFER_REDUCE, NGP_FF_RECOMPUTE = 1, 2, 4, 8, 16, 32
 NGP_FF_SERIAL_FLUSH = 64
+NGP_FF_RECOMPUTE_FIRST, NGP_FF_H0_ONLY, NGP_FF_RECOMPUTE_FIRST_SIGMA, NGP_FF_RECOMPUTE_FIRST_COLOR = 128, 256, 512, 1024
 NGP_MARCH_RESET_COUNTER, NGP_MARCH_ZERO_TAIL, NGP_MARCH_NOISE_FROM_SEED, NGP_MARCH_SCAN_LAUNCH = 1, 2, 4, 8
 NGP_OPT_PHASE_CHECK, NGP_OPT_PHASE_UPDATE, NGP_OPT_PHASE_COMMIT, NGP_OPT_PHASE_FLIP = 1, 2, 4, 8
 ABI_VERSION = 11
diff --git a/torch-ngp_amd/csrc/ffmlp.hip b/torch-ngp_amd/csrc/ffmlp.hip
--- a/torch-ngp_amd/csrc/ffmlp.hip
+++ b/torch-ngp_amd/csrc/ffmlp.hip
@@ -314,14 +314,14 @@
 template <bool TRAIN, int NT>
 __device__ __forceinline__ void relu_network_tail(float16_t (&acc)[NT][2], float16_t (&o)[NT], const half8_t* __restrict__ hid_img,
                                                   const half8_t* __restrict__ out_img, uint32_t nl, half_t* __restrict__ fb, size_t layer_stride,
-                                                  const uint32_t (&tile)[NT], const bool (&live)[NT], int lane) {
+                                                  const uint32_t (&tile)[NT], const bool (&live)[NT], int lane, uint32_t first_stored) {
     constexpr int WIDTH = 64, NIB = 2, NKB = 4;
     half8_t hid[NT][NKB];
     for (uint32_t l = 0;; l++) {
 #pragma unroll
         for (int t = 0; t < NT; t++) {
             pack_hidden_relu<WIDTH>(acc[t], hid[t]);
-            if (TRAIN && fb && live[t]) {
+            if (TRAIN && fb && live[t] && l >= first_stored) {
                 half8_t* dst = reinterpret_cast<half8_t*>(fb) + l * layer_stride + (size_t)tile[t] * NKB * 64 + lane;
 #pragma unroll
                 for (int kb = 0; kb < NKB; kb++) stream_store(dst + kb * 64, hid[t][kb]);
@@ -356,9 +356,11 @@
     const half_t* __restrict__ enc, bool enc_planar, const float* __restrict__ dirs, uint32_t M_valid, const half_t* __restrict__ w_sigma,
     const half_t* __restrict__ w_color, half_t* __restrict__ fb_s, half_t* __restrict__ h16, float* __restrict__ sigma,
     half_t* __restrict__ color_in, half_t* __restrict__ fb_c, float* __restrict__ rgb, uint32_t n_tiles_cap, uint32_t nl_s, uint32_t nl_c,
-    float density_scale, const uint32_t* __restrict__ rows_dev) {
+    float density_scale, const uint32_t* __restrict__ rows_dev, uint32_t store_flags) {
     constexpr int WIDTH = 64, NIB = 2, NKB = 4;
     constexpr uint32_t in_kb = 2;
+    const uint32_t first_stored_s = (store_flags & NGP_FF_RECOMPUTE_FIRST_SIGMA) ? 1u : 0u, first_stored_c = (store_flags & NGP_FF_RECOMPUTE_FIRST_COLOR) ? 1u : 0u;
+    const bool h0_only = (store_flags & NGP_FF_H0_ONLY) != 0;
     const uint32_t n_tiles = rows_dev ? min(n_tiles_cap, (rows_dev[0] + (uint32_t)FF_TILE - 1u) / (uint32_t)FF_TILE) : n_tiles_cap;
     extern __shared__ __attribute__((aligned(16))) unsigned char smem[];
     half8_t* img_s = reinterpret_cast<half8_t*>(smem);
@@ -427,7 +429,7 @@
 #pragma unroll
                 for (int t = 0; t < NT; t++) acc[t][ib] = mfma(a, x_cur[t][kb], acc[t][ib]);
             }
-        relu_network_tail<TRAIN, NT>(acc, o, s_hid, s_out, nl_s, fb_s, layer_stride, tile, live, lane);
+        relu_network_tail<TRAIN, NT>(acc, o, s_hid, s_out, nl_s, fb_s, layer_stride, tile, live, lane, first_stored_s);
         half8_t cin[NT][2];
 #pragma unroll
         for (int t = 0; t < NT; t++) {
@@ -435,9 +437,13 @@
 #pragma unroll
             for (int c = 0; c < 4; c++) { lo[c] = (half_t)o[t][c]; hi[c] = (half_t)o[t][4 + c]; }
             if (TRAIN && live[t]) {
-                half_t* hrow = h16 + srow[t] * 16 + 4 * h;
-                *reinterpret_cast<half4_t*>(hrow) = lo;
-                *reinterpret_cast<half4_t*>(hrow + 8) = hi;
+                if (h0_only) {
+                    if (h == 0) h16[srow[t]] = lo[0];
+                } else {
+                    half_t* hrow = h16 + srow[t] * 16 + 4 * h;
+                    *reinterpret_cast<half4_t*>(hrow) = lo;
+                    *reinterpret_cast<half4_t*>(hrow + 8) = hi;
+                }
             }
             if (h == 0 && live[t]) sigma[srow[t]] = density_scale * expf((float)lo[0]);
             const float x = dir_x[t], y = dir_y[t], z = dir_z[t];
@@ -486,7 +492,7 @@
 #pragma unroll
                 for (int t = 0; t < NT; t++) acc[t][ib] = mfma(a, cin[t][kb], acc[t][ib]);
             }
-        relu_network_tail<TRAIN, NT>(acc, o, c_hid, c_out, nl_c, fb_c, layer_stride, tile, live, lane);
+        relu_network_tail<TRAIN, NT>(acc, o, c_hid, c_out, nl_c, fb_c, layer_stride, tile, live, lane, first_stored_c);
 #pragma unroll
         for (int t = 0; t < NT; t++) {
             if (h == 0 && live[t]) {
@@ -1009,6 +1015,7 @@
     const half_t* h16;
     half_t* grad_h16;
     float density_scale;
+    uint32_t h16_stride;
 };
 
 template <int WIDTH, int NHM, typename Sink>
@@ -1040,12 +1047,27 @@
     }
 }
 
+template <int WIDTH>
+__device__ __forceinline__ void recompute_first(const half8_t* __restrict__ fimg_lane, uint32_t in_kb, const unsigned char* xb, bool in_planar,
+                                                int lane, half8_t (&hid)[Shape<WIDTH>::NKB]) {
+    constexpr int NIB = Shape<WIDTH>::NIB;
+    float16_t acc[NIB];
+#pragma unroll
+    for (int ib = 0; ib < NIB; ib++) acc[ib] = zero16();
+    for (uint32_t kb = 0; kb < in_kb; kb++) {
+        const half8_t x = tile_x(xb, kb, in_planar, lane);
+#pragma unroll
+        for (int ib = 0; ib < NIB; ib++) acc[ib] = mfma(fimg_lane[(ib * in_kb + kb) * 64], x, acc[ib]);
+    }
+    pack_hidden_relu<WIDTH>(acc, hid);
+}
+
 template <int N>
 __device__ __forceinline__ void wait_vmcnt() {
     asm volatile("s_waitcnt vmcnt(%0)" ::"n"(N) : "memory");
 }
 
-template <int WIDTH, int IN_JB, int NHM , bool RELU, bool RECOMP = false>
+template <int WIDTH, int IN_JB, int NHM , bool RELU, bool RECOMP = false, bool FIRST = false >
 __global__ __launch_bounds__(FP_THREADS) __attribute__((amdgpu_waves_per_eu(2, 2)))
 void k_ffmlp_backward_paired(const half_t* __restrict__ grad, const half_t* __restrict__ inputs, const half_t* __restrict__ weights,
                              const half_t* __restrict__ forward_buffer, uint32_t n_tiles, uint32_t in_dim, uint32_t num_layers, uint32_t act,
@@ -1053,19 +1075,22 @@
                              half_t* __restrict__ grad_weights_direct, bool in_planar, bool dx_planar, uint32_t pf_depth, MidEpilogue mid,
                              uint32_t lds_bytes, bool serial_flush) {
     static_assert(NHM == 1 || NHM == 2, "the paired backward covers 2- and 3-layer networks");
+    static_assert(RECOMP || !FIRST, "FIRST narrows RECOMP to hidden layer 0");
     constexpr int NIB = Shape<WIDTH>::NIB, NKB = Shape<WIDTH>::NKB;
+    constexpr bool FULL = RECOMP && !FIRST;
+    constexpr int L0 = FIRST ? 1 : 0;
     extern __shared__ __attribute__((aligned(16))) unsigned char smem[];
     half8_t* img = reinterpret_cast<half8_t*>(smem);
     const uint32_t nfrag = bwd_frag_count<WIDTH>(in_dim, num_layers, with_dx);
     const uint32_t in_kb = in_dim / 16;
-    const uint32_t ffrag = RECOMP ? NIB * in_kb + (num_layers - 1) * NIB * NKB : 0u;
+    const uint32_t ffrag = FULL ? NIB * in_kb + (num_layers - 1) * NIB * NKB : FIRST ? NIB * in_kb : 0u;
     const int lane = threadIdx.x & 63, wid = threadIdx.x >> 6;
     const int n = lane & 31, h = lane >> 5;
     const int pair = wid & (FP_PAIRS - 1), role = wid / FP_PAIRS;
     const size_t layer_stride = (size_t)n_tiles * NKB * 64;
-    const half8_t* fb = reinterpret_cast<const half8_t*>(forward_buffer);
+    const half8_t* fb = reinterpret_cast<const half8_t*>(forward_buffer) + (FIRST ? layer_stride : 0);
     const size_t rows = (size_t)n_tiles * FF_TILE;
-    const uint32_t act_layers = RECOMP ? 0u : num_layers;
+    const uint32_t act_layers = FULL ? 0u : num_layers - L0;
     const uint32_t tile_frags = 1 + act_layers * NKB + in_kb;
     unsigned char* pf_base = smem + (size_t)(nfrag + ffrag) * 1024 + (size_t)pair * pf_depth * tile_frags * 1024;
     half8_t* scratch = reinterpret_cast<half8_t*>(smem + (size_t)(nfrag + ffrag) * 1024 + (size_t)FP_PAIRS * pf_depth * tile_frags * 1024 +
@@ -1093,15 +1118,19 @@
     const half8_t* img_in = img_hid + (size_t)(num_layers - 1) * NIB * NKB * 64;
     const half8_t* fimg = img + (size_t)nfrag * 64 + lane;
     static_assert(tile_dma_count<64>(0, 32, false) == 3u && tile_dma_count<64>(0, 32, true) == 9u && tile_dma_count<64>(2, 32, false) == 11u &&
-                  tile_dma_count<64>(2, 32, true) == 17u, "the enumerated vmcnt immediates below are the DMA counts of the three-deep shapes");
-    const bool deep = pf_depth == 3 && (tile_loads == 3u || tile_loads == 9u || tile_loads == 11u || tile_loads == 17u);
+                  tile_dma_count<64>(2, 32, true) == 17u && tile_dma_count<64>(1, 32, false) == 7u && tile_dma_count<64>(1, 32, true) == 13u,
+                  "the enumerated vmcnt immediates below are the DMA counts of the three-deep shapes");
+    const bool deep = pf_depth == 3 && (tile_loads == 3u || tile_loads == 7u || tile_loads == 9u || tile_loads == 11u || tile_loads == 13u ||
+                                        tile_loads == 17u);
     auto next_tile_buffer = [&](uint32_t base) -> const unsigned char* {
         if (role == 0) {
             if (deep && base + base_step + pair < n_tiles) {
                 switch (tile_loads) {
                     case 3u: wait_vmcnt<3>(); break;
+                    case 7u: wait_vmcnt<7>(); break;
                     case 9u: wait_vmcnt<9>(); break;
                     case 11u: wait_vmcnt<11>(); break;
+                    case 13u: wait_vmcnt<13>(); break;
                     default: wait_vmcnt<17>(); break;
                 }
             } else {
@@ -1151,7 +1180,7 @@
                 const half8_t* tfrag = reinterpret_cast<const half8_t*>(tb) + lane;
                 const half8_t dy = tfrag[0];
                 half8_t a_top[NKB], a_below[NKB];
-                if constexpr (RECOMP) {
+                if constexpr (FULL) {
                     recompute_hidden<WIDTH, NHM>(fimg, in_kb, tb + 1024, in_planar, lane, [&](int l, const half8_t (&hid)[NKB]) {
                         if (l == NHM) {
 #pragma unroll
@@ -1163,9 +1192,11 @@
                     });
                 } else {
 #pragma unroll
-                    for (int kb = 0; kb < NKB; kb++) a_top[kb] = tfrag[(1 + NHM * NKB + kb) * 64];
-#pragma unroll
-                    for (int kb = 0; kb < NKB; kb++) a_below[kb] = tfrag[(1 + (NHM - 1) * NKB + kb) * 64];
+                    for (int kb = 0; kb < NKB; kb++) a_top[kb] = tfrag[(1 + (NHM - L0) * NKB + kb) * 64];
+                    if constexpr (!(FIRST && NHM == 1)) {
+#pragma unroll
+                        for (int kb = 0; kb < NKB; kb++) a_below[kb] = tfrag[(1 + (NHM - 1 - L0) * NKB + kb) * 64];
+                    }
                 }
                 half8_t aT[NIB][2], zT[NIB][2];
                 transpose_hidden<WIDTH>(a_top, sel, aT);
@@ -1182,6 +1213,7 @@
                 half8_t dz[NKB];
                 activation_transfer<WIDTH, RELU>(act, acc, a_top, dz);
                 transpose_hidden<WIDTH>(dz, sel, zT);
+                if constexpr (FIRST && NHM == 1) recompute_first<WIDTH>(fimg, in_kb, tb + (size_t)(1 + act_layers * NKB) * 1024, in_planar, lane, a_below);
                 transpose_hidden<WIDTH>(a_below, sel, aT);
                 wgrad_blocks(zT, aT, gw_top);
             }
@@ -1224,8 +1256,9 @@
                 const half8_t* tfrag = reinterpret_cast<const half8_t*>(tb) + lane;
                 const half8_t dy = tfrag[0];
                 half8_t a_prev[NKB];
-                const half8_t* afrag = RECOMP ? scratch : tfrag + 64;
-                if constexpr (RECOMP) {
+                const half8_t* afrag = FULL ? scratch : tfrag + 64;
+                const unsigned char* xb = tb + (size_t)(1 + act_layers * NKB) * 1024;
+                if constexpr (FULL) {
                     recompute_hidden<WIDTH, NHM>(fimg, in_kb, tb + 1024, in_planar, lane, [&](int l, const half8_t (&hid)[NKB]) {
                         if (l == NHM) {
 #pragma unroll
@@ -1238,20 +1271,28 @@
                     asm volatile("" ::: "memory");
                 } else {
 #pragma unroll
-                    for (int kb = 0; kb < NKB; kb++) a_prev[kb] = afrag[(NHM * NKB + kb) * 64];
+                    for (int kb = 0; kb < NKB; kb++) a_prev[kb] = afrag[((NHM - L0) * NKB + kb) * 64];
                 }
                 float16_t acc[NIB];
                 dgrad_out<WIDTH>(img_out, dy, acc);
                 half8_t dz[NKB];
                 half8_t aT[NIB][2], zT[NIB][2];
                 activation_transfer<WIDTH, RELU>(act, acc, a_prev, dz);
-#pragma unroll
-                for (int kb = 0; kb < NKB; kb++) a_prev[kb] = afrag[((NHM - 1) * NKB + kb) * 64];
+                if constexpr (FIRST && NHM == 1) {
+                    recompute_first<WIDTH>(fimg, in_kb, xb, in_planar, lane, a_prev);
+                } else {
+#pragma unroll
+                    for (int kb = 0; kb < NKB; kb++) a_prev[kb] = afrag[((NHM - 1 - L0) * NKB + kb) * 64];
+                }
                 dgrad_hidden<WIDTH>(img_hid, dz, acc);
                 if constexpr (NHM == 2) {
                     activation_transfer<WIDTH, RELU>(act, acc, a_prev, dz);
-#pragma unroll
-                    for (int kb = 0; kb < NKB; kb++) a_prev[kb] = afrag[kb * 64];
+                    if constexpr (FIRST) {
+                        recompute_first<WIDTH>(fimg, in_kb, xb, in_planar, lane, a_prev);
+                    } else {
+#pragma unroll
+                        for (int kb = 0; kb < NKB; kb++) a_prev[kb] = afrag[kb * 64];
+                    }
                     transpose_hidden<WIDTH>(dz, sel, zT);
                     transpose_hidden<WIDTH>(a_prev, sel, aT);
                     wgrad_blocks(zT, aT, gw_low);
@@ -1271,7 +1312,7 @@
 #pragma unroll
                     for (int e = 0; e < 2; e++) {
                         const uint32_t kb = 2 * jb + e;
-                        if (kb < in_kb) t = mfma(tile_x(tb + (size_t)(1 + act_layers * NKB) * 1024, kb, in_planar, lane), sel.nat[e], t);
+                        if (kb < in_kb) t = mfma(tile_x(xb, kb, in_planar, lane), sel.nat[e], t);
                     }
                     half8_t xT[2];
                     pack_transposed(t, xT);
@@ -1292,7 +1333,7 @@
                         const float sib2 = __shfl_xor((float)v2[3], 32, 64), sib3 = __shfl_xor((float)v3[3], 32, 64);
                         half4_t a, b;
                         if (h == 0) {
-                            const float x0 = (float)mid.h16[srow * 16];
+                            const float x0 = (float)mid.h16[srow * mid.h16_stride];
                             const float gs = (mid.density_scale * mid.grad_sigma[srow]) * (x0 != x0 ? x0 : expf(fminf(15.0f, fmaxf(-15.0f, x0))));
                             a = half4_t{to_half_rne(gs), v2[0], v2[1], v2[2]};
                             b = half4_t{(half_t)sib2, v3[0], v3[1], v3[2]};
@@ -1788,7 +1829,7 @@
     size_t stage, total;
 };
 template <int WIDTH, int IN_JB, int NHM>
-static BackwardLds backward_lds_plan(uint32_t in_dim, uint32_t num_layers, bool with_dx, uint32_t flags, bool recompute) {
+static BackwardLds backward_lds_plan(uint32_t in_dim, uint32_t num_layers, bool with_dx, uint32_t flags, bool recompute, bool first = false) {
     constexpr int NKB = Shape<WIDTH>::NKB;
     static_assert(FF_WAVES == FP_PAIRS, "one tile stream per wave or per pair: the same number of tile buffers");
     const SlabLayout lay{WIDTH, in_dim, num_layers};
@@ -1801,8 +1842,9 @@
         p.pf_depth = 3;
         scratch = (size_t)FP_PAIRS * NHM * NKB * 1024;
     } else {
-        p.image = (size_t)nfrag * 1024;
-        p.tile = (size_t)(1 + num_layers * NKB + in_dim / 16) * 1024;
+        const uint32_t first_frags = first ? (uint32_t)Shape<WIDTH>::NIB * (in_dim / 16) : 0u;
+        p.image = (size_t)(nfrag + first_frags) * 1024;
+        p.tile = (size_t)(1 + (num_layers - (first ? 1u : 0u)) * NKB + in_dim / 16) * 1024;
         p.pf_depth = p.image + 2 * FF_WAVES * p.tile > 160 * 1024 ? 1 : 2;
     }
     const bool paired = (NHM == 1 || NHM == 2) && !(flags & NGP_FF_SINGLE_WAVE);
@@ -1826,13 +1868,24 @@
     return reduce_slabs(backward_buffer, blocks, n_params, grad_weights, st, "ffmlp_backward(reduce)");
 }
 
+static const char* const FF_FIRST_SHAPES = "ffmlp_backward: NGP_FF_RECOMPUTE_FIRST serves 64-wide ReLU networks with 32 inputs and 2 or 3 layers";
+static int check_recompute_first(uint32_t flags, uint32_t in_dim, uint32_t hidden, uint32_t num_layers, uint32_t act) {
+    if (!(flags & NGP_FF_RECOMPUTE_FIRST)) return NGP_OK;
+    NGP_REQUIRE(!(flags & NGP_FF_RECOMPUTE), NGP_ERR_INVALID,
+                "ffmlp_backward: NGP_FF_RECOMPUTE_FIRST and NGP_FF_RECOMPUTE exclude each other (the first hidden layer, or all of them)");
+    NGP_REQUIRE(!(flags & (NGP_FF_SINGLE_WAVE | NGP_FF_LAYERED)), NGP_ERR_INVALID,
+                "ffmlp_backward: NGP_FF_RECOMPUTE_FIRST needs the paired kernel (not NGP_FF_SINGLE_WAVE, not NGP_FF_LAYERED)");
+    NGP_REQUIRE(hidden == 64 && in_dim == 32 && (num_layers == 2 || num_layers == 3) && act == ACT_RELU, NGP_ERR_INVALID, "%s", FF_FIRST_SHAPES);
+    return NGP_OK;
+}
+
 template <int WIDTH, int IN_JB, int NHM, bool RELU>
 static int launch_backward_t(const void* grad, const void* inputs, const void* weights, const void* fwd, uint32_t B, uint32_t in_dim,
                            uint32_t num_layers, uint32_t act, bool with_dx, void* backward_buffer, void* grad_inputs,
                            void* grad_weights, uint32_t flags, hipStream_t st, const MidEpilogue* mid_in) {
     const bool in_planar = (flags & NGP_FF_INPUT_PLANAR) != 0, dx_planar = (flags & NGP_FF_DX_PLANAR) != 0;
     const bool defer = (flags & NGP_FF_DEFER_REDUCE) != 0, serial = (flags & NGP_FF_SERIAL_FLUSH) != 0;
-    const MidEpilogue mid = mid_in ? *mid_in : MidEpilogue{nullptr, nullptr, nullptr, 0.0f};
+    const MidEpilogue mid = mid_in ? *mid_in : MidEpilogue{nullptr, nullptr, nullptr, 0.0f, 16u};
     const uint32_t n_tiles = B / FF_TILE;
     const uint32_t n_params = SlabLayout{WIDTH, in_dim, num_layers}.n_params();
     const BackwardLds lds = backward_lds_plan<WIDTH, IN_JB, NHM>(in_dim, num_layers, with_dx, flags, false);
@@ -1854,6 +1907,20 @@
             NGP_REQUIRE(false, NGP_ERR_INVALID, "ffmlp_backward: NGP_FF_RECOMPUTE serves 64-wide ReLU networks with 32 inputs and 2 or 3 layers");
         }
     }
+    if (flags & NGP_FF_RECOMPUTE_FIRST) {
+        if constexpr (WIDTH == 64 && IN_JB == 1 && RELU && (NHM == 1 || NHM == 2)) {
+            const BackwardLds lds_f = backward_lds_plan<WIDTH, IN_JB, NHM>(in_dim, num_layers, with_dx, flags, false, true);
+            NGP_REQUIRE(lds_f.total <= 160 * 1024, NGP_ERR_INVALID, "ffmlp_backward: LDS need (%zu B) exceeds 160 KiB", lds_f.total);
+            auto pk = k_ffmlp_backward_paired<WIDTH, IN_JB, NHM, RELU, true, true>;
+            return launch_and_reduce(reinterpret_cast<const void*>(pk), lds_f.total, blocks, defer, backward_buffer, grad_weights, n_params, st,
+                                     [&](dim3 grid, float* slabs, half_t* direct) {
+                NGP_LAUNCH(pk, grid, dim3(FP_THREADS), lds_f.total, st, g, x, w, (const half_t*)fwd, n_tiles, in_dim, num_layers, act, with_dx,
+                                   (half_t*)grad_inputs, slabs, direct, in_planar, dx_planar, lds_f.pf_depth, mid, (uint32_t)lds_f.total, serial);
+            });
+        } else {
+            NGP_REQUIRE(false, NGP_ERR_INVALID, "%s", FF_FIRST_SHAPES);
+        }
+    }
     if constexpr (NHM == 1 || NHM == 2) {
         if (!(flags & NGP_FF_SINGLE_WAVE)) {
             auto pk = k_ffmlp_backward_paired<WIDTH, IN_JB, NHM, RELU>;
@@ -1946,6 +2013,8 @@
     NGP_REQUIRE(grad && inputs && weights && (forward_buffer || (flags & NGP_FF_RECOMPUTE)) && backward_buffer && grad_weights, NGP_ERR_INVALID,
                 "ffmlp_backward: NULL tensor");
     NGP_REQUIRE(!calc_grad_inputs || grad_inputs, NGP_ERR_INVALID, "ffmlp_backward: grad_inputs is NULL but calc_grad_inputs is set");
+    rc = check_recompute_first(flags, input_dim, hidden_dim, num_layers, activation);
+    if (rc) return rc;
     hipStream_t st = as_stream(stream);
     const bool dx = calc_grad_inputs != 0;
     const bool fast = ff_register_resident(input_dim, hidden_dim, num_layers) && !(flags & NGP_FF_LAYERED);
@@ -2009,15 +2078,19 @@
                                           ngp_stream_t stream) {
     NGP_REQUIRE(num_layers_color == 2 || num_layers_color == 3, NGP_ERR_INVALID,
                 "network_backward_color: 2 or 3 layers (got %u); use ngp_ffmlp_backward_ex + ngp_pipeline_mid_backward", num_layers_color);
-    NGP_REQUIRE(!(flags & ~(NGP_FF_DEFER_REDUCE | NGP_FF_RECOMPUTE | NGP_FF_SERIAL_FLUSH)), NGP_ERR_INVALID,
-                "network_backward_color: only NGP_FF_DEFER_REDUCE, NGP_FF_RECOMPUTE and NGP_FF_SERIAL_FLUSH are accepted");
+    NGP_REQUIRE(!(flags & ~(NGP_FF_DEFER_REDUCE | NGP_FF_RECOMPUTE | NGP_FF_SERIAL_FLUSH | NGP_FF_RECOMPUTE_FIRST | NGP_FF_H0_ONLY)), NGP_ERR_INVALID,
+                "network_backward_color: only NGP_FF_DEFER_REDUCE, NGP_FF_RECOMPUTE, NGP_FF_SERIAL_FLUSH, NGP_FF_RECOMPUTE_FIRST and NGP_FF_H0_ONLY "
+                "are accepted");
+    NGP_REQUIRE((flags & (NGP_FF_RECOMPUTE | NGP_FF_RECOMPUTE_FIRST)) != (NGP_FF_RECOMPUTE | NGP_FF_RECOMPUTE_FIRST), NGP_ERR_INVALID,
+                "network_backward_color: NGP_FF_RECOMPUTE_FIRST and NGP_FF_RECOMPUTE exclude each other (the first hidden layer, or all of them)");
     int rc = check_ff_args("network_backward_color", M, 32, 16, 64, num_layers_color);
     if (rc) return rc;
     if (M == 0) return NGP_OK;
     NGP_REQUIRE(grad_out16 && color_in && w_color && (forward_buffer_color || (flags & NGP_FF_RECOMPUTE)) && backward_buffer && grad_sigma && h16 &&
                     grad_h16 && grad_w_color,
                 NGP_ERR_INVALID, "network_backward_color: NULL tensor");
-    const MidEpilogue mid{grad_sigma, (const half_t*)h16, (half_t*)grad_h16, density_scale};
+    const MidEpilogue mid{grad_sigma, (const half_t*)h16, (half_t*)grad_h16, density_scale, (flags & NGP_FF_H0_ONLY) ? 1u : 16u};
+    flags &= ~NGP_FF_H0_ONLY;
     if (num_layers_color == 2)
         return launch_backward<64, 1, 1>(grad_out16, color_in, w_color, forward_buffer_color, M, 32, 2, ACT_RELU, true, backward_buffer, nullptr,
                                          grad_w_color, flags, as_stream(stream), &mid);
@@ -2043,6 +2116,12 @@
     NGP_REQUIRE(enc && dirs && w_sigma && w_color && sigma && rgb, NGP_ERR_INVALID, "network_forward: NULL tensor");
     NGP_REQUIRE(!training || (h16 && color_in && (forward_buffer_sigma != nullptr) == (forward_buffer_color != nullptr)), NGP_ERR_INVALID,
                 "network_forward: the training variant needs h16 and color_in, and both forward buffers or (NGP_FF_RECOMPUTE backward) neither");
+    const uint32_t store_flags = flags & (NGP_FF_RECOMPUTE_FIRST_SIGMA | NGP_FF_RECOMPUTE_FIRST_COLOR | NGP_FF_H0_ONLY);
+    NGP_REQUIRE(training || !store_flags, NGP_ERR_INVALID,
+                "network_forward: NGP_FF_RECOMPUTE_FIRST_SIGMA, NGP_FF_RECOMPUTE_FIRST_COLOR and NGP_FF_H0_ONLY belong to the training variant");
+    NGP_REQUIRE(forward_buffer_sigma || !(store_flags & (NGP_FF_RECOMPUTE_FIRST_SIGMA | NGP_FF_RECOMPUTE_FIRST_COLOR)), NGP_ERR_INVALID,
+                "network_forward: NGP_FF_RECOMPUTE_FIRST_SIGMA / _COLOR and NGP_FF_RECOMPUTE exclude each other (without forward buffers no layer is "
+                "stored at all)");
     const size_t lds = forward_image_bytes<64>(32, num_layers_sigma) + forward_image_bytes<64>(32, num_layers_color);
     NGP_REQUIRE(lds <= 152 * 1024, NGP_ERR_INVALID, "network_forward: weights (%zu B) exceed the LDS of a CU", lds);
 #ifndef NGP_NETFWD_TRAIN_WAVES
@@ -2077,11 +2156,11 @@
     if (training)
         NGP_LAUNCH((k_network_forward<true, TW, TT>), dim3(blocks), dim3(TW * 64), lds, st, (const half_t*)enc, planar, dirs, M_valid, (const half_t*)w_sigma,
                            (const half_t*)w_color, (half_t*)forward_buffer_sigma, (half_t*)h16, sigma, (half_t*)color_in, (half_t*)forward_buffer_color, rgb,
-                           n_tiles, num_layers_sigma, num_layers_color, density_scale, rows_dev);
+                           n_tiles, num_layers_sigma, num_layers_color, density_scale, rows_dev, store_flags);
     else
         NGP_LAUNCH((k_network_forward<false, IW, IT>), dim3(blocks), dim3(IW * 64), lds, st, (const half_t*)enc, planar, dirs, M_valid, (const half_t*)w_sigma,
                            (const half_t*)w_color, (half_t*)nullptr, (half_t*)nullptr, sigma, (half_t*)nullptr, (half_t*)nullptr, rgb, n_tiles,
-                           num_layers_sigma, num_layers_color, density_scale, rows_dev);
+                           num_layers_sigma, num_layers_color, density_scale, rows_dev, 0u);
     return check_launch("network_forward");
 }
 
diff --git a/torch-ngp_amd/fused.py b/torch-ngp_amd/fused.py
--- a/torch-ngp_amd/fused.py
+++ b/torch-ngp_amd/fused.py
@@ -117,12 +117,15 @@
 USE_FUSED_NETWORK = True
 
 
-def _network_forward(enc, dirs, d_valid, ws16, wc16, nl_sigma, nl_color, density_scale, training, fb_s, h16, sigma, color_in, fb_c, out16, rgb, M, st):
+def _network_forward(enc, dirs, d_valid, ws16, wc16, nl_sigma, nl_color, density_scale, training, fb_s, h16, sigma, color_in, fb_c, out16, rgb, M, st,
+                     store_flags=0):
     if USE_FUSED_NETWORK:
         capi.check(capi.lib.ngp_network_forward(enc.data_ptr(), dirs.data_ptr(), M, d_valid, ws16.data_ptr(), wc16.data_ptr(), nl_sigma, nl_color,
                                                  float(density_scale), 1 if training else 0, capi.ptr(fb_s), capi.ptr(h16) if training else None,
-                                                 sigma.data_ptr(), capi.ptr(color_in) if training else None, capi.ptr(fb_c), rgb.data_ptr(), _PLANAR_IN, st))
+                                                 sigma.data_ptr(), capi.ptr(color_in) if training else None, capi.ptr(fb_c), rgb.data_ptr(), _PLANAR_IN | store_flags,
+                                                 st))
         return
+    assert not store_flags
     if training:
         capi.check(capi.lib.ngp_ffmlp_forward_ex(enc.data_ptr(), ws16.data_ptr(), M, 32, 16, 64, nl_sigma, 0, 6, fb_s.data_ptr(), h16.data_ptr(),
                                                   _PLANAR_IN, st))
@@ -216,7 +219,7 @@
     return Marched(xyzs, dirs, deltas, rays, nears, fars, ws)
 
 
-def _render_train_network(marched, bufs, bg, offsets, cfg, rcfg, composite=True):
+def _render_train_network(marched, bufs, bg, offsets, cfg, rcfg, composite=True, lean=None):
     xyzs, rays = marched.xyzs, marched.rays
     nl_sigma, nl_color = cfg.nl_sigma, cfg.nl_color
     N, M = rays.shape[0], rcfg.capacity
@@ -227,7 +230,8 @@
     enc = torch.empty(cfg.L, M, 2, **half)
     costs = capi.ray_level_costs(cfg.L, cfg.S, cfg.H, 3.0 ** 0.5 / (rcfg.max_steps * max(float(cfg.bound), 1e-6))) if USE_BALANCED_FORWARD else None
     _grid_forward(xyzs, bufs.emb16, offsets, enc, M, cfg.L, cfg.S, cfg.H, cfg.gridtype, cfg.align, cfg.interp, cfg.bound, costs, st)
-    h16 = torch.empty(M, 16, **half)
+    lean = lean or Lean(False, False, False)
+    h16 = torch.empty(M, **half) if lean.h0_only else torch.empty(M, 16, **half)
     color_in = torch.empty(M, 32, **half)
     out16 = torch.empty(M, 16, **half)
     sigma = torch.empty(M, **f32)
@@ -238,7 +242,7 @@
         fb_s = torch.empty(nl_sigma, M, 64, **half)
         fb_c = torch.empty(nl_color, M, 64, **half)
     _network_forward(enc, marched.dirs, M, bufs.ws16, bufs.wc16, nl_sigma, nl_color, float(rcfg.density_scale), True, fb_s, h16, sigma, color_in, fb_c,
-                     out16, rgb, M, st)
+                     out16, rgb, M, st, store_flags=lean.forward_flags())
     saved = Saved(xyzs, offsets, enc, bufs.ws16, bufs.wc16, fb_s, fb_c, h16, color_in, rgb, sigma, marched.deltas, rays, weights_sum=None,
                   image_raw=None, bg=bg, march_ws=marched.ws)
     if not composite:
@@ -275,7 +279,8 @@
 
 
 def _network_backward(saved, cfg, rcfg, g_sigma, g_out16, g_emb, g_ws, g_wc, found_inf=None, loss_job=None, overwrite=False, table_adam=None,
-                      input_grads=False):
+                      input_grads=False, lean=None):
+    lean = lean or Lean(False, False, False)
     if input_grads and saved.fb_c is None:
         raise RuntimeError('fused: gradients with respect to the rays need the stored activations of the MLPs; this render was run with '
                            'NGP_FUSED_RECOMPUTE=1 (NGP_FF_RECOMPUTE: no forward buffers) -- switch it off to refine poses')
@@ -292,12 +297,15 @@
         scratch_s = torch.empty(nl_sigma, M, 64, **half)
         g_h16 = torch.empty(M, 16, **half)
         rc = capi.NGP_FF_RECOMPUTE if s.fb_c is None else 0
+        first_c = capi.NGP_FF_RECOMPUTE_FIRST if lean.first_color else 0
+        first_s = capi.NGP_FF_RECOMPUTE_FIRST if lean.first_sigma else 0
+        h0 = capi.NGP_FF_H0_ONLY if lean.h0_only else 0
         capi.check(capi.lib.ngp_network_backward_color(g_out16.data_ptr(), s.color_in.data_ptr(), s.wc16.data_ptr(), capi.ptr(s.fb_c), M, nl_color,
                                                         scratch_c.data_ptr(), g_sigma.data_ptr(), s.h16.data_ptr(), float(density_scale),
-                                                        g_h16.data_ptr(), g_wc.data_ptr(), capi.NGP_FF_DEFER_REDUCE | rc, st))
+                                                        g_h16.data_ptr(), g_wc.data_ptr(), capi.NGP_FF_DEFER_REDUCE | rc | first_c | h0, st))
         capi.check(capi.lib.ngp_ffmlp_backward_ex(g_h16.data_ptr(), s.enc.data_ptr(), s.ws16.data_ptr(), capi.ptr(s.fb_s), M, 32, 16, 64, nl_sigma,
                                                    0, 6, 1, scratch_s.data_ptr(), g_enc.data_ptr(), g_ws.data_ptr(),
-                                                   _PLANAR_IN | _PLANAR_DX | capi.NGP_FF_DEFER_REDUCE | rc, st))
+                                                   _PLANAR_IN | _PLANAR_DX | capi.NGP_FF_DEFER_REDUCE | rc | first_s, st))
         n_c, n_s = capi.lib.ngp_ffmlp_backward_slab_count(M, 32, 64, nl_color), capi.lib.ngp_ffmlp_backward_slab_count(M, 32, 64, nl_sigma)
         if USE_SLABS_IN_ACCUMULATE:
             err, loss = loss_job if loss_job is not None else (None, None)
@@ -310,6 +318,8 @@
         capi.check(capi.lib.ngp_ffmlp_reduce_slabs_pair(scratch_c.data_ptr(), n_c, g_wc.numel(), g_wc.data_ptr(), scratch_s.data_ptr(), n_s, g_ws.numel(),
                                                          g_ws.data_ptr(), capi.ptr(found_inf), st))
     else:
+        if any(lean):
+            raise RuntimeError('fused: this backward reads hidden layer 0 and every column of h16; the forward was told not to store them')
         if found_inf is not None:
             raise RuntimeError('fused: found_inf needs the fused colour-head / slab-reduction path (see iteration_checks_gradients)')
         if loss_job is not None:
@@ -441,6 +451,24 @@
 USE_RECOMPUTE = os.environ.get('NGP_FUSED_RECOMPUTE', '0') == '1'
 
 
+_first = os.environ.get('NGP_FUSED_RECOMPUTE_FIRST', 'color').lower()
+USE_RECOMPUTE_FIRST = (_first in ('sigma', 'both', '1'), _first in ('color', 'colour', 'both', '1'))
+USE_H0_ONLY = os.environ.get('NGP_FUSED_H0_ONLY', '0') == '1'
+
+
+class Lean(namedtuple('Lean', 'first_sigma first_color h0_only')):
+    __slots__ = ()
+
+    def forward_flags(self):
+        return ((capi.NGP_FF_RECOMPUTE_FIRST_SIGMA if self.first_sigma else 0) | (capi.NGP_FF_RECOMPUTE_FIRST_COLOR if self.first_color else 0) |
+                (capi.NGP_FF_H0_ONLY if self.h0_only else 0))
+
+
+def _lean_stores(nl_sigma, nl_color):
+    ok = bool(USE_FUSED_NETWORK and USE_FUSED_MID and nl_color in (2, 3) and nl_sigma in (2, 3) and not _recompute(nl_sigma, nl_color))
+    return Lean(bool(ok and USE_RECOMPUTE_FIRST[0]), bool(ok and USE_RECOMPUTE_FIRST[1]), bool(ok and USE_H0_ONLY))
+
+
 def _carries_reductions(nl_sigma, nl_color):
     return bool(USE_SLABS_IN_ACCUMULATE and USE_FUSED_MID and nl_color in (2, 3) and nl_sigma in (2, 3))
 
@@ -469,7 +497,8 @@
                                                    grad_image.data_ptr(), capi.stream()))
         _render_train_backward(saved, cfg, rcfg, grad_image, None, g_emb, g_ws, g_wc, found_inf, overwrite)
         return loss, image, depth, weights_sum
-    s = _render_train_network(marched, bufs, bg_t, offsets, cfg, rcfg, composite=False)
+    lean = _lean_stores(cfg.nl_sigma, cfg.nl_color)
+    s = _render_train_network(marched, bufs, bg_t, offsets, cfg, rcfg, composite=False, lean=lean)
     N, M, dev = s.rays.shape[0], s.xyzs.shape[0], s.xyzs.device
     f32 = dict(device=dev, dtype=torch.float32)
     weights_sum, image, depth = torch.empty(N, **f32), torch.empty(N, 3, **f32), torch.empty(N, **f32)
@@ -494,7 +523,7 @@
                                                                    g_out16.data_ptr(), s.march_ws.data_ptr(),
                                                                    s.march_ws.numel() * s.march_ws.element_size(), capi.stream()))
         _network_backward(s, cfg, rcfg, g_sigma, g_out16, g_emb, g_ws, g_wc, found_inf, loss_job=(ray_err, loss) if defer else None,
-                          overwrite=overwrite, table_adam=table_adam)
+                          overwrite=overwrite, table_adam=table_adam, lean=lean)
         return loss, image, depth, weights_sum, depth_raw, distortion
     capi.check(capi.lib.ngp_composite_train_loss_backward(s.sigma.data_ptr(), s.rgb.data_ptr(), s.deltas.data_ptr(), s.rays.data_ptr(), M, N,
                                                            float(rcfg.T_thresh), 2 if s.bg is not None else 1, float(rcfg.bg_scalar), capi.ptr(s.bg),
@@ -504,7 +533,7 @@
                                                            g_out16.data_ptr(), s.march_ws.data_ptr(),
                                                            s.march_ws.numel() * s.march_ws.element_size(), capi.stream()))
     _network_backward(s, cfg, rcfg, g_sigma, g_out16, g_emb, g_ws, g_wc, found_inf, loss_job=(ray_err, loss) if defer else None,
-                      overwrite=overwrite, table_adam=table_adam)
+                      overwrite=overwrite, table_adam=table_adam, lean=lean)
     return loss, image, depth, weights_sum
 
 
```

After: 659.4 million, median of 6. About the same (+0.9%).
